# Meryx/ComputeRayTracer

Measured on AMD Instinct MI355X. Metric: Mrays/sec (+ HBM GB/s vs peak), 1080p 250k-tri scene, 1/2/4/8 MI355X, higher is better.
Workload: dtype f32; 1 GPU; S2 atrium250k: 253952 triangles + cornell walls/light, 1920x1080, 64 spp per step (BASELINE config 3)

## Files before the change

computeraytracer_amd/_lib.py:

```python
from __future__ import annotations

import ctypes as C
import os

_HERE = os.path.dirname(os.path.abspath(__file__))
LIB_PATH = os.environ.get("CRT_LIB") or os.path.join(_HERE, "libcrt.so")

NCOUNTERS = 8
ACCEL_NONE, ACCEL_BVH2, ACCEL_LBVH, ACCEL_PLOC = 0, 1, 2, 3
CNT = dict(rays=0, nodes=1, prims=2, paths=3, bounces=4, shadow=5, hits=6, walked=7)

_P = C.c_void_p
SIGNATURES = {
    "crt_create": (C.c_int, [C.POINTER(_P), C.c_int]),
    "crt_destroy": (None, [_P]),
    "crt_last_error": (C.c_char_p, [_P]),
    "crt_abi_version": (C.c_int, []),
    "crt_upload_scene": (C.c_int, [_P, _P, C.c_size_t, _P, C.c_size_t, _P, C.c_size_t, _P, _P]),
    "crt_set_tile": (C.c_int, [_P, C.c_uint32, C.c_uint32, C.c_uint32, C.c_uint32]),
    "crt_set_row_bands": (C.c_int, [_P, C.c_uint32, C.c_uint32, C.c_uint32]),
    "crt_build_accel": (C.c_int, [_P, C.c_int]),
    "crt_reset": (C.c_int, [_P]),
    "crt_trace": (C.c_int, [_P, C.c_uint32]),
    "crt_sync": (C.c_int, [_P]),
    "crt_sample_count": (C.c_int, [_P, _P]),
    "crt_tile": (C.c_int, [_P, _P]),
    "crt_read_accum": (C.c_int, [_P, _P]),
    "crt_read_rgba8": (C.c_int, [_P, _P]),
    "crt_write_accum": (C.c_int, [_P, _P, C.c_uint32]),
    "crt_read_latest_rgba8": (C.c_int, [_P, _P, _P]),
    "crt_latest_sample": (C.c_int, [_P, _P]),
    "crt_pin_host": (C.c_int, [_P, C.c_size_t]),
    "crt_unpin_host": (C.c_int, [_P]),
    "crt_read_sample_rgba8": (C.c_int, [_P, C.c_uint32, _P]),
    "crt_device_buffers": (C.c_int, [_P, C.POINTER(_P), C.POINTER(_P)]),
    "crt_bind_output": (C.c_int, [_P, _P, _P]),
    "crt_set_stream": (C.c_int, [_P, _P]),
    "crt_enable_counters": (C.c_int, [_P, C.c_int]),
    "crt_counters": (C.c_int, [_P, _P]),
    "crt_reset_counters": (C.c_int, [_P]),
    "crt_last_trace_ms": (C.c_int, [_P, _P, _P]),
    "crt_last_kernel_ms": (C.c_int, [_P, _P, _P]),
    "crt_set_option": (C.c_int, [_P, C.c_char_p, C.c_int64]),
    "crt_accel_stats": (C.c_int, [_P, _P]),
    "crt_get_device": (C.c_int, [_P, _P]),
    "crt_get_stream": (C.c_int, [_P, C.POINTER(_P)]),
    "crt_image_size": (C.c_int, [_P, _P]),
    "crt_comm_unique_id": (C.c_int, [_P, C.c_int]),
    "crt_comm_init": (C.c_int, [_P, _P, C.c_int, C.c_int]),
    "crt_comm_partition": (C.c_int, [_P, C.c_uint32]),
    "crt_gather": (C.c_int, [_P, C.c_int]),
    "crt_read_frame_rgba8": (C.c_int, [_P, _P]),
    "crt_read_frame_accum": (C.c_int, [_P, _P]),
    "crt_frame_device_buffers": (C.c_int, [_P, C.POINTER(_P), C.POINTER(_P)]),
    "crt_comm_info": (C.c_int, [_P, _P]),
    "crt_comm_destroy": (C.c_int, [_P]),
    "crt_layout_rows": (C.c_int, [C.c_uint32, C.c_uint32, C.c_uint32, C.c_uint32, _P, _P]),
    "crt_denoise": (C.c_int, [_P, _P, _P, _P]),
    "crt_denoise_latest": (C.c_int, [_P, _P, _P, _P, _P]),
    "crt_read_gbuffer": (C.c_int, [_P, _P]),
    "crt_read_motion": (C.c_int, [_P, _P]),
    "crt_render_aovs": (C.c_int, [_P, C.c_uint32, _P]),
    "crt_spectrum_rgb": (C.c_int, [_P, _P, _P]),
    "crt_read_albedo_table": (C.c_int, [_P, _P]),
    "crt_render_mattes": (C.c_int, [_P, C.c_uint32, C.c_int, C.c_uint32, _P]),
    "crt_set_primitive_ids": (C.c_int, [_P, C.c_uint32, C.c_uint32, _P]),
    "crt_read_primitive_ids": (C.c_int, [_P, C.c_uint32, C.c_uint32, _P]),
    "crt_debug_intersect": (C.c_int, [_P, _P, C.c_size_t, _P]),
    "crt_debug_trace_rays": (C.c_int, [_P, _P, C.c_size_t, _P, _P]),
    "crt_debug_walk_rays": (C.c_int, [_P, C.c_int, _P, C.c_size_t, _P, _P]),
    "crt_debug_read_accel": (C.c_int, [_P, C.c_int, _P, C.c_size_t, _P]),
    "crt_debug_probes": (C.c_int, [_P, _P]),
    "crt_debug_gen_culled": (C.c_int, [_P, _P]),
    "crt_debug_deferred_nee": (C.c_int, [_P, _P]),
    "crt_debug_tile_classes": (C.c_int, [_P, _P, C.c_size_t]),
    "crt_debug_tile_classes_host": (C.c_int, [_P, _P, C.c_size_t]),
    "crt_debug_tile_class_setups": (C.c_int, [_P, _P]),
# ... 120 lines not shown
```

computeraytracer_amd/csrc/crt_api.cpp:

```cpp
#include "crt_ctx.h"

using namespace crt;

extern "C" void crt_comm_on_destroy(crt_ctx *c);
extern "C" int crt_internal_comm_partitioned(crt_ctx *c);

namespace crt {

long long g_fail_alloc_in = 0;

namespace {
std::string g_create_error;
}

int fail(crt_ctx *c, int code, const char *fmt, ...)
{
    char buf[2048];
    va_list ap;
    va_start(ap, fmt);
    vsnprintf(buf, sizeof buf, fmt, ap);
    va_end(ap);
    if (c) c->err = buf; else g_create_error = buf;
    return code;
}
// ... 182 lines not shown
            return fail(c, CRT_EINVAL, "primitive %zu: spectrum index out of range", i);
    }
    for (size_t i = 0; i < nlight; i++) {
        lts[i] = read_prim((const uint8_t *)lights, i);
        if (lts[i].emission >= nspectra) return fail(c, CRT_EINVAL, "light %zu: emission index out of range", i);
    }
    c->have_scene = false;
    c->accel_mode = -1;
    c->dn.valid = false; c->fdn.valid = false;
    c->sample_offset = 0;
    c->dn.drop();
    c->prims.swap(prims);
    c->prims_moved = false;
    matte_ids_identity(c);
    c->lights.swap(lts);
    std::memcpy(c->camera, camera, sizeof c->camera);
    c->W = (uint32_t)camera[11];
    c->H = (uint32_t)camera[12];

    DevScene &S = c->sc;
    S = DevScene{};
    S.W = c->W; S.H = c->H;
    S.nspectra = (uint32_t)nspectra;
    S.nlight = (uint32_t)nlight;
    S.inv_nlight = 1.0f / (float)S.nlight;
    c->s_prims = prims_scale(c->prims);
    S.hit_pad = pad_of(c->s_prims, c->camera);
    c->accel_stale = false; c->accel_topo = false;
    c->rf_ready = false;
    S.nf_last[0] = S.nf_last[1] = kNoHit;
    for (size_t i = c->prims.size(); i-- > 0 && S.nf_last[1] == kNoHit;)
        if (c->prims[i].category != 2u) (S.nf_last[0] == kNoHit ? S.nf_last[0] : S.nf_last[1]) = (uint32_t)i;
    camera_frame(c->camera, S.cam);

    HIPCHK(c, c->d_raw.alloc(std::max<size_t>(nprim * 80, 16)));
    if (nprim) HIPCHK(c, hipMemcpy(c->d_raw.p, primitives, nprim * 80, hipMemcpyHostToDevice));
    HIPCHK(c, c->d_spectra.alloc(nspectra * kNLambda));
    HIPCHK(c, hipMemcpy(c->d_spectra.p, spectra, nspectra * kNLambda * sizeof(float), hipMemcpyHostToDevice));
    HIPCHK(c, c->d_cie.alloc(3 * kNCie));
    HIPCHK(c, hipMemcpy(c->d_cie.p, cie, 3 * kNCie * sizeof(float), hipMemcpyHostToDevice));
    c->cie_zero = tc_culled_is_zero(cie);
    aov_rebuild_albedo(c, spectra, nspectra, cie);
    std::vector<float4> hl(nlight * 3);
    for (size_t i = 0; i < nlight; i++) light_rows(c->lights[i], &hl[3 * i]);
    HIPCHK(c, c->d_lights.alloc(hl.size()));
    HIPCHK(c, hipMemcpy(c->d_lights.p, hl.data(), hl.size() * sizeof(float4), hipMemcpyHostToDevice));
    S.spectra = c->d_spectra.p; S.cie = c->d_cie.p; S.lights = c->d_lights.p;

    c->x0 = 0; c->y0 = 0; c->tw = c->W; c->th = c->H;
    c->band = 0x40000000u; c->stride = 1; c->phase = 0;
    c->accum_bound = nullptr; c->rgba_bound = nullptr;
    c->have_scene = true;
    int rc = alloc_tile(c);
    if (rc == CRT_OK) rc = zero_state(c);
    if (rc) c->have_scene = false;
    return rc;
}

int crt_set_tile(crt_ctx *c, uint32_t x0, uint32_t y0, uint32_t x1, uint32_t y1)
{
    if (!c) return CRT_EINVAL;
    if (!c->have_scene) return fail(c, CRT_ESTATE, "crt_set_tile: upload a scene first");
    if (x0 > x1 || y0 > y1 || x1 > c->W || y1 > c->H)
        return fail(c, CRT_EINVAL, "crt_set_tile: rectangle [%u,%u)x[%u,%u) outside %ux%u", x0, x1, y0, y1, c->W, c->H);
    CRT_TRY(quiesce(c, true));
    c->x0 = x0; c->y0 = y0; c->tw = x1 - x0; c->th = y1 - y0;
    c->band = 0x40000000u; c->stride = 1; c->phase = 0;
    return retile(c);
}

int crt_set_row_bands(crt_ctx *c, uint32_t band_rows, uint32_t parts, uint32_t part)
{
    if (!c) return CRT_EINVAL;
    if (!c->have_scene) return fail(c, CRT_ESTATE, "crt_set_row_bands: upload a scene first");
    if (band_rows == 0 || parts == 0 || part >= parts || band_rows > 65536u)
        return fail(c, CRT_EINVAL, "crt_set_row_bands: need band_rows >= 1 and part < parts");
    CRT_TRY(quiesce(c, true));
    uint32_t rows = 0;
    for (uint32_t b = part; (unsigned long long)b * band_rows < c->H; b += parts)
        rows += std::min<uint32_t>(band_rows, c->H - b * band_rows);
    c->x0 = 0; c->y0 = 0; c->tw = c->W; c->th = rows;
    c->band = band_rows; c->stride = parts; c->phase = part;
    return retile(c);
}

int crt_build_accel(crt_ctx *c, int mode)
{
    if (!c) return CRT_EINVAL;
    if (!c->have_scene) return fail(c, CRT_ESTATE, "crt_build_accel: upload a scene first");
    if (mode != CRT_ACCEL_NONE && mode != CRT_ACCEL_BVH2 && mode != CRT_ACCEL_LBVH && mode != CRT_ACCEL_PLOC)
        return fail(c, CRT_EINVAL, "crt_build_accel: unknown mode %d", mode);
    c->want_builder = mode == CRT_ACCEL_LBVH ? 1 : mode == CRT_ACCEL_PLOC ? 2 : 0;
    if (c->want_builder) mode = CRT_ACCEL_BVH2;
    CRT_TRY(quiesce(c, true));
    c->accel_mode = -1;
    c->dn.valid = false; c->fdn.valid = false;
    return build_tree(c, mode);
}

int crt_reset(crt_ctx *c)
{
    if (!c) return CRT_EINVAL;
    if (!c->have_scene) return fail(c, CRT_ESTATE, "crt_reset: upload a scene first");
    CRT_TRY(quiesce(c, false));
    return zero_state(c);
}

int crt_trace(crt_ctx *c, uint32_t n_samples)
{
    if (!c) return CRT_EINVAL;
    if (c->as_on) return as_refuse(c, "crt_trace");
    if (!c->have_scene) return fail(c, CRT_ESTATE, "crt_trace: upload a scene first");
    if (c->accel_mode < 0) return fail(c, CRT_ESTATE, "crt_trace: call crt_build_accel first");
    if (c->accel_stale) return fail(c, CRT_ESTATE, "crt_trace: primitives were updated: call crt_refit_accel or crt_build_accel first");
    if (c->sample_offset) {
        if (!(c->pipeline == 1 && c->accel_mode == CRT_ACCEL_BVH2))
            return fail(c, CRT_ESTATE, "crt_trace: a sample offset needs the wavefront pipeline (\"pipeline\" = 1 and a tree): "
                                       "crt_set_sample_offset(ctx, 0) first");
        if ((unsigned long long)c->sample_offset + c->sample + n_samples > 0xFFFFFFFFull)
            return fail(c, CRT_EINVAL, "crt_trace: sample offset %u + %u samples so far + %u pass 2^32 - 1", c->sample_offset, c->sample, n_samples);
    }
    HIPCHK(c, hipSetDevice(c->device));
    if ((size_t)c->tw * c->th != 0 && (!accum_ptr(c) || !rgba_ptr(c)))
        return fail(c, CRT_ENOMEM, "crt_trace: the tile's output buffers are not allocated (an earlier crt_set_tile / crt_set_row_bands failed)");
    TraceParams P = trace_params(c);
    c->last_launches = 0;
    c->last_timed = true;
    c->last_iterations = 0;
    HIPCHK(c, hipEventRecord(c->ev0, c->stream));
// ... 451 lines not shown
        if (!c->time_kernels) return fail(c, CRT_ESTATE, "crt_last_kernel_ms: set option time_kernels=1 before crt_trace");
        HIPCHK(c, hipStreamSynchronize(c->stream));
        n = c->last_trace_kernel_launches;
        for (uint32_t i = 0; i < n; i++) {
            float t = 0.0f;
            HIPCHK(c, hipEventElapsedTime(&t, c->kev[2 * (size_t)i], c->kev[2 * (size_t)i + 1]));
            total += t;
        }
        c->last_trace_kernel_launches = 0;
    } else {
        HIPCHK(c, hipEventElapsedTime(&total, c->ev0, c->ev1));
        n = c->last_launches;
    }
    if (ms) *ms = total;
    if (launches) *launches = n;
    return CRT_OK;
}

int crt_accel_stats(crt_ctx *c, uint64_t out[8])
{
    if (!c || !out) return CRT_EINVAL;
    if (c->accel_topo) return fail(c, CRT_ESTATE, "crt_accel_stats: the tree belongs to another primitive list: call crt_refit_accel or crt_build_accel first");
    const bool wide = c->pipeline == 1 && c->accel_mode == CRT_ACCEL_BVH2 && c->bvh4.n_inner > 0;
    const bool wide8 = wide && c->bvh8q.ok;
    out[4] = wide ? (c->bvh4q.ok ? 16 : 32) : 32;
    out[5] = wide8 ? 8 : wide ? 4 : 2;
    out[6] = wide8 ? c->bvh8q.n_inner : wide ? c->bvh4.n_inner : c->bvh.n_inner;
    out[7] = (uint64_t)c->accel_builder;
    out[0] = c->bvh.n_inner; out[1] = c->bvh.n_leaves; out[2] = c->bvh.max_depth;
    out[3] = (uint64_t)c->bvh.n_inner * 64u + (uint64_t)c->bvh4.n_inner * 128u + (uint64_t)c->prims.size() * 48u;
    return CRT_OK;
}

int crt_set_option(crt_ctx *c, const char *name, int64_t value)
{
    if (!c || !name) return CRT_EINVAL;
    CRT_TRY(wf_flush(c));
    if (!std::strcmp(name, "debug_fail_alloc")) { g_fail_alloc_in = value; return CRT_OK; }
    if (!std::strcmp(name, "ploc_radius")) {
        if (value < 1 || value > 32) return fail(c, CRT_EINVAL, "crt_set_option: ploc_radius is 1..32");
        c->ploc.radius = (uint32_t)value;
        return CRT_OK;
    }
    if (!std::strcmp(name, "refit_rebuild_pct")) {
        if (value != 0 && (value < 100 || value > 100000)) return fail(c, CRT_EINVAL, "crt_set_option: refit_rebuild_pct is 0 (off) or 100..100000");
        c->refit_rebuild_pct = (int)value;
        return CRT_OK;
    }
    if (!std::strcmp(name, "debug_ploc_max_depth")) {
        if (value < 1 || value > 62) return fail(c, CRT_EINVAL, "crt_set_option: debug_ploc_max_depth is 1..62");
        c->ploc.max_depth = (uint32_t)value;
        return CRT_OK;
    }
    if (!std::strcmp(name, "debug_ploc_max_rounds")) {
        if (value < 1) return fail(c, CRT_EINVAL, "crt_set_option: debug_ploc_max_rounds is >= 1");
        c->ploc.max_rounds = (uint32_t)std::min<int64_t>(value, 1 << 30);
        return CRT_OK;
    }
    if (!std::strcmp(name, "wf_defer")) { c->wf_defer = value != 0; return CRT_OK; }
    if (!std::strcmp(name, "spp_per_launch")) { c->spp_per_launch = (uint32_t)std::max<int64_t>(0, value); return CRT_OK; }
    if (!std::strcmp(name, "pipeline")) { c->pipeline = value ? 1 : 0; return CRT_OK; }
    if (!std::strcmp(name, "quantize")) { c->quantize = value ? 1 : 0; return CRT_OK; }
    if (!std::strcmp(name, "wf_width")) { c->wf_width = value == 4 ? 4 : 8; return CRT_OK; }
    if (!std::strcmp(name, "wf_finish_at")) { c->wf_finish_at = (uint32_t)std::max<int64_t>(0, value); return CRT_OK; }
    if (!std::strcmp(name, "wf_flush_at")) { c->wf_flush_at = (uint32_t)std::max<int64_t>(0, value); return CRT_OK; }
    if (!std::strcmp(name, "wf_side_ppw")) { c->wf_side_ppw = (uint32_t)std::min<int64_t>(64, std::max<int64_t>(1, value)); return CRT_OK; }
// ... 15 lines not shown
    if (!std::strcmp(name, "adaptive_temporal")) {
        if (value != 0 && value != 1) return fail(c, CRT_EINVAL, "crt_set_option: adaptive_temporal is 0 or 1");
        c->adaptive_temporal = value != 0;
        return CRT_OK;
    }
    if (!std::strcmp(name, "svgf_spatial_pct")) {
        if (value != 0 && (value < 25 || value > 10000)) return fail(c, CRT_EINVAL, "crt_set_option: svgf_spatial_pct is 0 (off) or 25..10000");
        c->svgf_spatial_pct = (int)value;
        return CRT_OK;
    }
    if (!std::strcmp(name, "denoise_latest_wave_blocks")) {
        if (value != 0 && value != 1) return fail(c, CRT_EINVAL, "crt_set_option: denoise_latest_wave_blocks is 0 or 1");
        c->dn.wave_blocks = value != 0;
        return CRT_OK;
    }
    if (!std::strcmp(name, "temporal_clip_pct")) {
        if (value != 0 && (value < 25 || value > 10000)) return fail(c, CRT_EINVAL, "crt_set_option: temporal_clip_pct is 0 (off) or 25..10000");
        if (!value && c->dn.relit) c->dn.drop();
        if (!value) { c->dn.box.release(); c->dn.box_ran = false; }
        c->dn.clip_pct = (int)value;
        return CRT_OK;
    }
    if (!std::strcmp(name, "frame_ring")) {
        c->frame_ring = (uint32_t)std::min<int64_t>(256, std::max<int64_t>(0, value));
        c->ring_from = c->sample + 1u;
        if (c->have_scene) { HIPCHK(c, hipSetDevice(c->device)); HIPCHK(c, hipStreamSynchronize(c->stream)); return alloc_frames(c); }
        return CRT_OK;
    }
    if (!std::strcmp(name, "wf_gen_blocks")) { c->wf_gen_blocks = (int)std::min<int64_t>(4096, std::max<int64_t>(1, value)); return CRT_OK; }
    if (!std::strcmp(name, "wf_trace_form")) { c->wf_trace_form = value == 1 ? 1 : 2; return CRT_OK; }
    if (!std::strcmp(name, "wf_cull_miss")) { c->wf_cull_miss = value != 0; return CRT_OK; }
    if (!std::strcmp(name, "wf_cull_classes")) { c->wf_cull_classes = value != 0; return CRT_OK; }
    if (!std::strcmp(name, "wf_defer_nee")) { c->wf_defer_nee = value != 0; return CRT_OK; }
    if (!std::strcmp(name, "wf_affinity")) { c->wf_affinity = value != 0; return CRT_OK; }
    if (!std::strcmp(name, "wf_pipes")) { c->wf_pipes = (int)std::min<int64_t>(crt_ctx::kMaxPipes, std::max<int64_t>(1, value)); return CRT_OK; }
    if (!std::strcmp(name, "wf_pool")) { c->wf_pool = (uint32_t)std::max<int64_t>(0, value); return CRT_OK; }
    if (!std::strcmp(name, "wf_waves_per_cu")) { c->wf_waves_per_cu = (uint32_t)std::min<int64_t>(32, std::max<int64_t>(0, value)); return CRT_OK; }
    if (!std::strcmp(name, "time_kernels")) {
        c->time_kernels = value != 0; c->last_trace_kernel_launches = 0;
        HIPCHK(c, hipSetDevice(c->device));
        while (value > 1 && c->kev.size() < 2 * (size_t)std::min<int64_t>(value, 1 << 20)) {
            Event e;
            HIPCHK(c, e.create());
            c->kev.push_back(std::move(e));
        }
        return CRT_OK;
    }
    return fail(c, CRT_EINVAL, "crt_set_option: unknown option '%s'", name);
}

}
```

computeraytracer_amd/csrc/crt_ctx.h:

```cpp
#pragma once
#include <hip/hip_runtime.h>

#include <algorithm>
#include <cfloat>
#include <cmath>
#include <cstdarg>
#include <cstdio>
#include <cstdlib>
#include <cstring>
#include <memory>
#include <string>
#include <utility>
#include <vector>

#include "../../include/crt.h"
#include "crt_bvh.h"
#include "crt_device.h"
#include "crt_launch.h"
#include "crt_math.h"
#include "crt_tile_class.h"
#include "crt_wf_policy.h"

namespace crt {

struct HostPrim {
    uint32_t category;
    f3 d1, d2, d3;
    uint32_t emission, reflectance, material, index;
};

extern long long g_fail_alloc_in;

template <typename T>
struct DevBuf {
    T *p = nullptr;
    size_t n = 0;
    DevBuf() = default;
    DevBuf(DevBuf &&o) noexcept : p(o.p), n(o.n) { o.p = nullptr; o.n = 0; }
    DevBuf &operator=(DevBuf &&o) noexcept { std::swap(p, o.p); std::swap(n, o.n); return *this; }
    DevBuf(const DevBuf &) = delete;
    DevBuf &operator=(const DevBuf &) = delete;
    ~DevBuf() { release(); }
    hipError_t alloc(size_t count) {
        release();
        if (count == 0) return hipSuccess;
        const bool inject = g_fail_alloc_in > 0 && --g_fail_alloc_in == 0;
        const hipError_t e = inject ? hipErrorOutOfMemory : hipMalloc((void **)&p, count * sizeof(T));
        if (e != hipSuccess) { p = nullptr; return e; }
        n = count;
        return hipSuccess;
    }
    void release() { if (p) (void)hipFree(p); p = nullptr; n = 0; }
// ... 97 lines not shown
    uint32_t published = 0;
    uint32_t pending = 0;
    bool in_publish = false;
    uint32_t sample_offset = 0;
    uint32_t frame_id = 0;
    int wf_cohort = 16;

    DevBuf<unsigned long long> d_counters;
    bool counting = false;
    float last_ms = 0.0f;
    uint32_t last_launches = 0;
    bool last_timed = false;
    uint32_t spp_per_launch = 0;

    int pipeline = 1;
    uint32_t wf_pool = 0;
    uint32_t wf_waves_per_cu = 0;
    int num_cu = 0;
    DevBuf<float4> w_ray_o, w_ray_d, w_sh_d, w_beta, w_radiance, w_nee, w_staging[crt::kWfRing], w_recA, w_recB;
    DevBuf<uint4> w_rng, w_misc, w_recC;
    DevBuf<float2> w_hit;
    DevBuf<uint32_t> w_vis, w_dead, w_tea;
    DevBuf<uint8_t> w_dflag;
    DevBuf<uint32_t> w_tile_cls;
    static constexpr int kMaxPipes = crt::kWfMaxPipes;
    int wf_pipes = 2;
    int wf_defer = 1;
    int wf_tail_walk = 1;
    int wf_gen_blocks = 128;
    int wf_trace_form = 2;
    int wf_cull_miss = 1;
    int wf_cull_classes = 1;
    int wf_defer_nee = 1;
    int wf_affinity = 0;
    uint64_t mapped_gen_launches = 0;
    uint64_t tile_cls_setups = 0;
    bool cie_zero = false;
    int wf_chunk = 1;
    int wf_ahead = 3;
    int wf_ring = 32;
    int wf_pool_spp = 8;
    double wf_feed = 1.0;
    std::unique_ptr<crt::WfRun> run;
    uint32_t wf_finish_at = 32768;
    uint32_t wf_flush_at = 4096;
    uint32_t wf_side_ppw = 64, wf_flush_ppw = 4;
    DevBuf<crt::WfCtl> w_ctl[kMaxPipes];
    DevBuf<crt::WfWorkQ> w_wq;
    crt::Pinned<crt::WfStatus> h_status[kMaxPipes];
    crt::WfStatus *d_status[kMaxPipes] = {};
    crt::Event ev_status[kMaxPipes][crt::kStatusRing];
    crt::Event ev_done[kMaxPipes][crt::kStatusRing];
    crt::Pinned<uint32_t> h_dropped;
    bool wf_host_ready = false;
    crt::Stream pipe_stream[kMaxPipes];
    crt::Stream pub_stream;
    static constexpr int kFinishStreams = 3;
    crt::Stream fin_stream[kFinishStreams];
    crt::Event ev_fin[kFinishStreams];
    int fin_next = 0;
    crt::Event ev_fork, ev_join[kMaxPipes], ev_pub_join[kMaxPipes];
    crt::Event ev_evict[kMaxPipes][crt::kWfRing];
    crt::Event ev_resolved[crt::kWfRing];
    crt::Event ev_pub[crt::kWfRing];
    bool time_kernels = false;
    std::vector<crt::Event> kev;
// ... 107 lines not shown
        hipError_t e_ = (call);                                                                   \
        if (e_ != hipSuccess)                                                                     \
            return fail(c, e_ == hipErrorOutOfMemory ? CRT_ENOMEM : CRT_EDEVICE, "%s: %s", #call, \
                        hipGetErrorString(e_));                                                   \
    } while (0)

#define CRT_TRY(expr)                 \
    do {                              \
        const int rc_ = (expr);       \
        if (rc_) return rc_;          \
    } while (0)

#define CRT_ENSURE(c, buf, count)                              \
    do {                                                       \
        if (buf.n < (count)) HIPCHK(c, buf.alloc(count));      \
    } while (0)

inline float4 *accum_ptr(crt_ctx *c) { return c->accum_bound ? c->accum_bound : c->d_accum.p; }
inline uchar4 *rgba_ptr(crt_ctx *c) { return c->rgba_bound ? c->rgba_bound : c->d_rgba.p; }

int quiesce(crt_ctx *c, bool sync);

int alloc_tile(crt_ctx *c);
int zero_state(crt_ctx *c);
int as_refuse(crt_ctx *c, const char *what);
int as_refuse_broken(crt_ctx *c, const char *what);

HostPrim read_prim(const uint8_t *base, size_t i);
float prims_scale(const std::vector<HostPrim> &prims);
float pad_of(float S, const float cam[16]);
void light_rows(const HostPrim &l, float4 out[3]);
void camera_frame(const float cam[16], float out[12]);
int build_tree(crt_ctx *c, int mode);
uint32_t wf_stack_need(const crt_ctx *c);
uint32_t wf_stack_lds(const crt_ctx *c);
uint32_t wf_overflow_levels(const crt_ctx *c);

enum DnState { DN_UNIFORM, DN_ADAPTIVE, DN_EITHER, DN_TEMPORAL };
int dn_begin(crt_ctx *c, const char *what, uint32_t iterations, const float *values, int count, const char *which, DnState state);
int dn_finish(crt_ctx *c, size_t n, const float4 *res, float *rgb_out, uint8_t *rgba8_out, const float *plane = nullptr,
              float *plane_out = nullptr);
int dn_adaptive_params(crt_ctx *c, const char *what, const crt_denoise_adaptive_params *params, crt_denoise_adaptive_params *out);
int dn_check_state(crt_ctx *c, const char *what, bool adaptive = false);
int dn_adaptive_run(crt_ctx *c, const crt_denoise_adaptive_params &dp, bool rgba, bool var, float4 **res, const float **var_dev);

void aov_rebuild_albedo(crt_ctx *c, const float *spectra, size_t nspectra, const float *cie);

void matte_ids_identity(crt_ctx *c);
void matte_ids_reserve(crt_ctx *c, size_t n_new);
void matte_ids_remove(crt_ctx *c, const crt_prim_range *live, size_t m);
void matte_ids_append(crt_ctx *c, uint32_t count);

struct AsBatch {
    uint32_t off;
    uint32_t n_active;
    uint32_t commit;
};
WfOptions wf_options(const crt_ctx *c);
int wf_ensure_overflow(crt_ctx *c);
int wf_flush(crt_ctx *c);
int wf_check_dropped(crt_ctx *c);
int wf_tick(crt_ctx *c);
int wf_publish_pending(crt_ctx *c, bool force);
int wf_trace_batch(crt_ctx *c, uint32_t n, const AsBatch *as = nullptr);
int wf_wait_sample(crt_ctx *c, uint32_t sample);
double wf_now_ms();
// ... 4 lines not shown
```

computeraytracer_amd/csrc/crt_debug.cpp:

```cpp
#include "crt_ctx.h"

using namespace crt;

extern "C" {

int crt_debug_intersect(crt_ctx *c, const float *rays, size_t n, float *out)
{
    if (!c || (!rays && n) || (!out && n)) return CRT_EINVAL;
    if (!c->have_scene || c->accel_mode < 0) return fail(c, CRT_ESTATE, "crt_debug_intersect: scene + accel required");
    if (c->accel_stale) return fail(c, CRT_ESTATE, "crt_debug_intersect: primitives were updated: call crt_refit_accel or crt_build_accel first");
    HIPCHK(c, hipSetDevice(c->device));
    DevBuf<float> din, dout;
    HIPCHK(c, din.alloc(n * 8));
    hipError_t e = dout.alloc(n * 8);
    if (e == hipSuccess) e = hipMemcpyAsync(din.p, rays, n * 8 * sizeof(float), hipMemcpyHostToDevice, c->stream);
    if (e == hipSuccess) e = launch_debug_intersect(c->sc, din.p, n, dout.p, c->accel_mode == CRT_ACCEL_NONE, c->stream);
    if (e == hipSuccess) e = hipMemcpyAsync(out, dout.p, n * 8 * sizeof(float), hipMemcpyDeviceToHost, c->stream);
    if (e == hipSuccess) e = hipStreamSynchronize(c->stream);
    if (e != hipSuccess) return fail(c, CRT_EDEVICE, "crt_debug_intersect: %s", hipGetErrorString(e));
    return CRT_OK;
}

int crt_debug_trace_rays(crt_ctx *c, const float *rays, size_t n, uint32_t *out, uint64_t report[8])
{
// ... 166 lines not shown
    const bool device_route = tree && n4 > 0 && c->bvh4.nodes.size() < n4 * (size_t)kNode4Floats;
    const bool live4 = tree && n4 > 0 && !device_route, live4q = tree && n4 > 0 && c->sc.nodes4q != nullptr, live8q = n8 > 0 && c->sc.nodes8q != nullptr;
    double hdr[CRT_ACCEL_HEADER_N] = {0};
    const void *src = nullptr;
    size_t need = 0;
    switch (what) {
    case CRT_ACCEL_PART_HEADER: {
        const size_t lanes = (size_t)c->num_cu * wf_waves(wf_options(c)) * 64u * (size_t)std::max(1, c->wf_pipes);
        hdr[0] = c->accel_mode; hdr[1] = c->accel_builder; hdr[2] = (double)n;
        hdr[3] = tree ? c->sc.root : -1; hdr[4] = tree ? c->sc.root4 : -1; hdr[5] = live8q ? c->sc.root8 : -1;
        hdr[6] = (double)n2; hdr[7] = (double)n4; hdr[8] = (double)n8;
        hdr[9] = live4; hdr[10] = live4q; hdr[11] = live8q;
        for (int a = 0; a < 3; a++) { hdr[12 + a] = c->sc.qbase[a]; hdr[15 + a] = c->sc.qscale[a]; }
        hdr[18] = c->sc.hit_pad; hdr[19] = c->tree_pad;
        hdr[20] = c->bvh.max_depth; hdr[21] = c->bvh4.max_depth; hdr[22] = c->bvh8q.max_depth; hdr[23] = c->wf_depth;
        hdr[24] = wf_stack_need(c); hdr[25] = wf_stack_lds(c); hdr[26] = wf_overflow_levels(c);
        hdr[27] = lanes ? (double)(c->w_overflow.n / lanes) : 0.0;
        hdr[28] = c->accel_stale; hdr[29] = device_route;
        need = sizeof hdr;
        break;
    }
    case CRT_ACCEL_PART_NODES2: src = c->d_nodes.p; need = n2 * kNodeFloats * sizeof(float); break;
    case CRT_ACCEL_PART_NODES4: src = c->d_nodes4.p; need = live4 ? n4 * kNode4Floats * sizeof(float) : 0; break;
    case CRT_ACCEL_PART_NODES4Q: src = c->d_nodes4q.p; need = live4q ? n4 * 16 * sizeof(uint32_t) : 0; break;
    case CRT_ACCEL_PART_NODES8Q: src = c->d_nodes8q.p; need = live8q ? n8 * 32 * sizeof(uint32_t) : 0; break;
    case CRT_ACCEL_PART_PRIM: src = c->d_prim.p; need = n * 3 * sizeof(float4); break;
    case CRT_ACCEL_PART_PRIMD: src = c->d_primD.p; need = tree ? n * sizeof(float4) : 0; break;
    default: src = c->d_slot_of_index.p; need = n * sizeof(uint32_t); break;
    }
    if (bytes) *bytes = need;
    if (!out) return CRT_OK;
    if (capacity < need) return fail(c, CRT_EINVAL, "crt_debug_read_accel: part %d holds %zu bytes, the buffer %zu", what, need, capacity);
    if (what == CRT_ACCEL_PART_HEADER) std::memcpy(out, hdr, need);
    else if (need) HIPCHK(c, hipMemcpy(out, src, need, hipMemcpyDeviceToHost));
    return CRT_OK;
}

int crt_debug_math(crt_ctx *c, int fn, const float *a, const float *b, float *out, size_t n)
{
    if (!c || !a || !b || !out) return CRT_EINVAL;
    HIPCHK(c, hipSetDevice(c->device));
    DevBuf<float> da, db, dout;
    hipError_t e = da.alloc(n);
    if (e == hipSuccess) e = db.alloc(n);
    if (e == hipSuccess) e = dout.alloc(n);
    if (e == hipSuccess && n) e = hipMemcpyAsync(da.p, a, n * sizeof(float), hipMemcpyHostToDevice, c->stream);
    if (e == hipSuccess && n) e = hipMemcpyAsync(db.p, b, n * sizeof(float), hipMemcpyHostToDevice, c->stream);
    if (e == hipSuccess) e = launch_debug_math(fn, da.p, db.p, dout.p, n, c->stream);
    if (e == hipSuccess && n) e = hipMemcpyAsync(out, dout.p, n * sizeof(float), hipMemcpyDeviceToHost, c->stream);
    if (e == hipSuccess) e = hipStreamSynchronize(c->stream);
    if (e != hipSuccess) return fail(c, CRT_EDEVICE, "crt_debug_math: %s", hipGetErrorString(e));
    return CRT_OK;
}

int crt_debug_read_moments(crt_ctx *c, float *out)
{
    if (!c || !out) return CRT_EINVAL;
    CRT_TRY(dn_begin(c, "crt_debug_read_moments", 0, nullptr, 0, "", DN_TEMPORAL));
    if (!c->dn.cur.valid || c->dn.cur.frame != c->frame_id || !c->dn.cur.has_m)
        return fail(c, CRT_ESTATE, "crt_debug_read_moments: no crt_denoise_svgf in this frame yet, or a crt_denoise_temporal after it "
                                   "(the CURRENT slot carries no moments)");
    const size_t n = (size_t)c->tw * c->th;
    if (n) HIPCHK(c, hipMemcpyAsync(out, c->dn.cur.m.p, n * sizeof(float4), hipMemcpyDeviceToHost, c->stream));
    return dn_finish(c, n, nullptr, nullptr, nullptr);
}

// ... 81 lines not shown
```

computeraytracer_amd/csrc/crt_device.h:

```cpp
#pragma once
#include <hip/hip_runtime.h>
#include <stdint.h>

#include "crt_work_map.h"

namespace crt {

constexpr uint32_t kNoHit = 0xFFFFFFFFu;
constexpr int kStackDepth = 64;
constexpr uint32_t kWalk4q = 1u, kWalkFellBack = 2u;
constexpr uint32_t kNLambda = 301;
constexpr uint32_t kNCie = 471;
constexpr int CRT_NCOUNTERS_DEV = 16;

struct DevScene {
    const float4 *prim;
    const float4 *primD;
    const uint32_t *slot_of_index;
    const float4 *nodes;
    const float4 *nodes4;
    const uint4 *nodes4q;
    const uint4 *nodes8q;
    const float *spectra;
    const float *cie;
    const float4 *lights;
    uint32_t nprim;
    uint32_t npatch;
    int32_t root;
    int32_t root4;
    int32_t root8;
    uint32_t n_nodes4;
    uint32_t nspectra;
    uint32_t nlight;
    float hit_pad;
    uint32_t nf_last[2];
    float inv_nlight;
    uint32_t W, H;
    float qbase[3], qscale[3];
    float cam[12];
};

struct TraceParams {
    DevScene sc;
    uint32_t x0, y0, tw, th;
    uint32_t band, stride, phase;
    uint32_t first_sample, n_samples;
    float4 *accum;
    uchar4 *rgba;
    unsigned long long *counters;
    uint32_t tiles_x, tiles_y;
};

struct AsTiles {
    const uint32_t *active;
    const uint32_t *base;
    float *q;
    uint32_t n_active;
};

struct AsParams {
    const float4 *accum;
    const float *q;
    const uint32_t *counts;
    float *errors;
    uint32_t *flags;
    uint32_t *active;
    uint32_t *n_active;
    uint32_t tw, th, tiles_x, tiles_y;
    uint32_t min_samples, max_samples;
    float threshold;
};

struct AsVarParams {
// ... 220 lines not shown
```

computeraytracer_amd/csrc/crt_launch.h:

```cpp
#pragma once
#include <hip/hip_runtime.h>

#include <vector>

#include "../../include/crt.h"
#include "crt_bvh.h"
#include "crt_device.h"

namespace crt {

hipError_t launch_trace(const TraceParams &P, bool count, bool brute, hipStream_t stream);
hipError_t launch_trace_adaptive(const TraceParams &P, const AsTiles &A, bool count, bool brute, hipStream_t stream);
hipError_t launch_debug_intersect(const DevScene &S, const float *rays, size_t n, float *out, int brute, hipStream_t stream);
hipError_t launch_debug_walk_rays(const DevScene &S, int walk, const float *rays, size_t n, uint32_t *out, hipStream_t stream);
hipError_t launch_debug_math(int fn, const float *a, const float *b, float *out, size_t n, hipStream_t stream);
hipError_t launch_assemble(const void *full, void *frame, uint32_t elem_bytes, uint32_t W, uint32_t H, uint32_t world, uint32_t rows_max,
                           uint32_t band, hipStream_t stream);

hipError_t wf_launch_init(const WfParams &P, hipStream_t s);
hipError_t wf_launch_tea(const WfParams &P, uint32_t *out, hipStream_t s);
hipError_t wf_launch_tile_classes(const WfParams &P, uint32_t *out, hipStream_t s);
bool wf_gen_culls(const WfParams &P);
bool wf_gen_mapped(const WfParams &P);
hipError_t wf_launch_shade(const WfParams &P, uint32_t it, hipStream_t s);
hipError_t wf_launch_gen(const WfParams &P, uint32_t it, hipStream_t s, const AsTiles *A);
hipError_t wf_launch_trace(const WfParams &P, uint32_t it, uint32_t trace_blocks, hipStream_t s);
int wf_trace_kernel(const WfParams &P);
hipError_t wf_launch_finish(const WfParams &P, WfFinishSegs G, uint32_t max_paths, hipStream_t s);
hipError_t wf_launch_resolve(const WfParams &P, uint32_t last_sample, hipStream_t s);
hipError_t wf_launch_resolve_adaptive(const WfParams &P, const AsTiles &A, uint32_t call_end, hipStream_t s);

hipError_t as_launch_select(const AsParams &A, bool compact, hipStream_t s);
hipError_t as_launch_select_var(const AsVarParams &V, const AsParams *compact, hipStream_t s);
hipError_t as_launch_commit(uint32_t *counts, const uint32_t *active, uint32_t n_active, uint32_t samples, hipStream_t s);

hipError_t build_lbvh(const float *lo, const float *hi, uint32_t n, Bvh &out, hipStream_t stream);
hipError_t build_lbvh_device(const unsigned char *d_raw, uint32_t n, float hit_pad, float4 *d_prim, float4 *d_primD,
                             uint32_t *d_slot_of_index, float *d_nodes2, uint4 *d_nodes4q, LbvhDeviceResult &res, hipStream_t stream);
template <typename T> struct DevBuf;
hipError_t lbvh_sorted_keys_host(const float *lo, const float *hi, uint32_t n, float *d_lo, float *d_hi, unsigned long long *d_keys,
                                 unsigned long long *d_sorted, DevBuf<char> &sort_tmp, hipStream_t stream);
hipError_t lbvh_sorted_keys_device(const unsigned char *d_raw, uint32_t n, float hit_pad, float *d_lo, float *d_hi, uint32_t *d_cbox,
                                   unsigned long long *d_keys, unsigned long long *d_sorted, DevBuf<char> &sort_tmp, hipStream_t stream);
hipError_t lbvh_launch_gather(const unsigned char *d_raw, const unsigned long long *d_keys, uint32_t n, float4 *d_prim, float4 *d_primD,
                              uint32_t *d_slot_of_index, hipStream_t stream);
hipError_t lbvh_collapse_device(const float *d_nodes2, uint32_t n, uint4 *d_nodes4q, LbvhDeviceResult &res, hipStream_t stream);

hipError_t build_ploc(const float *lo, const float *hi, uint32_t n, const PlocOptions &opt, Bvh &out, PlocInfo &info, hipStream_t stream);
hipError_t build_ploc_device(const unsigned char *d_raw, uint32_t n, float hit_pad, const PlocOptions &opt, float4 *d_prim, float4 *d_primD,
                             uint32_t *d_slot_of_index, float *d_nodes2, uint4 *d_nodes4q, LbvhDeviceResult &res, PlocInfo &info,
                             hipStream_t stream);

hipError_t refit_launch_pad(const unsigned char *raw, uint32_t n, uint32_t *out, hipStream_t s);
hipError_t refit_launch_prims(const unsigned char *raw, uint32_t first, uint32_t count, const uint32_t *slot_of_index, float4 *prim,
                              float4 *primD, hipStream_t s);
hipError_t refit_launch_transform(unsigned char *raw, const uint32_t *start, const crt_prim_transform *ops, uint32_t n_ops, uint32_t total,
                                  const uint32_t *slot_of_index, float4 *prim, float4 *primD, hipStream_t s);
hipError_t refit_launch_compact(const unsigned char *src, unsigned char *dst, const uint32_t *tab, uint32_t n_gaps, uint32_t n_new, hipStream_t s);
hipError_t refit_levels(const void *nodes, uint32_t width, bool quantised, int root, uint32_t cap, int *list, uint32_t *counter,
                        uint32_t *nch, std::vector<uint32_t> &off, hipStream_t s);
hipError_t refit_launch_bvh2(const float4 *prim, float pad, const int *list, const std::vector<uint32_t> &off, float *nodes, hipStream_t s);
hipError_t refit_launch_wide(const float4 *prim, float pad, const int *list, const std::vector<uint32_t> &off, const void *refs,
                             bool quantised, const uint32_t *nch, float *fb, hipStream_t s);
hipError_t refit_launch_quant4(const float *fb, const uint32_t *nch, uint32_t n4, uint4 *nodes4q, const double base[3], const double scale[3],
                               hipStream_t s);

hipError_t quality_launch(int layout, const void *nodes, uint32_t n, uint32_t root, const float base[3], const float scale[3],
                          double2 *partial, double *out, hipStream_t s);

hipError_t dn_launch_gbuffer(const DevScene &S, uint32_t x0, uint32_t y0, uint32_t tw, uint32_t th, float4 *gbuf, uint32_t *key,
                             int brute, hipStream_t stream);
hipError_t dn_launch_filter(const DnFilter &F, const float4 *accum, float n, float sigma_color, float4 **out);
hipError_t dn_launch_prepare(const DnFilter &F, const float4 *accum, float n, hipStream_t stream);
hipError_t dn_launch_passes(const DnFilter &F, float sigma_color, bool wave_blocks, float4 **out);
hipError_t dn_launch_filter_adaptive(const DnFilter &F, const float4 *accum, const float *q, const uint32_t *counts, uint2 *kv,
                                     float *var, float sigma_variance, float4 **out);
hipError_t dn_launch_temporal(const DnFilter &F, DnReprojParams P, const uint32_t *counts, float sigma_color, float4 *box, float gamma,
                              float4 **out);
hipError_t dn_launch_svgf(const DnFilter &F, DnSvgfParams P, const uint32_t *counts, uint2 *kv, float *var, float sigma_variance,
                          float spatial_b, float4 *box, float gamma, float4 **out);
hipError_t dn_launch_motion(const DnReprojParams &P, float2 *out, hipStream_t stream);

hipError_t aov_launch(const DevScene &S, const AovParams &P, hipStream_t stream);

hipError_t matte_launch(const DevScene &S, const MatteParams &P, hipStream_t stream);

}
```

computeraytracer_amd/csrc/crt_lbvh.hip:

```cpp
#include <hip/hip_runtime.h>
#include <hipcub/hipcub.hpp>

#include <algorithm>
#include <cfloat>
#include <cstring>
#include <vector>

#include "crt_bvh.h"
#include "crt_ctx.h"
#include "crt_launch.h"
#include "crt_math.h"
#include "crt_prim.h"

namespace crt {
namespace {

__device__ __forceinline__ uint32_t expand10(uint32_t v)
{
    v &= 0x3FFu;
    v = (v | (v << 16)) & 0x030000FFu;
    v = (v | (v << 8)) & 0x0300F00Fu;
    v = (v | (v << 4)) & 0x030C30C3u;
    v = (v | (v << 2)) & 0x09249249u;
    return v;
// ... 262 lines not shown
        if (best < 0) break;
        CBox a, b;
        load_children(nodes2, ch[best].ref, a, b);
        ch[best] = a; ch[n++] = b;
    }
    uint32_t k = 0;
    for (int i = 0; i < n; i++) k += ch[i].ref >= 0 ? 1u : 0u;
    uint32_t pos = 0;
    if (k) pos = atomicAdd(out_count, k);
    int refs[4] = {0, 0, 0, 0};
    uint32_t j = 0;
    for (int i = 0; i < n; i++) {
        if (ch[i].ref >= 0) { frontier_out[pos + j] = ch[i].ref; refs[i] = (int)(next_base + pos + j); j++; }
        else refs[i] = ch[i].ref;
    }
    const double base[3] = {bx, by, bz}, scale[3] = {sx, sy, sz};
    uint32_t q[24];
    for (int i = 0; i < 4; i++)
        for (int a = 0; a < 3; a++) {
            if (i >= n) { q[4 * a + i] = 65535u; q[12 + 4 * a + i] = 0u; continue; }
            const double l = ((double)ch[i].lo[a] - base[a]) / scale[a], h = ((double)ch[i].hi[a] - base[a]) / scale[a];
            long long ql = (long long)floor(l) - 1, qh = (long long)ceil(h) + 1;
            ql = ql < 0 ? 0 : (ql > 65535 ? 65535 : ql); qh = qh < 0 ? 0 : (qh > 65535 ? 65535 : qh);
            q[4 * a + i] = (uint32_t)ql; q[12 + 4 * a + i] = (uint32_t)qh;
        }
    uint4 *o = nodes4q + 4 * (size_t)(level_base + t);
    o[0] = uint4{q[0] | (q[1] << 16), q[2] | (q[3] << 16), q[4] | (q[5] << 16), q[6] | (q[7] << 16)};
    o[1] = uint4{q[8] | (q[9] << 16), q[10] | (q[11] << 16), q[12] | (q[13] << 16), q[14] | (q[15] << 16)};
    o[2] = uint4{q[16] | (q[17] << 16), q[18] | (q[19] << 16), q[20] | (q[21] << 16), q[22] | (q[23] << 16)};
    o[3] = uint4{(uint32_t)refs[0], (uint32_t)refs[1], (uint32_t)refs[2], (uint32_t)refs[3]};
}

__global__ __launch_bounds__(256) void k_lbvh_gather_prims(const unsigned char *__restrict__ raw, const unsigned long long *__restrict__ keys, uint32_t n,
                                                           float4 *__restrict__ prim, float4 *__restrict__ primD, uint32_t *__restrict__ slot_of_index)
{
    const uint32_t slot = blockIdx.x * 256u + threadIdx.x;
    if (slot >= n) return;
    const RawPrim p = load_raw(raw, (size_t)(keys[slot] & 0xFFFFFFFFull));
    float4 A, B, C, D;
    prim_record(p, A, B, C, D);
    prim[3 * (size_t)slot + 0] = A; prim[3 * (size_t)slot + 1] = B; prim[3 * (size_t)slot + 2] = C;
    primD[slot] = D;
    slot_of_index[p.index] = slot;
}

}

hipError_t lbvh_sorted_keys_device(const unsigned char *d_raw, uint32_t n, float hit_pad, float *d_lo, float *d_hi, uint32_t *d_cbox,
                                   unsigned long long *d_keys, unsigned long long *d_sorted, DevBuf<char> &sort_tmp, hipStream_t stream)
{
    hipError_t e;
    const uint32_t cinit[6] = {0xFFFFFFFFu, 0xFFFFFFFFu, 0xFFFFFFFFu, 0u, 0u, 0u};
    LB(hipMemcpyAsync(d_cbox, cinit, sizeof cinit, hipMemcpyHostToDevice, stream));
    const unsigned blocks = (n + 255u) / 256u;
    hipLaunchKernelGGL(k_lbvh_prim_bounds, dim3(blocks), dim3(256), 0, stream, d_raw, n, hit_pad, d_lo, d_hi, d_cbox);
    LB(hipGetLastError());
    hipLaunchKernelGGL(k_lbvh_keys_dev, dim3(blocks), dim3(256), 0, stream, d_lo, d_hi, n, d_cbox, d_keys);
    LB(hipGetLastError());
    size_t tmp_bytes = 0;
    LB(hipcub::DeviceRadixSort::SortKeys(nullptr, tmp_bytes, d_keys, d_sorted, (int)n, 0, 62, stream));
    LB(sort_tmp.alloc(std::max<size_t>(tmp_bytes, 1)));
    LB(hipcub::DeviceRadixSort::SortKeys(sort_tmp.p, tmp_bytes, d_keys, d_sorted, (int)n, 0, 62, stream));
    return hipSuccess;
}

hipError_t lbvh_launch_gather(const unsigned char *d_raw, const unsigned long long *d_keys, uint32_t n, float4 *d_prim, float4 *d_primD,
                              uint32_t *d_slot_of_index, hipStream_t stream)
{
    hipLaunchKernelGGL(k_lbvh_gather_prims, dim3((n + 255u) / 256u), dim3(256), 0, stream, d_raw, d_keys, n, d_prim, d_primD, d_slot_of_index);
    return hipGetLastError();
}

hipError_t lbvh_collapse_device(const float *d_nodes2, uint32_t n, uint4 *d_nodes4q, LbvhDeviceResult &res, hipStream_t stream)
{
    hipError_t e;
    DevBuf<int> d_front[2];
    DevBuf<unsigned int> d_count;
    float rootrec[kNodeFloats];
    LB(hipMemcpyAsync(rootrec, d_nodes2, sizeof rootrec, hipMemcpyDeviceToHost, stream));
    LB(hipStreamSynchronize(stream));
    double base[3], scale[3];
    for (int a = 0; a < 3; a++) {
        const float glo = std::min(rootrec[a], rootrec[6 + a]), ghi = std::max(rootrec[3 + a], rootrec[9 + a]);
        if (!(glo > -1.0e30f) || !(ghi < 1.0e30f)) return hipSuccess;
        const float ext = std::max(ghi - glo, 1.0e-3f);
        const float mag = std::max(std::fabs(glo), std::fabs(ghi));
        if (mag > 16.0f * ext) return hipSuccess;
        res.qbase[a] = glo; res.qscale[a] = ext / 65533.0f;
        base[a] = res.qbase[a]; scale[a] = res.qscale[a];
    }
    LB(d_front[0].alloc(n / 2 + 2)); LB(d_front[1].alloc(n / 2 + 2)); LB(d_count.alloc(1));
    const int root = 0;
    LB(hipMemcpyAsync(d_front[0].p, &root, sizeof root, hipMemcpyHostToDevice, stream));
    uint32_t count = 1, level_base = 0;
    int cur = 0;
    for (int level = 0; count > 0; level++) {
        if (level > 64) return hipErrorUnknown;
        LB(hipMemsetAsync(d_count.p, 0, 4, stream));
        hipLaunchKernelGGL(k_lbvh_collapse_level, dim3((count + 255u) / 256u), dim3(256), 0, stream, d_nodes2, (const int *)d_front[cur].p, count,
                           level_base, d_front[cur ^ 1].p, d_count.p, level_base + count, d_nodes4q, base[0], base[1], base[2], scale[0], scale[1], scale[2]);
        LB(hipGetLastError());
        uint32_t next = 0;
        LB(hipMemcpyAsync(&next, d_count.p, 4, hipMemcpyDeviceToHost, stream));
        LB(hipStreamSynchronize(stream));
        level_base += count;
        count = next;
        cur ^= 1;
        res.depth4 = (uint32_t)level + 1u;
    }
    res.n_nodes4 = level_base;
    res.quantised = true;
    return hipSuccess;
}

hipError_t build_lbvh_device(const unsigned char *d_raw, uint32_t n, float hit_pad, float4 *d_prim, float4 *d_primD,
                             uint32_t *d_slot_of_index, float *d_nodes2, uint4 *d_nodes4q, LbvhDeviceResult &res, hipStream_t stream)
{
    res = LbvhDeviceResult();
    if (n < 2) return hipErrorInvalidValue;
    Tmp<float> d_lo, d_hi, d_nb;
    Tmp<unsigned long long> d_keys, d_sorted;
    Tmp<int> d_child, d_pi, d_pl, d_height;
    Tmp<unsigned int> d_flag, d_small;
    DevBuf<char> d_tmp;
    hipError_t e;
    LB(d_lo.alloc((size_t)n * 3)); LB(d_hi.alloc((size_t)n * 3));
    LB(d_keys.alloc(n)); LB(d_sorted.alloc(n));
    LB(d_child.alloc((size_t)2 * (n - 1))); LB(d_pi.alloc(n - 1)); LB(d_pl.alloc(n));
    LB(d_flag.alloc(n - 1)); LB(d_nb.alloc((size_t)6 * (n - 1))); LB(d_height.alloc(n - 1));
    LB(d_small.alloc(16));
    LB(hipMemsetAsync(d_flag.p, 0, (size_t)(n - 1) * 4, stream));
    LB(lbvh_sorted_keys_device(d_raw, n, hit_pad, d_lo.p, d_hi.p, d_small.p, d_keys.p, d_sorted.p, d_tmp, stream));
    const unsigned blocks = (n + 255u) / 256u;
    hipLaunchKernelGGL(k_lbvh_hierarchy, dim3(blocks), dim3(256), 0, stream, d_sorted.p, (int)n, d_child.p, d_pi.p, d_pl.p);
    LB(hipGetLastError());
    hipLaunchKernelGGL(k_lbvh_bounds, dim3(blocks), dim3(256), 0, stream, d_sorted.p, (int)n, d_lo.p, d_hi.p, d_child.p, d_pi.p, d_pl.p,
                       d_flag.p, d_nb.p, d_nodes2, d_height.p);
    LB(hipGetLastError());
    LB(lbvh_launch_gather(d_raw, d_sorted.p, n, d_prim, d_primD, d_slot_of_index, stream));
    int depth = 0;
    LB(hipMemcpyAsync(&depth, d_height.p, sizeof depth, hipMemcpyDeviceToHost, stream));
    LB(hipStreamSynchronize(stream));
    res.max_depth = (uint32_t)depth;
    return lbvh_collapse_device(d_nodes2, n, d_nodes4q, res, stream);
}
#undef LB

}
```

computeraytracer_amd/csrc/crt_matte.hip:

```cpp
#include "crt_launch.h"
#include "crt_shade.h"

namespace crt {

__global__ __launch_bounds__(64) void k_matte(const DevScene S, const MatteParams P)
{
    __shared__ int lds_stack[kStackDepth * 64];
    extern __shared__ uint32_t lds_table[];
    const uint32_t lane = threadIdx.x;
    const uint32_t lx = (blockIdx.x % P.tiles_x) * 8u + (lane & 7u), ly = (blockIdx.x / P.tiles_x) * 8u + (lane >> 3);
    if (lx >= P.tw || ly >= P.th) return;
    int *stk = lds_stack + lane;
    uint32_t *tid = lds_table + lane, *tcount = lds_table + P.slots * 64u + lane;
    const uint32_t px = P.x0 + lx, py = P.y0 + ly;
    const uint32_t n = P.counts ? P.counts[blockIdx.x] : P.n;
    const uint32_t tea_xy = tea(px, py * 100u);
    uint32_t h = 0, used = 0, over = 0;
    for (uint32_t j = 1; j <= n; j++) {
        Rng rng;
        f3 o, d;
        primary_ray(S, px, py, P.first + j, tea_xy, rng, o, d);
        float t_max = CRT_INFINITY;
        uint32_t b_index = kNoHit, b_slot = kNoHit, cn = 0, cp = 0;
        if (P.brute || !finite3(o) || !finite3(d)) {
            for (uint32_t i = 0; i < S.nprim; i++)
                hit_test<true>(S, S.slot_of_index[i], o, d, 0xFFFFFFFFu, 0.001f, t_max, b_index, b_slot);
        } else {
            traverse<false>(S, stk, o, d, 0xFFFFFFFFu, false, t_max, b_index, b_slot, cn, cp);
        }
        if (b_slot == kNoHit) continue;
        uint32_t id = b_index;
        if (P.source == CRT_MATTE_OBJECT) {
            id = P.table[b_index];
        } else if (P.source == CRT_MATTE_MATERIAL) {
            const uint32_t meta = f_bits(S.prim[3 * b_slot].w);
            id = (((meta >> 2) & 3u) << 24) | ((meta >> 18) & 0x3FFFu);
        }
        h++;
        uint32_t s = 0;
        while (s < used && tid[s * 64u] != id) s++;
        if (s < used) {
            tcount[s * 64u]++;
        } else if (used < P.slots) {
            tid[used * 64u] = id;
            tcount[used * 64u] = 1u;
            used++;
        } else {
            over++;
        }
    }
    const size_t npix = (size_t)P.tw * P.th, pix = (size_t)ly * P.tw + lx;
    for (uint32_t r = 0; r < P.slots; r++) {
        uint32_t id = 0xFFFFFFFFu, count = 0;
        if (r < used) {
            uint32_t best = r;
            id = tid[r * 64u];
            count = tcount[r * 64u];
            for (uint32_t s = r + 1; s < used; s++) {
                const uint32_t is = tid[s * 64u], cs = tcount[s * 64u];
                if (cs > count || (cs == count && is < id)) { best = s; id = is; count = cs; }
            }
            if (best != r) {
                tid[best * 64u] = tid[r * 64u];
                tcount[best * 64u] = tcount[r * 64u];
            }
        }
        if (P.ids) P.ids[r * npix + pix] = id;
        if (P.counts_out) P.counts_out[r * npix + pix] = count;
// ... 15 lines not shown
```

computeraytracer_amd/csrc/crt_ploc.hip:

```cpp
#include <hip/hip_runtime.h>
#include <hipcub/hipcub.hpp>

#include <algorithm>
#include <cfloat>
#include <utility>
#include <vector>

#include "crt_bvh.h"
#include "crt_ctx.h"
#include "crt_launch.h"
#include "crt_math.h"

namespace crt {
namespace {

constexpr int kPlocBlock = 256;
constexpr int kPlocMaxRadius = 32;
constexpr int kPlocStage = kPlocBlock + 2 * kPlocMaxRadius;

struct PlocClusters {
    float *box;
    int *ref;
    uint32_t *cnt;
    int *height;
// ... 180 lines not shown
}

}

hipError_t build_ploc(const float *lo, const float *hi, uint32_t n, const PlocOptions &opt, Bvh &out, PlocInfo &info, hipStream_t stream)
{
    out = Bvh();
    info = PlocInfo();
    if (n < 2) return hipErrorInvalidValue;
    DevBuf<float> d_lo, d_hi, d_nodes;
    DevBuf<unsigned long long> d_keys, d_sorted, d_order;
    DevBuf<char> d_tmp;
    hipError_t e;
    PL(d_lo.alloc((size_t)n * 3)); PL(d_hi.alloc((size_t)n * 3));
    PL(d_keys.alloc(n)); PL(d_sorted.alloc(n)); PL(d_order.alloc(n));
    PL(d_nodes.alloc((size_t)(n - 1) * kNodeFloats));
    PL(lbvh_sorted_keys_host(lo, hi, n, d_lo.p, d_hi.p, d_keys.p, d_sorted.p, d_tmp, stream));
    PL(ploc_core(d_sorted.p, d_lo.p, d_hi.p, n, opt, d_nodes.p, d_order.p, info, stream));
    if (info.abandoned) return hipSuccess;
    out.nodes.resize((size_t)(n - 1) * kNodeFloats);
    std::vector<unsigned long long> keys(n);
    PL(hipMemcpyAsync(out.nodes.data(), d_nodes.p, out.nodes.size() * sizeof(float), hipMemcpyDeviceToHost, stream));
    PL(hipMemcpyAsync(keys.data(), d_order.p, (size_t)n * 8, hipMemcpyDeviceToHost, stream));
    PL(hipStreamSynchronize(stream));
    out.order.resize(n);
    for (size_t s = 0; s < n; s++) out.order[s] = (uint32_t)(keys[s] & 0xFFFFFFFFull);
    out.root = 0;
    out.n_inner = n - 1;
    out.n_leaves = n;
    out.max_depth = info.depth;
    return hipSuccess;
}

hipError_t build_ploc_device(const unsigned char *d_raw, uint32_t n, float hit_pad, const PlocOptions &opt, float4 *d_prim, float4 *d_primD,
                             uint32_t *d_slot_of_index, float *d_nodes2, uint4 *d_nodes4q, LbvhDeviceResult &res, PlocInfo &info,
                             hipStream_t stream)
{
    res = LbvhDeviceResult();
    info = PlocInfo();
    if (n < 2) return hipErrorInvalidValue;
    DevBuf<float> d_lo, d_hi;
    DevBuf<unsigned long long> d_keys, d_sorted, d_order;
    DevBuf<uint32_t> d_cbox;
    DevBuf<char> d_tmp;
    hipError_t e;
    PL(d_lo.alloc((size_t)n * 3)); PL(d_hi.alloc((size_t)n * 3));
    PL(d_keys.alloc(n)); PL(d_sorted.alloc(n)); PL(d_order.alloc(n)); PL(d_cbox.alloc(8));
    PL(lbvh_sorted_keys_device(d_raw, n, hit_pad, d_lo.p, d_hi.p, d_cbox.p, d_keys.p, d_sorted.p, d_tmp, stream));
    PL(ploc_core(d_sorted.p, d_lo.p, d_hi.p, n, opt, d_nodes2, d_order.p, info, stream));
    if (info.abandoned) return hipSuccess;
    PL(lbvh_launch_gather(d_raw, d_order.p, n, d_prim, d_primD, d_slot_of_index, stream));
    res.max_depth = info.depth;
    return lbvh_collapse_device(d_nodes2, n, d_nodes4q, res, stream);
}
#undef PL

}
```

computeraytracer_amd/csrc/crt_prim.h:

```cpp
#pragma once
#include <hip/hip_runtime.h>

#include "crt_math.h"

namespace crt {

struct RawPrim { uint32_t category; f3 d1, d2, d3; uint32_t emission, reflectance, material, index; };

__device__ __forceinline__ RawPrim load_raw(const unsigned char *__restrict__ raw, size_t i)
{
    const uint4 *r = (const uint4 *)(raw + i * 80);
    const uint4 a = r[0], b = r[1], c = r[2], d = r[3], e = r[4];
    RawPrim p;
    p.category = a.x;
    p.d1 = f3{bits_f(b.x), bits_f(b.y), bits_f(b.z)};
    p.d2 = f3{bits_f(c.x), bits_f(c.y), bits_f(c.z)};
    p.d3 = f3{bits_f(d.x), bits_f(d.y), bits_f(d.z)};
    p.emission = e.x; p.reflectance = e.y; p.material = e.z; p.index = e.w;
    return p;
}

__device__ __forceinline__ void prim_bounds(uint32_t category, f3 d1, f3 d2, f3 d3, float pad, float l[3], float h[3])
{
    const float S = pad * 131072.0f;
    f3 cs[4];
    int nc;
    if (category == 1u) {
        const float r = abs_(d2.x);
        cs[0] = f3{d1.x - r, d1.y - r, d1.z - r}; cs[1] = f3{d1.x + r, d1.y + r, d1.z + r}; nc = 2;
    } else {
        cs[0] = d1; cs[1] = d1 + d2; cs[2] = d1 + d3; nc = 3;
        if (category == 0u) { cs[3] = cs[1] + d3; nc = 4; }
    }
    l[0] = cs[0].x; l[1] = cs[0].y; l[2] = cs[0].z; h[0] = cs[0].x; h[1] = cs[0].y; h[2] = cs[0].z;
    for (int k = 1; k < nc; k++) {
        l[0] = fminf(l[0], cs[k].x); l[1] = fminf(l[1], cs[k].y); l[2] = fminf(l[2], cs[k].z);
        h[0] = fmaxf(h[0], cs[k].x); h[1] = fmaxf(h[1], cs[k].y); h[2] = fmaxf(h[2], cs[k].z);
    }
// ... 51 lines not shown
```

computeraytracer_amd/csrc/crt_refit.hip:

```cpp
#include <hip/hip_runtime.h>

#include <vector>

#include "../../include/crt.h"
#include "crt_bvh.h"
#include "crt_launch.h"
#include "crt_math.h"
#include "crt_prim.h"

namespace crt {
namespace {

__device__ __forceinline__ void leaf_box(const float4 *__restrict__ prim, uint32_t first, uint32_t count, float pad, float b[6])
{
    for (uint32_t k = 0; k < count; k++) {
        const float4 A = prim[3 * (size_t)(first + k) + 0], B = prim[3 * (size_t)(first + k) + 1], C = prim[3 * (size_t)(first + k) + 2];
        float l[3], h[3];
        prim_bounds(f_bits(A.w) & 3u, f3{A.x, A.y, A.z}, f3{B.x, B.y, B.z}, f3{C.x, C.y, C.z}, pad, l, h);
        for (int a = 0; a < 3; a++) {
            b[a] = k ? fminf(b[a], l[a]) : l[a];
            b[3 + a] = k ? fmaxf(b[3 + a], h[a]) : h[a];
        }
    }
}

__global__ __launch_bounds__(256) void k_refit_pad(const unsigned char *__restrict__ raw, uint32_t n, uint32_t *__restrict__ out)
{
    const uint32_t i = blockIdx.x * 256u + threadIdx.x;
    float S = 0.0f;
    if (i < n) {
        const RawPrim p = load_raw(raw, i);
        f3 c[4];
        int nc;
        if (p.category == 1u) {
            const float r = abs_(p.d2.x);
            c[0] = f3{p.d1.x - r, p.d1.y - r, p.d1.z - r}; c[1] = f3{p.d1.x + r, p.d1.y + r, p.d1.z + r}; nc = 2;
        } else {
            c[0] = p.d1; c[1] = p.d1 + p.d2; c[2] = p.d1 + p.d3; nc = 3;
            if (p.category == 0u) { c[3] = c[1] + p.d3; nc = 4; }
        }
        for (int k = 0; k < nc; k++) { S = max_(S, abs_(c[k].x)); S = max_(S, abs_(c[k].y)); S = max_(S, abs_(c[k].z)); }
    }
    uint32_t u = f_bits(S);
    for (int off = 32; off > 0; off >>= 1) { const uint32_t o = (uint32_t)__shfl_xor((int)u, off, 64); u = o > u ? o : u; }
    if ((threadIdx.x & 63u) == 0u) atomicMax(out, u);
}

__global__ __launch_bounds__(256) void k_refit_prims(const unsigned char *__restrict__ raw, uint32_t first, uint32_t count,
                                                     const uint32_t *__restrict__ slot_of_index, float4 *__restrict__ prim,
                                                     float4 *__restrict__ primD)
{
    const uint32_t k = blockIdx.x * 256u + threadIdx.x;
    if (k >= count) return;
    const RawPrim p = load_raw(raw, (size_t)first + k);
    float4 A, B, C, D;
    prim_record(p, A, B, C, D);
    const uint32_t slot = slot_of_index[first + k];
    prim[3 * (size_t)slot + 0] = A; prim[3 * (size_t)slot + 1] = B; prim[3 * (size_t)slot + 2] = C;
    primD[slot] = D;
}

__device__ __forceinline__ f3 xf_vector(const float *__restrict__ m, f3 v)
{
    return f3{__fadd_rn(__fadd_rn(__fmul_rn(m[0], v.x), __fmul_rn(m[1], v.y)), __fmul_rn(m[2], v.z)),
              __fadd_rn(__fadd_rn(__fmul_rn(m[4], v.x), __fmul_rn(m[5], v.y)), __fmul_rn(m[6], v.z)),
              __fadd_rn(__fadd_rn(__fmul_rn(m[8], v.x), __fmul_rn(m[9], v.y)), __fmul_rn(m[10], v.z))};
}
__device__ __forceinline__ f3 xf_point(const float *__restrict__ m, f3 p)
{
    const f3 v = xf_vector(m, p);
    return f3{__fadd_rn(v.x, m[3]), __fadd_rn(v.y, m[7]), __fadd_rn(v.z, m[11])};
}

__global__ __launch_bounds__(256) void k_refit_transform(unsigned char *raw, const uint32_t *__restrict__ start, const crt_prim_transform *__restrict__ ops,
                                                         uint32_t n_ops, uint32_t total, const uint32_t *__restrict__ slot_of_index,
                                                         float4 *__restrict__ prim, float4 *__restrict__ primD)
{
    const uint32_t t = blockIdx.x * 256u + threadIdx.x;
    if (t >= total) return;
    uint32_t lo = 0, hi = n_ops;
    while (hi - lo > 1u) {
        const uint32_t mid = (lo + hi) >> 1;
        if (start[mid] <= t) lo = mid; else hi = mid;
    }
    const crt_prim_transform &op = ops[lo];
    const size_t i = (size_t)op.first + (t - start[lo]);
    RawPrim p = load_raw(raw, i);
    float *rec = (float *)(raw + i * 80);
    p.d1 = xf_point(op.m, p.d1);
    rec[4] = p.d1.x; rec[5] = p.d1.y; rec[6] = p.d1.z;
    if (p.category == 1u) {
        p.d2.x = __fmul_rn(p.d2.x, op.radius_scale);
        rec[8] = p.d2.x;
    } else {
        p.d2 = xf_vector(op.m, p.d2);
        p.d3 = xf_vector(op.m, p.d3);
        rec[8] = p.d2.x; rec[9] = p.d2.y; rec[10] = p.d2.z;
        rec[12] = p.d3.x; rec[13] = p.d3.y; rec[14] = p.d3.z;
    }
    if (!prim) return;
    float4 A, B, C, D;
    prim_record(p, A, B, C, D);
    const uint32_t slot = slot_of_index[i];
    prim[3 * (size_t)slot + 0] = A; prim[3 * (size_t)slot + 1] = B; prim[3 * (size_t)slot + 2] = C;
    primD[slot] = D;
}

__global__ __launch_bounds__(256) void k_edit_compact(const uint4 *__restrict__ src, uint4 *__restrict__ dst, const uint32_t *__restrict__ gap,
                                                      const uint32_t *__restrict__ cum, uint32_t n_gaps, uint32_t n_new)
{
    const size_t t = (size_t)blockIdx.x * 256u + threadIdx.x;
    if (t >= (size_t)n_new * 5u) return;
    const uint32_t j = (uint32_t)(t / 5u), chunk = (uint32_t)(t - (size_t)j * 5u);
    uint32_t lo = 0, hi = n_gaps;
    while (lo < hi) {
        const uint32_t mid = (lo + hi) >> 1;
        if (gap[mid] <= j) lo = mid + 1; else hi = mid;
    }
    uint4 v = src[((size_t)j + cum[lo]) * 5u + chunk];
    if (chunk == 4u) v.w = j;
    dst[t] = v;
}

__global__ __launch_bounds__(256) void k_refit_expand(const uint32_t *__restrict__ nodes, uint32_t stride, uint32_t ref_at, uint32_t width,
                                                      const int *__restrict__ in, uint32_t count, int *__restrict__ out, uint32_t cap,
                                                      uint32_t *__restrict__ out_count, uint32_t *__restrict__ nch)
{
    const uint32_t t = blockIdx.x * 256u + threadIdx.x;
    if (t >= count) return;
    const int node = in[t];
    int inner[4];
    uint32_t k = 0, m = 0;
    for (uint32_t c = 0; c < width; c++) {
        const int ref = (int)nodes[(size_t)node * stride + ref_at + c];
        if (width == 4 && ref == 0) continue;
        m++;
        if (ref >= 0) inner[k++] = ref;
    }
    if (nch) nch[node] = m;
    if (!k) return;
    const uint32_t pos = atomicAdd(out_count, k);
    for (uint32_t j = 0; j < k; j++)
        if (pos + j < cap) out[pos + j] = inner[j];
}

__global__ __launch_bounds__(256) void k_refit_bvh2(const float4 *__restrict__ prim, float pad, const int *__restrict__ list, uint32_t count,
                                                    float *__restrict__ nodes)
{
    const uint32_t t = blockIdx.x * 256u + threadIdx.x;
    if (t >= count) return;
    float *nd = nodes + (size_t)list[t] * kNodeFloats;
    for (int c = 0; c < 2; c++) {
        const int ref = (int)f_bits(nd[12 + c]);
        float b[6];
        if (ref < 0) {
            leaf_box(prim, (uint32_t)(~ref) >> 3, ((uint32_t)(~ref) & 7u) + 1u, pad, b);
        } else {
            const float4 *ch = (const float4 *)(nodes + (size_t)ref * kNodeFloats);
            const float4 q0 = ch[0], q1 = ch[1], q2 = ch[2];
            b[0] = fminf(q0.x, q1.z); b[1] = fminf(q0.y, q1.w); b[2] = fminf(q0.z, q2.x);
            b[3] = fmaxf(q0.w, q2.y); b[4] = fmaxf(q1.x, q2.z); b[5] = fmaxf(q1.y, q2.w);
        }
        for (int a = 0; a < 6; a++) nd[6 * c + a] = b[a];
    }
}

__global__ __launch_bounds__(256) void k_refit_wide(const float4 *__restrict__ prim, float pad, const int *__restrict__ list, uint32_t count,
                                                    const uint32_t *__restrict__ refs, uint32_t stride, uint32_t ref_at,
                                                    const uint32_t *__restrict__ nch, float *__restrict__ fb)
{
    const uint32_t t = blockIdx.x * 256u + threadIdx.x;
    if (t >= count) return;
    const int node = list[t];
    float *nd = fb + (size_t)node * kNode4Floats;
    for (uint32_t c = 0; c < 4; c++) {
        const int ref = (int)refs[(size_t)node * stride + ref_at + c];
        if (ref == 0) continue;
        float b[6];
        if (ref < 0) {
            leaf_box(prim, (uint32_t)(~ref) >> 3, ((uint32_t)(~ref) & 7u) + 1u, pad, b);
        } else {
            const float *ch = fb + (size_t)ref * kNode4Floats;
            const uint32_t k = nch[ref];
            for (int a = 0; a < 6; a++) b[a] = ch[4 * a];
            for (uint32_t i = 1; i < k; i++)
                for (int a = 0; a < 3; a++) { b[a] = fminf(b[a], ch[4 * a + i]); b[3 + a] = fmaxf(b[3 + a], ch[12 + 4 * a + i]); }
        }
        for (int a = 0; a < 6; a++) nd[4 * a + c] = b[a];
    }
}

__global__ __launch_bounds__(256) void k_refit_quant4(const float *__restrict__ fb, const uint32_t *__restrict__ nch, uint32_t n4,
                                                      uint4 *__restrict__ nodes4q, double bx, double by, double bz, double sx, double sy, double sz)
{
    const uint32_t t = blockIdx.x * 256u + threadIdx.x;
    if (t >= n4) return;
    const float *nd = fb + (size_t)t * kNode4Floats;
    const uint32_t n = nch[t];
    const double base[3] = {bx, by, bz}, scale[3] = {sx, sy, sz};
    uint32_t q[24];
    for (int i = 0; i < 4; i++)
        for (int a = 0; a < 3; a++) {
            if ((uint32_t)i >= n) { q[4 * a + i] = 65535u; q[12 + 4 * a + i] = 0u; continue; }
            const double l = ((double)nd[4 * a + i] - base[a]) / scale[a], h = ((double)nd[12 + 4 * a + i] - base[a]) / scale[a];
            long long ql = (long long)floor(l) - 1, qh = (long long)ceil(h) + 1;
            ql = ql < 0 ? 0 : (ql > 65535 ? 65535 : ql); qh = qh < 0 ? 0 : (qh > 65535 ? 65535 : qh);
            q[4 * a + i] = (uint32_t)ql; q[12 + 4 * a + i] = (uint32_t)qh;
        }
    uint4 *o = nodes4q + 4 * (size_t)t;
    o[0] = uint4{q[0] | (q[1] << 16), q[2] | (q[3] << 16), q[4] | (q[5] << 16), q[6] | (q[7] << 16)};
    o[1] = uint4{q[8] | (q[9] << 16), q[10] | (q[11] << 16), q[12] | (q[13] << 16), q[14] | (q[15] << 16)};
    o[2] = uint4{q[16] | (q[17] << 16), q[18] | (q[19] << 16), q[20] | (q[21] << 16), q[22] | (q[23] << 16)};
}

inline unsigned blocks_of(size_t n) { return (unsigned)((n + 255u) / 256u); }

}

hipError_t refit_launch_pad(const unsigned char *raw, uint32_t n, uint32_t *out, hipStream_t s)
{
    hipError_t e = hipMemsetAsync(out, 0, 4, s);
    if (e != hipSuccess || n == 0) return e;
    hipLaunchKernelGGL(k_refit_pad, dim3(blocks_of(n)), dim3(256), 0, s, raw, n, out);
    return hipGetLastError();
}

hipError_t refit_launch_prims(const unsigned char *raw, uint32_t first, uint32_t count, const uint32_t *slot_of_index, float4 *prim,
                              float4 *primD, hipStream_t s)
{
    if (count == 0) return hipSuccess;
    hipLaunchKernelGGL(k_refit_prims, dim3(blocks_of(count)), dim3(256), 0, s, raw, first, count, slot_of_index, prim, primD);
    return hipGetLastError();
}

hipError_t refit_launch_transform(unsigned char *raw, const uint32_t *start, const crt_prim_transform *ops, uint32_t n_ops, uint32_t total,
                                  const uint32_t *slot_of_index, float4 *prim, float4 *primD, hipStream_t s)
{
    if (total == 0) return hipSuccess;
    hipLaunchKernelGGL(k_refit_transform, dim3(blocks_of(total)), dim3(256), 0, s, raw, start, ops, n_ops, total, slot_of_index, prim, primD);
    return hipGetLastError();
}

hipError_t refit_launch_compact(const unsigned char *src, unsigned char *dst, const uint32_t *tab, uint32_t n_gaps, uint32_t n_new, hipStream_t s)
{
    if (n_new == 0) return hipSuccess;
    hipLaunchKernelGGL(k_edit_compact, dim3(blocks_of((size_t)n_new * 5u)), dim3(256), 0, s, (const uint4 *)src, (uint4 *)dst, tab, tab + n_gaps,
                       n_gaps, n_new);
    return hipGetLastError();
}

hipError_t refit_levels(const void *nodes, uint32_t width, bool quantised, int root, uint32_t cap, int *list, uint32_t *counter,
                        uint32_t *nch, std::vector<uint32_t> &off, hipStream_t s)
{
    off.assign(1, 0u);
    if (root < 0 || cap == 0) return hipSuccess;
    const uint32_t stride = (width == 2 || quantised) ? 16u : 32u, ref_at = (width == 2 || quantised) ? 12u : 24u;
    hipError_t e = hipMemcpyAsync(list, &root, 4, hipMemcpyHostToDevice, s);
    uint32_t count = 1;
    while (e == hipSuccess && count) {
        const uint32_t base = off.back();
        off.push_back(base + count);
        if (off.size() > 130) return hipErrorUnknown;
        e = hipMemsetAsync(counter, 0, 4, s);
        if (e != hipSuccess) break;
        hipLaunchKernelGGL(k_refit_expand, dim3(blocks_of(count)), dim3(256), 0, s, (const uint32_t *)nodes, stride, ref_at, width,
                           list + base, count, list + base + count, cap - (base + count), counter, nch);
        e = hipGetLastError();
        uint32_t next = 0;
        if (e == hipSuccess) e = hipMemcpyAsync(&next, counter, 4, hipMemcpyDeviceToHost, s);
        if (e == hipSuccess) e = hipStreamSynchronize(s);
        if (e == hipSuccess && next > cap - (base + count)) return hipErrorUnknown;
        count = next;
    }
    return e;
}

hipError_t refit_launch_bvh2(const float4 *prim, float pad, const int *list, const std::vector<uint32_t> &off, float *nodes, hipStream_t s)
{
    for (size_t l = off.size() - 1; l-- > 0;) {
        const uint32_t count = off[l + 1] - off[l];
        hipLaunchKernelGGL(k_refit_bvh2, dim3(blocks_of(count)), dim3(256), 0, s, prim, pad, list + off[l], count, nodes);
        const hipError_t e = hipGetLastError();
        if (e != hipSuccess) return e;
    }
    return hipSuccess;
}

hipError_t refit_launch_wide(const float4 *prim, float pad, const int *list, const std::vector<uint32_t> &off, const void *refs,
                             bool quantised, const uint32_t *nch, float *fb, hipStream_t s)
{
    for (size_t l = off.size() - 1; l-- > 0;) {
        const uint32_t count = off[l + 1] - off[l];
        hipLaunchKernelGGL(k_refit_wide, dim3(blocks_of(count)), dim3(256), 0, s, prim, pad, list + off[l], count, (const uint32_t *)refs,
                           quantised ? 16u : 32u, quantised ? 12u : 24u, nch, fb);
        const hipError_t e = hipGetLastError();
        if (e != hipSuccess) return e;
    }
    return hipSuccess;
}

hipError_t refit_launch_quant4(const float *fb, const uint32_t *nch, uint32_t n4, uint4 *nodes4q, const double base[3], const double scale[3],
                               hipStream_t s)
{
    if (n4 == 0) return hipSuccess;
    hipLaunchKernelGGL(k_refit_quant4, dim3(blocks_of(n4)), dim3(256), 0, s, fb, nch, n4, nodes4q, base[0], base[1], base[2], scale[0],
                       scale[1], scale[2]);
    return hipGetLastError();
}

}
```

computeraytracer_amd/csrc/crt_scene.cpp:

```cpp
#include "crt_ctx.h"

using namespace crt;

namespace crt {

HostPrim read_prim(const uint8_t *base, size_t i)
{
    HostPrim p;
    const uint8_t *r = base + i * 80;
    float f[9];
    uint32_t u[4];
    std::memcpy(&p.category, r, 4);
    std::memcpy(f, r + 16, 12); std::memcpy(f + 3, r + 32, 12); std::memcpy(f + 6, r + 48, 12);
    std::memcpy(u, r + 64, 16);
    p.d1 = f3{f[0], f[1], f[2]}; p.d2 = f3{f[3], f[4], f[5]}; p.d3 = f3{f[6], f[7], f[8]};
    p.emission = u[0]; p.reflectance = u[1]; p.material = u[2]; p.index = u[3];
    return p;
}

static int prim_corners(const HostPrim &p, f3 out[4])
{
    if (p.category == 1u) {
        float r = abs_(p.d2.x);
        out[0] = f3{p.d1.x - r, p.d1.y - r, p.d1.z - r};
// ... 43 lines not shown
    float light_area = length(l.d2) * length(l.d3);
    out[0] = float4{l.d1.x, l.d1.y, l.d1.z, bits_f(l.emission)};
    out[1] = float4{l.d2.x, l.d2.y, l.d2.z, bits_f(l.index)};
    out[2] = float4{l.d3.x, l.d3.y, l.d3.z, 1.0f / light_area};
}

void camera_frame(const float cam[16], float out[12])
{
    f3 eye = f3{cam[0], cam[1], cam[2]}, lookat = f3{cam[4], cam[5], cam[6]}, up = f3{cam[8], cam[9], cam[10]};
    f3 w = normalize(eye - lookat);
    f3 u = normalize(cross(up, w));
    f3 v = cross(w, u);
    float aspect_ratio = cam[11] / cam[12];
    float viewport_height = 2.0f * tan_(cam[13] / 2.0f);
    float viewport_width = aspect_ratio * viewport_height;
    f3 horizontal = u * viewport_width;
    f3 vertical = v * viewport_height;
    f3 llc = ((eye - horizontal / 2.0f) - vertical / 2.0f) - w;
    out[0] = llc.x; out[1] = llc.y; out[2] = llc.z;
    out[3] = horizontal.x; out[4] = horizontal.y; out[5] = horizontal.z;
    out[6] = vertical.x; out[7] = vertical.y; out[8] = vertical.z;
    out[9] = eye.x; out[10] = eye.y; out[11] = eye.z;
}

static void ploc_abandoned_note(crt_ctx *c, const PlocInfo &info)
{
    if (info.abandoned == 1)
        (void)fail(c, CRT_OK, "crt_build_accel: the PLOC hierarchy is %u levels deep, more than the %u the walk's stacks allow; built the LBVH instead",
                   info.depth, c->ploc.max_depth);
    else
        (void)fail(c, CRT_OK, "crt_build_accel: the PLOC build had not finished after %u rounds (the limit); built the LBVH instead", info.rounds);
}

static int build_accel_on_device(crt_ctx *c, bool *done)
{
    *done = false;
    const uint32_t n = (uint32_t)c->prims.size();
    if (n < 2 || !c->quantize || c->wf_width != 4 || c->d_raw.n < (size_t)n * 80) return CRT_OK;
    HIPCHK(c, c->d_prim.alloc((size_t)n * 3));
    HIPCHK(c, c->d_primD.alloc(n));
    HIPCHK(c, c->d_slot_of_index.alloc(n));
    HIPCHK(c, c->d_nodes.alloc((size_t)(n - 1) * 4));
    HIPCHK(c, c->d_nodes4q.alloc((size_t)(n - 1) * 4));
    HIPCHK(c, c->d_nodes4.alloc(8));
    LbvhDeviceResult res;
    int builder = 1;
    if (c->want_builder == 2) {
        PlocInfo info;
        const hipError_t e = build_ploc_device(c->d_raw.p, n, c->sc.hit_pad, c->ploc, c->d_prim.p, c->d_primD.p, c->d_slot_of_index.p,
                                               (float *)c->d_nodes.p, c->d_nodes4q.p, res, info, c->stream);
        if (e != hipSuccess) return fail(c, e == hipErrorOutOfMemory ? CRT_ENOMEM : CRT_EDEVICE, "crt_build_accel: GPU PLOC build: %s", hipGetErrorString(e));
        if (info.abandoned) ploc_abandoned_note(c, info);
        else builder = 2;
    }
    if (builder == 1) {
        const hipError_t e = build_lbvh_device(c->d_raw.p, n, c->sc.hit_pad, c->d_prim.p, c->d_primD.p, c->d_slot_of_index.p,
                                               (float *)c->d_nodes.p, c->d_nodes4q.p, res, c->stream);
        if (e != hipSuccess) return fail(c, e == hipErrorOutOfMemory ? CRT_ENOMEM : CRT_EDEVICE, "crt_build_accel: GPU LBVH build: %s", hipGetErrorString(e));
    }
    if (!res.quantised) return CRT_OK;
    c->bvh = Bvh(); c->bvh4 = Bvh4(); c->bvh4q = Bvh4Q(); c->bvh8q = Bvh8Q();
    c->bvh.root = 0; c->bvh.n_inner = n - 1; c->bvh.n_leaves = n; c->bvh.max_depth = res.max_depth;
    c->bvh4.root = 0; c->bvh4.n_inner = res.n_nodes4; c->bvh4.max_depth = res.depth4;
    c->bvh4q.ok = true;
    for (int a = 0; a < 3; a++) { c->bvh4q.base[a] = res.qbase[a]; c->bvh4q.scale[a] = res.qscale[a]; c->sc.qbase[a] = res.qbase[a]; c->sc.qscale[a] = res.qscale[a]; }
    c->accel_builder = builder;
    c->sc.prim = c->d_prim.p; c->sc.primD = c->d_primD.p; c->sc.slot_of_index = c->d_slot_of_index.p;
    c->sc.nodes = c->d_nodes.p; c->sc.root = 0;
    c->sc.nodes4 = c->d_nodes4.p; c->sc.root4 = 0; c->sc.n_nodes4 = res.n_nodes4;
    c->sc.nodes4q = c->d_nodes4q.p;
    c->sc.nodes8q = nullptr; c->sc.root8 = -1;
    c->sc.nprim = n;
    c->sc.npatch = 0;
    for (const HostPrim &hp_ : c->prims) c->sc.npatch += hp_.category == 0u ? 1u : 0u;
    c->accel_mode = CRT_ACCEL_BVH2;
    *done = true;
    return CRT_OK;
}

static int upload_geometry(crt_ctx *c, int mode)
{
    const uint32_t n = (uint32_t)c->prims.size();
    const float pad = c->sc.hit_pad;
    if (mode == CRT_ACCEL_BVH2 && c->want_builder != 0) {
        bool done = false;
        int rc = build_accel_on_device(c, &done);
        if (rc || done) return rc;
    }
    CRT_TRY(refresh_prims(c));
    std::vector<uint32_t> order;
    c->bvh = Bvh();
    if (mode == CRT_ACCEL_BVH2 && n > 0) {
        float S = pad * 131072.0f;
        std::vector<float> lo((size_t)n * 3), hi((size_t)n * 3);
        f3 cs[4];
        for (uint32_t i = 0; i < n; i++) {
            const HostPrim &p = c->prims[i];
            int nc = prim_corners(p, cs);
            float l[3] = {cs[0].x, cs[0].y, cs[0].z}, h[3] = {cs[0].x, cs[0].y, cs[0].z};
            for (int k = 1; k < nc; k++) {
                l[0] = std::min(l[0], cs[k].x); l[1] = std::min(l[1], cs[k].y); l[2] = std::min(l[2], cs[k].z);
                h[0] = std::max(h[0], cs[k].x); h[1] = std::max(h[1], cs[k].y); h[2] = std::max(h[2], cs[k].z);
            }
            float g = 2.0f * pad;
            if (p.category == 0u) {
                double e1[3] = {p.d2.x, p.d2.y, p.d2.z}, e2[3] = {p.d3.x, p.d3.y, p.d3.z};
                double g11 = e1[0] * e1[0] + e1[1] * e1[1] + e1[2] * e1[2];
// ... 21 lines not shown
            }
            for (int a = 0; a < 3; a++) {
                if (!(l[a] == l[a]) || !(h[a] == h[a]) || std::isinf(l[a]) || std::isinf(h[a])) {
                    l[a] = -3.0e38f; h[a] = 3.0e38f;
                }
                lo[3 * i + a] = l[a] - g; hi[3 * i + a] = h[a] + g;
            }
        }
        c->accel_builder = 0;
        if (c->want_builder != 0 && n >= 2) {
            int builder = 1;
            if (c->want_builder == 2) {
                PlocInfo info;
                hipError_t e = build_ploc(lo.data(), hi.data(), n, c->ploc, c->bvh, info, c->stream);
                if (e != hipSuccess) return fail(c, e == hipErrorOutOfMemory ? CRT_ENOMEM : CRT_EDEVICE, "crt_build_accel: GPU PLOC build: %s", hipGetErrorString(e));
                if (info.abandoned) ploc_abandoned_note(c, info);
                else builder = 2;
            }
            if (builder == 1) {
                hipError_t e = build_lbvh(lo.data(), hi.data(), n, c->bvh, c->stream);
                if (e != hipSuccess) return fail(c, e == hipErrorOutOfMemory ? CRT_ENOMEM : CRT_EDEVICE, "crt_build_accel: GPU LBVH build: %s", hipGetErrorString(e));
            }
            c->accel_builder = builder;
        } else {
            build_bvh2(lo.data(), hi.data(), n, c->bvh);
        }
        order = c->bvh.order;
    } else {
        order.resize(n);
        for (uint32_t i = 0; i < n; i++) order[i] = i;
        c->bvh.root = -1;
    }

    std::vector<float4> hp((size_t)n * 3), hd(n);
    std::vector<uint32_t> slot_of(n);
    for (uint32_t slot = 0; slot < n; slot++) {
        const HostPrim &p = c->prims[order[slot]];
        slot_of[p.index] = slot;
        uint32_t meta = (p.category & 3u) | ((p.material & 3u) << 2) | ((p.emission & 0x3FFFu) << 4) |
                        ((p.reflectance & 0x3FFFu) << 18);
        float4 A = {p.d1.x, p.d1.y, p.d1.z, bits_f(meta)};
        float4 B = {p.d2.x, p.d2.y, p.d2.z, bits_f(p.index)};
        float4 C = {p.d3.x, p.d3.y, p.d3.z, 0.0f};
        float4 D = {0.0f, 0.0f, 0.0f, 0.0f};
        if (p.category == 0u) {
            f3 nrm = normalize(cross(p.d2, p.d3));
            D = float4{nrm.x, nrm.y, nrm.z, dot(p.d2, p.d2)};
            C.w = dot(p.d3, p.d3);
        } else if (p.category == 1u) {
            float r = p.d2.x;
            B = float4{r, r * r, 0.0f, bits_f(p.index)};
        }
        hp[3 * (size_t)slot + 0] = A; hp[3 * (size_t)slot + 1] = B; hp[3 * (size_t)slot + 2] = C;
        hd[slot] = D;
    }
    HIPCHK(c, c->d_prim.alloc(std::max<size_t>(hp.size(), 3)));
    HIPCHK(c, c->d_primD.alloc(std::max<size_t>(hd.size(), 1)));
    HIPCHK(c, c->d_slot_of_index.alloc(std::max<size_t>(n, 1)));
    if (n) {
        HIPCHK(c, hipMemcpy(c->d_prim.p, hp.data(), hp.size() * sizeof(float4), hipMemcpyHostToDevice));
        HIPCHK(c, hipMemcpy(c->d_primD.p, hd.data(), hd.size() * sizeof(float4), hipMemcpyHostToDevice));
        HIPCHK(c, hipMemcpy(c->d_slot_of_index.p, slot_of.data(), n * sizeof(uint32_t), hipMemcpyHostToDevice));
    }
    size_t nn = c->bvh.nodes.size() / 4;
    HIPCHK(c, c->d_nodes.alloc(std::max<size_t>(nn, 4)));
    if (nn) HIPCHK(c, hipMemcpy(c->d_nodes.p, c->bvh.nodes.data(), nn * sizeof(float4), hipMemcpyHostToDevice));
    c->sc.prim = c->d_prim.p;
    c->sc.primD = c->d_primD.p;
    c->sc.slot_of_index = c->d_slot_of_index.p;
    c->bvh4 = Bvh4();
    if (mode == CRT_ACCEL_BVH2 && n > 0) collapse_bvh4(c->bvh, c->bvh4);
    size_t nn4 = c->bvh4.nodes.size() / 4;
    HIPCHK(c, c->d_nodes4.alloc(std::max<size_t>(nn4, 8)));
    if (nn4) HIPCHK(c, hipMemcpy(c->d_nodes4.p, c->bvh4.nodes.data(), nn4 * sizeof(float4), hipMemcpyHostToDevice));
    c->sc.nodes4 = c->d_nodes4.p;
    c->sc.root4 = c->bvh4.root;
    c->sc.n_nodes4 = c->bvh4.n_inner;
    c->bvh4q = Bvh4Q();
    c->sc.nodes4q = nullptr;
    if (c->quantize && c->bvh4.n_inner) quantize_bvh4(c->bvh4, c->bvh4q);
    if (c->bvh4q.ok) {
        size_t nq = c->bvh4q.nodes.size() / 4;
        HIPCHK(c, c->d_nodes4q.alloc(nq));
        HIPCHK(c, hipMemcpy(c->d_nodes4q.p, c->bvh4q.nodes.data(), nq * sizeof(uint4), hipMemcpyHostToDevice));
        c->sc.nodes4q = c->d_nodes4q.p;
        for (int a = 0; a < 3; a++) { c->sc.qbase[a] = c->bvh4q.base[a]; c->sc.qscale[a] = c->bvh4q.scale[a]; }
    }
    c->bvh8q = Bvh8Q();
    c->sc.nodes8q = nullptr;
    c->sc.root8 = -1;
    if (c->quantize && c->wf_width == 8 && c->bvh4q.ok) build_bvh8q(c->bvh, c->bvh8q);
    if (c->bvh8q.ok) {
        const size_t nq = c->bvh8q.nodes.size() / 4;
        HIPCHK(c, c->d_nodes8q.alloc(nq));
        HIPCHK(c, hipMemcpy(c->d_nodes8q.p, c->bvh8q.nodes.data(), nq * sizeof(uint4), hipMemcpyHostToDevice));
        c->sc.nodes8q = c->d_nodes8q.p;
        c->sc.root8 = c->bvh8q.root;
        for (int a = 0; a < 3; a++) { c->sc.qbase[a] = c->bvh8q.base[a]; c->sc.qscale[a] = c->bvh8q.scale[a]; }
    }
    c->sc.nodes = c->d_nodes.p;
    c->sc.root = c->bvh.root;
    c->sc.nprim = n;
    c->sc.npatch = 0;
    for (const HostPrim &hp_ : c->prims) c->sc.npatch += hp_.category == 0u ? 1u : 0u;
    c->accel_mode = mode;
    return CRT_OK;
}

uint32_t wf_stack_need(const crt_ctx *c) { return (c->bvh8q.ok ? 7u : 3u) * c->wf_depth; }
uint32_t wf_stack_lds(const crt_ctx *c) { return (c->wf_trace_form == 2 && c->bvh4q.ok && !c->bvh8q.ok) ? (uint32_t)kWfStackLds2 : (uint32_t)kWfStackLds; }
uint32_t wf_overflow_levels(const crt_ctx *c)
{
    const uint32_t need = wf_stack_need(c), lds = wf_stack_lds(c);
    return std::max(kWfOverflowLevels, need > lds ? need - lds : 0u);
}

int build_tree(crt_ctx *c, int mode)
{
    c->rf_ready = false;
    c->q_built_ok = false;
    c->refits = 0;
    c->wf_depth = 0;
    int rc = upload_geometry(c, mode);
    if (rc == CRT_OK && mode == CRT_ACCEL_BVH2) {
        c->wf_depth = c->bvh8q.ok ? c->bvh8q.max_depth : c->bvh4.max_depth;
        const uint32_t lds_min = c->bvh4q.ok && !c->bvh8q.ok ? (uint32_t)kWfStackLds2 : (uint32_t)kWfStackLds;
        if (c->accel_builder != 0 && wf_stack_need(c) > lds_min + kWfOverflowMaxLevels) {
            const uint32_t depth = c->wf_depth, width = c->bvh8q.ok ? 8u : 4u;
            const int wanted = c->want_builder;
            const char *made = c->accel_builder == 2 ? "PLOC tree" : "LBVH";
            c->want_builder = 0; c->accel_mode = -1;
            rc = upload_geometry(c, mode);
            c->want_builder = wanted;
            if (rc == CRT_OK) {
                c->wf_depth = c->bvh8q.ok ? c->bvh8q.max_depth : c->bvh4.max_depth;
                (void)fail(c, CRT_OK, "crt_build_accel: the %u-wide %s is %u levels deep (its walk would need %u stack entries per lane, "
                                      "more than %u + %u); built with the host SAH builder instead (%u levels)",
                           width, made, depth, (width - 1u) * depth, lds_min, kWfOverflowMaxLevels, c->wf_depth);
            }
        }
    }
    if (rc == CRT_OK) { c->accel_stale = false; c->accel_topo = false; c->tree_pad = c->sc.hit_pad; }
    return rc;
}

}

// ... 58 lines not shown
    if (c->accel_topo) {
        *rebuilt = true;
        c->accel_mode = -1;
        CRT_TRY(build_tree(c, CRT_ACCEL_BVH2));
        return quality_as_built(c);
    }
    if (c->bvh8q.ok) {
        *rebuilt = true;
        c->accel_mode = -1;
        return build_tree(c, CRT_ACCEL_BVH2);
    }
    const float pad = c->sc.hit_pad;
    const uint32_t n2 = c->bvh.n_inner, n4 = c->bvh4.n_inner;
    if (n2 == 0 || c->sc.root < 0) { c->accel_stale = false; c->tree_pad = pad; return CRT_OK; }
    const bool quant = c->sc.nodes4q != nullptr && n4 > 0;
    const bool wide_float = n4 > 0 && c->bvh4.nodes.size() >= (size_t)n4 * kNode4Floats;
    const bool wide = quant || wide_float;
    const void *refs4 = quant ? (const void *)c->d_nodes4q.p : (const void *)c->d_nodes4.p;
    if (!c->rf_ready) {
        CRT_TRY(quality_as_built(c));
        HIPCHK(c, c->rf_cnt.alloc(1));
        HIPCHK(c, c->rf_lv2.alloc(n2));
        HIPCHK(c, refit_levels(c->d_nodes.p, 2, false, c->sc.root, n2, c->rf_lv2.p, c->rf_cnt.p, nullptr, c->rf_off2, c->stream));
        if (c->rf_off2.back() != n2) return fail(c, CRT_EDEVICE, "crt_refit_accel: the BVH2 has %u inner nodes, its levels list %u", n2, c->rf_off2.back());
        if (wide) {
            HIPCHK(c, c->rf_lv4.alloc(n4));
            HIPCHK(c, c->rf_nch4.alloc(n4));
            HIPCHK(c, refit_levels(refs4, 4, quant, 0, n4, c->rf_lv4.p, c->rf_cnt.p, c->rf_nch4.p, c->rf_off4, c->stream));
            if (c->rf_off4.back() != n4) return fail(c, CRT_EDEVICE, "crt_refit_accel: the 4-wide tree has %u nodes, its levels list %u", n4, c->rf_off4.back());
            if (!wide_float) HIPCHK(c, c->rf_fb.alloc((size_t)n4 * kNode4Floats));
        }
        c->rf_ready = true;
    }
    HIPCHK(c, refit_launch_bvh2(c->d_prim.p, pad, c->rf_lv2.p, c->rf_off2, (float *)c->d_nodes.p, c->stream));
    if (wide) {
        float *fb = wide_float ? (float *)c->d_nodes4.p : c->rf_fb.p;
        HIPCHK(c, refit_launch_wide(c->d_prim.p, pad, c->rf_lv4.p, c->rf_off4, refs4, quant, c->rf_nch4.p, fb, c->stream));
        if (quant) {
            float root[kNode4Floats];
            uint32_t k = 0;
            HIPCHK(c, hipMemcpyAsync(root, fb, sizeof root, hipMemcpyDeviceToHost, c->stream));
            HIPCHK(c, hipMemcpyAsync(&k, c->rf_nch4.p, 4, hipMemcpyDeviceToHost, c->stream));
            HIPCHK(c, hipStreamSynchronize(c->stream));
            float glo[3] = {FLT_MAX, FLT_MAX, FLT_MAX}, ghi[3] = {-FLT_MAX, -FLT_MAX, -FLT_MAX}, base[3], scale[3];
            bool ok = k > 0 && k <= 4;
            for (uint32_t i = 0; ok && i < k; i++)
                for (int a = 0; a < 3; a++) {
                    const float l = root[4 * a + i], h = root[12 + 4 * a + i];
                    if (!(l > -1.0e30f) || !(h < 1.0e30f)) ok = false;
                    glo[a] = std::min(glo[a], l); ghi[a] = std::max(ghi[a], h);
                }
            for (int a = 0; ok && a < 3; a++) {
                const float ext = std::max(ghi[a] - glo[a], 1.0e-3f);
                const float mag = std::max(std::fabs(glo[a]), std::fabs(ghi[a]));
                if (mag > 16.0f * ext) ok = false;
                base[a] = glo[a]; scale[a] = ext / 65533.0f;
            }
            if (!ok) {
                *rebuilt = true;
                c->accel_mode = -1;
                return build_tree(c, CRT_ACCEL_BVH2);
            }
            const double bd[3] = {base[0], base[1], base[2]}, sd[3] = {scale[0], scale[1], scale[2]};
            HIPCHK(c, refit_launch_quant4(fb, c->rf_nch4.p, n4, c->d_nodes4q.p, bd, sd, c->stream));
            for (int a = 0; a < 3; a++) { c->sc.qbase[a] = c->bvh4q.base[a] = base[a]; c->sc.qscale[a] = c->bvh4q.scale[a] = scale[a]; }
        }
    }
    HIPCHK(c, hipStreamSynchronize(c->stream));
    c->tree_pad = pad;
    c->accel_stale = false;
// ... 49 lines not shown
    HIPCHK(c, hipMemcpyAsync(&sb, scan_out, 4, hipMemcpyDeviceToHost, c->stream));
    HIPCHK(c, hipStreamSynchronize(c->stream));
    c->s_prims = bits_f(sb);
    c->sc.hit_pad = pad_of(c->s_prims, c->camera);
    if (c->accel_mode == CRT_ACCEL_BVH2) c->accel_stale = true;
    return edit_end(c);
}

int crt_update_primitives(crt_ctx *c, uint32_t first, uint32_t count, const void *records)
{
    if (!c) return CRT_EINVAL;
    if (!records && count) return fail(c, CRT_EINVAL, "crt_update_primitives: records is NULL");
    if (!c->have_scene) return fail(c, CRT_ESTATE, "crt_update_primitives: upload a scene first");
    const size_t n = c->prims.size();
    if ((uint64_t)first + count > n)
        return fail(c, CRT_EINVAL, "crt_update_primitives: range [%u, %llu) outside the scene's %zu primitives", first,
                    (unsigned long long)first + count, n);
    std::vector<HostPrim> np(count);
    for (uint32_t k = 0; k < count; k++) {
        const uint32_t i = first + k;
        const HostPrim p = np[k] = read_prim((const uint8_t *)records, k), &o = c->prims[i];
        if (p.index != i) return fail(c, CRT_EINVAL, "crt_update_primitives: record %u: index is %u, must equal the array position %u", k, p.index, i);
        if (p.category != o.category || p.material != o.material)
            return fail(c, CRT_EINVAL, "crt_update_primitives: primitive %u: category and material cannot change (a topology edit: crt_upload_scene)", i);
        if (p.emission >= c->sc.nspectra || p.reflectance >= c->sc.nspectra)
            return fail(c, CRT_EINVAL, "crt_update_primitives: primitive %u: spectrum index out of range", i);
    }
    CRT_TRY(quiesce(c, true));
    CRT_TRY(prims_edit_history(c));
    std::copy(np.begin(), np.end(), c->prims.begin() + first);
    if (count) {
        HIPCHK(c, hipMemcpyAsync(c->d_raw.p + (size_t)first * 80, records, (size_t)count * 80, hipMemcpyHostToDevice, c->stream));
        if (c->accel_mode >= 0 && !c->accel_topo)
            HIPCHK(c, refit_launch_prims(c->d_raw.p, first, count, c->d_slot_of_index.p, c->d_prim.p, c->d_primD.p, c->stream));
    }
    return prims_edit_end(c);
}

int crt_transform_primitives(crt_ctx *c, const crt_prim_transform *ops, uint32_t n_ops)
{
    if (!c) return CRT_EINVAL;
    if (!ops && n_ops) return fail(c, CRT_EINVAL, "crt_transform_primitives: ops is NULL");
    if (!c->have_scene) return fail(c, CRT_ESTATE, "crt_transform_primitives: upload a scene first");
    const size_t n = c->prims.size();
    std::vector<uint32_t> live;
    for (uint32_t k = 0; k < n_ops; k++) {
        const crt_prim_transform &o = ops[k];
        if ((uint64_t)o.first + o.count > n)
            return fail(c, CRT_EINVAL, "crt_transform_primitives: op %u: range [%u, %llu) outside the scene's %zu primitives", k, o.first,
                        (unsigned long long)o.first + o.count, n);
        bool finite = std::isfinite(o.radius_scale);
        for (int a = 0; a < 12; a++) finite = finite && std::isfinite(o.m[a]);
        if (!finite) return fail(c, CRT_EINVAL, "crt_transform_primitives: op %u: a non-finite matrix entry or radius_scale", k);
        if (o.count) live.push_back(k);
    }
    std::vector<uint32_t> by_first(live);
    std::sort(by_first.begin(), by_first.end(), [&](uint32_t a, uint32_t b) { return ops[a].first < ops[b].first; });
    for (size_t j = 1; j < by_first.size(); j++) {
        const crt_prim_transform &a = ops[by_first[j - 1]], &b = ops[by_first[j]];
        if (a.first + a.count > b.first)
            return fail(c, CRT_EINVAL, "crt_transform_primitives: ops %u and %u overlap: both move primitive %u", by_first[j - 1], by_first[j], b.first);
    }
    const size_t op_dw = sizeof(crt_prim_transform) / 4, head = (live.size() + 1 + op_dw - 1) / op_dw * op_dw;
    std::vector<uint32_t> tab(head + live.size() * op_dw, 0u);
    uint32_t total = 0;
    for (size_t j = 0; j < live.size(); j++) {
        tab[j] = total;
        total += ops[live[j]].count;
        std::memcpy(&tab[head + j * op_dw], &ops[live[j]], sizeof(crt_prim_transform));
    }
    tab[live.size()] = total;
    CRT_TRY(quiesce(c, true));
    if (total && c->xf_tab.n < tab.size()) HIPCHK(c, c->xf_tab.alloc(std::max(tab.size(), 2 * c->xf_tab.n)));
    CRT_TRY(prims_edit_history(c));
    if (total) {
        HIPCHK(c, hipMemcpyAsync(c->xf_tab.p, tab.data(), tab.size() * 4, hipMemcpyHostToDevice, c->stream));
        const bool built = c->accel_mode >= 0 && !c->accel_topo;
        HIPCHK(c, refit_launch_transform(c->d_raw.p, c->xf_tab.p, (const crt_prim_transform *)(c->xf_tab.p + head), (uint32_t)live.size(), total,
                                         c->d_slot_of_index.p, built ? c->d_prim.p : nullptr, built ? c->d_primD.p : nullptr, c->stream));
        c->prims_moved = true;
    }
    return prims_edit_end(c);
}


struct TopoEdit {
    std::vector<HostPrim> lights;
    bool lights_replaced = false;
    bool lights_changed = false;
    DevBuf<float4> d_lights;
    DevBuf<unsigned char> raw, snap;
    DevBuf<float4> prim, primD;
    DevBuf<uint32_t> slot, scan;
    std::vector<uint32_t> iota, tab;
    std::vector<float4> rows;
};

static int topo_lights(crt_ctx *c, const char *what, const void *lights, size_t nlight, TopoEdit &e)
{
    if (!lights) {
        if (nlight) return fail(c, CRT_EINVAL, "%s: lights is NULL with nlight = %zu (NULL, 0 keeps the light list)", what, nlight);
        e.lights = c->lights;
        return CRT_OK;
    }
    if (nlight < 1) return fail(c, CRT_EINVAL, "%s: at least one light record is required", what);
    e.lights.resize(nlight);
    for (size_t i = 0; i < nlight; i++) {
        e.lights[i] = read_prim((const uint8_t *)lights, i);
        if (e.lights[i].emission >= c->sc.nspectra) return fail(c, CRT_EINVAL, "%s: light %zu: emission index out of range", what, i);
    }
    e.lights_replaced = true;
    return CRT_OK;
}

static int topo_alloc(crt_ctx *c, TopoEdit &e, size_t n_new, size_t new_raw, size_t new_snap, bool records_change)
{
    if (new_raw) HIPCHK(c, e.raw.alloc(new_raw));
    if (new_snap) HIPCHK(c, e.snap.alloc(new_snap));
    if (e.lights_replaced) HIPCHK(c, e.d_lights.alloc(e.lights.size() * 3));
    if (records_change && c->accel_mode == CRT_ACCEL_NONE) {
        HIPCHK(c, e.prim.alloc(std::max<size_t>(n_new * 3, 3)));
        HIPCHK(c, e.primD.alloc(std::max<size_t>(n_new, 1)));
        HIPCHK(c, e.slot.alloc(std::max<size_t>(n_new, 1)));
    }
    HIPCHK(c, e.scan.alloc(1));
    return CRT_OK;
}

static int topo_commit(crt_ctx *c, TopoEdit &e, bool records_change)
{
    DevScene &S = c->sc;
    const uint32_t n = (uint32_t)c->prims.size();
    if (e.lights_replaced || e.lights_changed) {
        e.rows.resize(e.lights.size() * 3);
        for (size_t i = 0; i < e.lights.size(); i++) light_rows(e.lights[i], &e.rows[3 * i]);
        if (e.lights_replaced) {
            c->d_lights = std::move(e.d_lights);
            S.lights = c->d_lights.p;
            S.nlight = (uint32_t)e.lights.size();
            S.inv_nlight = 1.0f / (float)S.nlight;
            c->dn.drop();
        }
        c->lights.swap(e.lights);
        HIPCHK(c, hipMemcpyAsync(c->d_lights.p, e.rows.data(), e.rows.size() * sizeof(float4), hipMemcpyHostToDevice, c->stream));
    }
    if (records_change) {
        S.nf_last[0] = S.nf_last[1] = kNoHit;
        for (size_t i = n; i-- > 0 && S.nf_last[1] == kNoHit;)
            if (c->prims[i].category != 2u) (S.nf_last[0] == kNoHit ? S.nf_last[0] : S.nf_last[1]) = (uint32_t)i;
        if (c->accel_mode == CRT_ACCEL_NONE) {
            e.iota.resize(n);
            for (uint32_t i = 0; i < n; i++) e.iota[i] = i;
            HIPCHK(c, hipMemcpyAsync(e.slot.p, e.iota.data(), (size_t)n * 4, hipMemcpyHostToDevice, c->stream));
            HIPCHK(c, refit_launch_prims(c->d_raw.p, 0, n, e.slot.p, e.prim.p, e.primD.p, c->stream));
            c->d_prim = std::move(e.prim); c->d_primD = std::move(e.primD); c->d_slot_of_index = std::move(e.slot);
            S.prim = c->d_prim.p; S.primD = c->d_primD.p; S.slot_of_index = c->d_slot_of_index.p;
            S.nprim = n;
            S.npatch = 0;
            for (const HostPrim &p : c->prims) S.npatch += p.category == 0u ? 1u : 0u;
        }
        if (c->accel_mode == CRT_ACCEL_BVH2) c->accel_topo = true;
    }
    return prims_edit_end(c, e.scan.p);
}

int crt_remove_primitives(crt_ctx *c, const crt_prim_range *ranges, uint32_t n_ranges, const void *lights, size_t nlight)
{
    if (!c) return CRT_EINVAL;
    if (!ranges && n_ranges) return fail(c, CRT_EINVAL, "crt_remove_primitives: ranges is NULL");
    if (!c->have_scene) return fail(c, CRT_ESTATE, "crt_remove_primitives: upload a scene first");
    const size_t n = c->prims.size();
    std::vector<crt_prim_range> live;
    for (uint32_t k = 0; k < n_ranges; k++) {
        if ((uint64_t)ranges[k].first + ranges[k].count > n)
            return fail(c, CRT_EINVAL, "crt_remove_primitives: range %u: [%u, %llu) outside the scene's %zu primitives", k, ranges[k].first,
                        (unsigned long long)ranges[k].first + ranges[k].count, n);
        if (ranges[k].count) live.push_back(ranges[k]);
    }
    std::sort(live.begin(), live.end(), [](const crt_prim_range &a, const crt_prim_range &b) { return a.first < b.first; });
    for (size_t j = 1; j < live.size(); j++)
        if (live[j - 1].first + live[j - 1].count > live[j].first)
            return fail(c, CRT_EINVAL, "crt_remove_primitives: two ranges overlap: both remove primitive %u", live[j].first);
    const size_t m = live.size();
    TopoEdit e;
    e.tab.assign(2 * m + 1, 0u);
    uint32_t total = 0;
    for (size_t j = 0; j < m; j++) {
        e.tab[j] = live[j].first - total;
        total += live[j].count;
        e.tab[m + 1 + j] = total;
    }
    if (total && total == n)
// ... 173 lines not shown
```

computeraytracer_amd/csrc/crt_shade.h:

```cpp
#pragma once
#include "crt_device.h"
#include "crt_math.h"
#include "../../include/crt.h"

namespace crt {

#define CRT_PI 3.14159265359f
#define CRT_INFINITY 2139095040.0f
constexpr uint32_t kMaxDepthPath = 100;
constexpr uint32_t kGrid = 16;
constexpr uint32_t kDiffuse = 0, kLight = 1, kGlass = 2;

struct Rng { uint32_t x, y, z, w; };

__device__ __forceinline__ uint32_t tea(uint32_t v0, uint32_t v1)
{
    uint32_t s0 = 0;
#pragma unroll
    for (int n = 0; n < 16; n++) {
        s0 += 0x9e3779b9u;
        v0 += ((v1 << 4) + 0xa341316cu) ^ (v1 + s0) ^ ((v1 >> 5) + 0xc8013ea4u);
        v1 += ((v0 << 4) + 0xad90777du) ^ (v0 + s0) ^ ((v0 >> 5) + 0x7e95761eu);
    }
    return v0;
}

__device__ __forceinline__ float rnd(Rng &s)
{
    s.x = s.x * 1664525u + 1013904223u;
    s.y = s.y * 1664525u + 1013904223u;
    s.z = s.z * 1664525u + 1013904223u;
    s.w = s.w * 1664525u + 1013904223u;
    s.x += s.y * s.w; s.y += s.z * s.x; s.z += s.x * s.y; s.w += s.y * s.z;
    s.x ^= s.x >> 16; s.y ^= s.y >> 16; s.z ^= s.z >> 16; s.w ^= s.w >> 16;
    s.x += s.y * s.w; s.y += s.z * s.x; s.z += s.x * s.y; s.w += s.y * s.z;
// ... 96 lines not shown
    t = dot(e2, qvec) * inv;
    const f3 p = ray_at(o, d, t);
    const f3 v1 = v0 + e1, v2 = v0 + e2;
    const f3 lo = f3{min_(v0.x, min_(v1.x, v2.x)) - hit_pad, min_(v0.y, min_(v1.y, v2.y)) - hit_pad, min_(v0.z, min_(v1.z, v2.z)) - hit_pad};
    const f3 hi = f3{max_(v0.x, max_(v1.x, v2.x)) + hit_pad, max_(v0.y, max_(v1.y, v2.y)) + hit_pad, max_(v0.z, max_(v1.z, v2.z)) + hit_pad};
    const bool in = (p.x >= lo.x) & (p.x <= hi.x) & (p.y >= lo.y) & (p.y <= hi.y) & (p.z >= lo.z) & (p.z <= hi.z);
    const bool wins = beats_flat(t, t_min, t_max, index, b_index, b_slot);
    return (exclude != index) & (det != 0.0f) & (u >= 0.0f) & (u <= 1.0f) & (v >= 0.0f) & ((u + v) <= 1.0f) & wins & in;
}

__device__ __forceinline__ bool patch_accepts_flat(const float4 A, const float4 B, const float4 C, const float4 D, f3 o, f3 d,
                                                   uint32_t exclude, float t_min, float t_max, uint32_t b_index, uint32_t b_slot, float &t)
{
    const uint32_t index = f_bits(B.w);
    f3 n = xyz(D);
    float ndotd = dot(n, d);
    const bool flip = ndotd > 0.0f;
    n = f3{flip ? -n.x : n.x, flip ? -n.y : n.y, flip ? -n.z : n.z};
    ndotd = flip ? -ndotd : ndotd;
    const f3 P0 = xyz(A);
    t = dot(n, P0 - o) / ndotd;
    const f3 m = ray_at(o, d, t) - P0;
    const float u = dot(m, xyz(B)) / D.w;
    const float v = dot(m, xyz(C)) / C.w;
    const bool grazing = abs_(ndotd) < 0.0001f;
    const bool wins = beats_flat(t, t_min, t_max, index, b_index, b_slot);
    return (exclude != index) & !grazing & wins & !((u < 0.0f) | (u > 1.0f) | (v < 0.0f) | (v > 1.0f));
}

template <bool LITERAL>
__device__ __forceinline__ bool hit_test(const DevScene &S, uint32_t slot, f3 o, f3 d, uint32_t exclude,
                                         float t_min, float &t_max, uint32_t &b_index, uint32_t &b_slot)
{
    const float4 A = S.prim[3 * slot + 0];
    const float4 B = S.prim[3 * slot + 1];
    const float4 C = S.prim[3 * slot + 2];
    float4 D = float4{0.0f, 0.0f, 0.0f, 0.0f};
    if (exclude != f_bits(B.w) && (f_bits(A.w) & 3u) == 0u) D = S.primD[slot];
    return hit_test_rec<LITERAL>(A, B, C, D, S.hit_pad, slot, o, d, exclude, t_min, t_max, b_index, b_slot);
}

__device__ __forceinline__ void hit_attributes_rec(const float4 A, const float4 B, const float4 C, const float4 D, f3 o, f3 d,
                                                   float t, f3 &pos, f3 &nrm, uint32_t &meta)
{
    meta = f_bits(A.w);
    const uint32_t cat = meta & 3u;
    pos = ray_at(o, d, t);
    if (cat == 1u) {
        nrm = normalize(pos - xyz(A));
    } else {
        f3 n;
        if (cat == 0u) n = xyz(D);
        else n = normalize(cross(xyz(B), xyz(C)));
        nrm = (dot(n, d) > 0.0f) ? -n : n;
    }
}

__device__ __forceinline__ void hit_attributes(const DevScene &S, uint32_t slot, f3 o, f3 d, float t,
                                               f3 &pos, f3 &nrm, uint32_t &meta)
{
    const float4 A = S.prim[3 * slot + 0];
    const uint32_t cat = f_bits(A.w) & 3u;
    float4 B = float4{0.0f, 0.0f, 0.0f, 0.0f}, C = B, D = B;
    if (cat == 0u) D = S.primD[slot];
    else if (cat == 2u) { B = S.prim[3 * slot + 1]; C = S.prim[3 * slot + 2]; }
    hit_attributes_rec(A, B, C, D, o, d, t, pos, nrm, meta);
}

__device__ __noinline__ void intersect_all(const DevScene &S, f3 o, f3 d, uint32_t exclude, float &t_max,
                                           uint32_t &b_index, uint32_t &b_slot, uint32_t &c_prims)
{
    for (uint32_t i = 0; i < S.nprim; i++)
        hit_test<true>(S, S.slot_of_index[i], o, d, exclude, 0.001f, t_max, b_index, b_slot);
    c_prims += S.nprim;
}

__device__ __forceinline__ bool finite3(f3 v)
{
    return abs_(v.x) < 3.0e38f && abs_(v.y) < 3.0e38f && abs_(v.z) < 3.0e38f;
}

template <bool COUNT>
__device__ __forceinline__ void traverse(const DevScene &S, int *stk, f3 o, f3 d, uint32_t exclude,
                                         bool anyhit, float &t_max, uint32_t &b_index, uint32_t &b_slot,
                                         uint32_t &c_nodes, uint32_t &c_prims)
{
    const float t_min = 0.001f;
    if (S.nprim == 0u) return;
    const float tiny = 1.0e-20f;
    f3 id;
    id.x = 1.0f / (abs_(d.x) > tiny ? d.x : __builtin_copysignf(tiny, d.x));
    id.y = 1.0f / (abs_(d.y) > tiny ? d.y : __builtin_copysignf(tiny, d.y));
    id.z = 1.0f / (abs_(d.z) > tiny ? d.z : __builtin_copysignf(tiny, d.z));
    const f3 oid = f3{o.x * id.x, o.y * id.y, o.z * id.z};
    const uint32_t b_slot_in = b_slot;
    int sp = 0;
    int node = S.root;
    for (;;) {
// ... 296 lines not shown
```

computeraytracer_amd/csrc/crt_wavefront.hip:

```cpp
#include "crt_shade.h"
#include "crt_tile_class.h"
#include "crt_launch.h"
#include <algorithm>

namespace crt {

#ifndef CRT_WF_STACK
#define CRT_WF_STACK 32
#endif
#ifndef CRT_WF_REFILL
#define CRT_WF_REFILL 24
#endif
#ifndef CRT_WF_INNER_RUN
#define CRT_WF_INNER_RUN 6
#endif
#ifndef CRT_WF_BURSTS
#define CRT_WF_BURSTS 4
#endif
#ifndef CRT_WF_BVH4
#define CRT_WF_BVH4 1
#endif
#ifndef CRT_WF_LEAF_AT
#define CRT_WF_LEAF_AT 32
#endif
#ifndef CRT_WF_SPEC
#define CRT_WF_SPEC 1
#endif
#ifndef CRT_WF_PATCH_RECOMPUTE
#define CRT_WF_PATCH_RECOMPUTE 20
#endif
#ifndef CRT_WF_SHADE_BLOCK
#define CRT_WF_SHADE_BLOCK 64
#endif
#ifndef CRT_WF_SHADE_MIN_WAVES
#define CRT_WF_SHADE_MIN_WAVES 1
#endif
#ifndef CRT_WF_MIN_WAVES
#define CRT_WF_MIN_WAVES 1
#endif
static_assert(kTcGrid == kGrid && kTcNLambda == kNLambda && kTcNCie == kNCie, "crt_tile_class.h restates these");
constexpr int kWfStack = CRT_WF_STACK;
static_assert(kWfStack == kWfStackLds, "crt_scene.cpp sizes the overflow area from kWfStackLds");
constexpr int kNoNode = 0x7FFFFFFF;
constexpr int kTraceChunk = 128;
constexpr int kRefillAt = CRT_WF_REFILL;

__device__ __forceinline__ uint32_t lane_id() { return threadIdx.x & 63u; }

#ifndef CRT_WF_NT
#define CRT_WF_NT 1
#endif
typedef float v4f __attribute__((ext_vector_type(4)));
typedef float v2f __attribute__((ext_vector_type(2)));
typedef uint32_t v4u __attribute__((ext_vector_type(4)));
#if CRT_WF_NT
__device__ __forceinline__ float4 ldnt(const float4 *p) { const v4f v = __builtin_nontemporal_load((const v4f *)p); return float4{v.x, v.y, v.z, v.w}; }
__device__ __forceinline__ uint4 ldnt(const uint4 *p) { const v4u v = __builtin_nontemporal_load((const v4u *)p); return uint4{v.x, v.y, v.z, v.w}; }
__device__ __forceinline__ float2 ldnt(const float2 *p) { const v2f v = __builtin_nontemporal_load((const v2f *)p); return float2{v.x, v.y}; }
__device__ __forceinline__ uint32_t ldnt(const uint32_t *p) { return __builtin_nontemporal_load(p); }
__device__ __forceinline__ void stnt(float4 *p, float4 v) { __builtin_nontemporal_store(v4f{v.x, v.y, v.z, v.w}, (v4f *)p); }
__device__ __forceinline__ void stnt(uint4 *p, uint4 v) { __builtin_nontemporal_store(v4u{v.x, v.y, v.z, v.w}, (v4u *)p); }
__device__ __forceinline__ void stnt(float2 *p, float2 v) { __builtin_nontemporal_store(v2f{v.x, v.y}, (v2f *)p); }
__device__ __forceinline__ void stnt(uint32_t *p, uint32_t v) { __builtin_nontemporal_store(v, p); }
typedef uint32_t v2u __attribute__((ext_vector_type(2)));
__device__ __forceinline__ void stnt(uint2 *p, uint2 v) { __builtin_nontemporal_store(v2u{v.x, v.y}, (v2u *)p); }
#else
template <class T> __device__ __forceinline__ T ldnt(const T *p) { return *p; }
template <class T> __device__ __forceinline__ void stnt(T *p, T v) { *p = v; }
#endif
__device__ __forceinline__ uint32_t prefix_popc(unsigned long long mask, uint32_t lane)
{
    return (uint32_t)__popcll(mask & ((1ull << lane) - 1ull));
}

__device__ __noinline__ float2 resolve_nonfinite(const float4 *prim, const float4 *primD, const uint32_t *slot_of_index,
                                                 uint32_t nprim, float hit_pad, float ox, float oy, float oz, float dx,
                                                 float dy, float dz, uint32_t exclude)
{
    DevScene S{};
    S.prim = prim; S.primD = primD; S.slot_of_index = slot_of_index; S.nprim = nprim; S.hit_pad = hit_pad;
    float tm = CRT_INFINITY;
    uint32_t bi = kNoHit, bs = kNoHit;
    const f3 o = f3{ox, oy, oz}, d = f3{dx, dy, dz};
    for (uint32_t i = 0; i < nprim; i++) hit_test<true>(S, slot_of_index[i], o, d, exclude, 0.001f, tm, bi, bs);
    return float2{tm, bits_f(bs)};
}

struct CamRay { f3 eye, d; Rng rng; uint32_t lambda; bool nan_ray; };
__device__ __forceinline__ CamRay camera_ray(const DevScene &S, uint32_t px, uint32_t py, uint32_t sample, uint32_t seed)
{
    CamRay c;
    c.rng = Rng{py, px * 100u, sample, seed};
    const float jx = rnd(c.rng);
    const float fs = ((float)px + ((float)(sample % kGrid) + jx) / (float)kGrid) / (float)S.W;
    const float jy = rnd(c.rng);
    const float ft = ((float)S.H - (float)py + ((float)(sample % kGrid) + jy) / (float)kGrid) / (float)S.H;
    const f3 llc = f3{S.cam[0], S.cam[1], S.cam[2]}, hor = f3{S.cam[3], S.cam[4], S.cam[5]};
    const f3 ver = f3{S.cam[6], S.cam[7], S.cam[8]};
    c.eye = f3{S.cam[9], S.cam[10], S.cam[11]};
    c.d = normalize(((llc + hor * fs) + ver * ft) - c.eye);
    const float ul = rnd(c.rng);
    c.lambda = (uint32_t)(301.0f * ul);
    c.nan_ray = !finite3(c.eye) || !finite3(c.d);
    return c;
}

__device__ __forceinline__ void work_pixel(const WfParams &P, uint32_t work, uint32_t &px, uint32_t &py)
{
    const uint32_t pp = work % P.npix_padded;
    const uint32_t tile = pp >> 6, l = pp & 63u;
    const uint32_t lx = (tile % P.tiles_x) * 8u + (l & 7u), ly = (tile / P.tiles_x) * 8u + (l >> 3);
    px = P.x0 + lx;
    py = P.y0 + (ly / P.band) * P.band * P.stride + P.phase * P.band + ly % P.band;
}

struct PathRegs {
    f3 ray_o, ray_d;
    f4 beta, radiance;
    Rng rng;
    float last_pdf, etaScale;
    uint32_t exclude, work, flags;
};

__device__ __forceinline__ void wavelengths_of(uint32_t lambda, uint32_t wl[4])
{
    wl[0] = lambda; wl[1] = (lambda + 4u) % kNLambda; wl[2] = (lambda + 8u) % kNLambda;
    wl[3] = (lambda + 12u) % kNLambda;
}

struct LightRec { float4 L0, L1, L2, A, B, C, D; uint32_t slot; float pdf_area; };

template <bool UNIFORM>
__device__ __forceinline__ LightRec load_light(const DevScene &S, uint32_t li)
{
    LightRec r;
    r.A = float4{0.0f, 0.0f, 0.0f, 0.0f}; r.B = r.A; r.C = r.A; r.D = r.A; r.slot = kNoHit; r.pdf_area = 0.0f;
    if (UNIFORM) {
        typedef const __attribute__((address_space(4))) v4f *cptr4;
        typedef const __attribute__((address_space(4))) uint32_t *cptr1;
        auto ld = [](cptr4 p) { const v4f v = *p; return float4{v.x, v.y, v.z, v.w}; };
        const cptr4 lg = (cptr4)S.lights;
        r.L0 = ld(lg); r.L1 = ld(lg + 1); r.L2 = ld(lg + 2);
        const uint32_t include = f_bits(r.L1.w);
        if (include < S.nprim) {
            r.slot = ((cptr1)S.slot_of_index)[include];
            const cptr4 pg = (cptr4)S.prim + 3 * (size_t)r.slot;
            r.A = ld(pg); r.B = ld(pg + 1); r.C = ld(pg + 2); r.D = ld((cptr4)S.primD + r.slot);
            r.pdf_area = r.L2.w;
        }
    } else {
        r.L0 = S.lights[3 * li + 0]; r.L1 = S.lights[3 * li + 1]; r.L2 = S.lights[3 * li + 2];
        const uint32_t include = f_bits(r.L1.w);
        if (include < S.nprim) {
            r.slot = S.slot_of_index[include];
            r.A = S.prim[3 * (size_t)r.slot + 0]; r.B = S.prim[3 * (size_t)r.slot + 1]; r.C = S.prim[3 * (size_t)r.slot + 2];
            r.D = S.primD[r.slot];
            uint32_t l2 = (f_bits(r.A.w) >> 4) & 0x3FFFu;
            if (l2 >= S.nlight) l2 = S.nlight - 1u;
            r.pdf_area = S.lights[3 * l2 + 2].w;
        }
    }
    return r;
}

__device__ __forceinline__ f4 nee_term(const DevScene &S, const LightRec &L, f3 pos, f3 ldir, float t_l, float cos_theta,
                                       const f4 spec)
{
    f3 lp, ln; uint32_t lmeta;
    hit_attributes_rec(L.A, L.B, L.C, L.D, pos, ldir, t_l, lp, ln, lmeta);
    f4 le = spec * cos_theta;
    float pdf_l = compute_light_pdf_area(L.pdf_area, S.inv_nlight, lp, ln, pos, ldir);
    float pdf_b = cos_theta / CRT_PI;
    float weight_l = power_heuristic(1.0f, pdf_l, 1.0f, pdf_b);
    return (le * weight_l) / pdf_l;
}

struct ShadeCnt { uint32_t rays = 0, bounces = 0, shadow = 0, hits = 0, paths = 0, prims = 0, walk = 0; };
struct ShadowOut { bool emit; f3 d; float t_l; uint32_t l_index, l_slot; f4 c; };

template <bool COUNT, bool FINISH>
__device__ __forceinline__ ShadowOut light_sample(const WfParams &P, const LightRec &L, uint32_t slot, f3 pos, f3 nrm, uint32_t b_index,
                                                  float u, float v2, f4 brdf, f4 beta, f4 &radiance, bool &rad_dirty, const uint32_t wl[4], ShadeCnt &cn)
{
    const DevScene &S = P.sc;
    ShadowOut out{false, f3{0.0f, 0.0f, 0.0f}, 0.0f, 0u, 0u, f4{0.0f, 0.0f, 0.0f, 0.0f}};
    f3 pl = (xyz(L.L0) + xyz(L.L1) * u) + xyz(L.L2) * v2;
    f3 ldir = normalize(pl - pos);
    const uint32_t include = f_bits(L.L1.w);
    if (COUNT) { cn.rays++; cn.shadow++; }
// ... 56 lines not shown
    PathRegs R;
    R.flags = 0;
    LightRec LU{};
    if (S.nlight == 1u) LU = load_light<true>(S, 0u);
    uint4 misc = uint4{0, 0, 0, 0}, rs = uint4{0, 0, 0, 0};
    float4 v_ro = float4{0, 0, 0, 0}, v_rd = v_ro, v_beta = v_ro, v_rad = v_ro, v_nee = v_ro;
    float2 h = float2{0.0f, 0.0f};
    uint32_t vis_in = 0, dflag = 0;
    if (in_pool) {
        misc = ldnt(&P.misc[slot]); v_ro = ldnt(&P.ray_o[slot]); v_rd = ldnt(&P.ray_d[slot]); v_beta = ldnt(&P.beta[slot]);
        v_rad = ldnt(&P.radiance[slot]); rs = ldnt(&P.rng[slot]); h = ldnt(&P.hit[slot]); vis_in = ldnt(&P.vis[slot]);
#ifndef CRT_WHATIF_NO_NEE
        v_nee = ldnt(&P.nee[slot]);
#endif
        if (!FINISH) dflag = P.dflag[slot];
    }
    CRT_PROBE(tp, 1)
    if (!FINISH && (dflag & kWfDeferred)) {
        if (vis_in == 1u) stnt(&P.staging[dflag & (kWfRing - 1u)][f_bits(v_nee.w)], float4{v_nee.x, v_nee.y, v_nee.z, 0.0f});
        P.dflag[slot] = (uint8_t)0;
    }
    R.work = misc.x; R.flags = misc.y; R.last_pdf = bits_f(misc.z); R.etaScale = bits_f(misc.w);
    bool alive = in_pool && (R.flags & kWfAlive);
    bool emit_ext = false, emit_sh = false;
    bool sh_primary = false;
    bool finished = false, rad_dirty = false, deferred = false;
    f4 sh_c = f4{0.0f, 0.0f, 0.0f, 0.0f};
    f3 out_sd = f3{0, 0, 0}; float out_tl = 0.0f; uint32_t out_lindex = 0, out_lslot = 0;
    const bool nan_ray = alive && (R.flags & kWfNanRay) != 0u;
    if (nan_ray) R.flags &= ~kWfNanRay;
    const uint32_t h_slot = f_bits(h.y);
    const bool has_hit = alive && !nan_ray && !(R.flags & kWfDying) && h_slot != kNoHit;
    float4 hA = float4{0, 0, 0, 0}, hB = hA, hC = hA, hD = hA;
    if (has_hit) { hA = S.prim[3 * (size_t)h_slot + 0]; hB = S.prim[3 * (size_t)h_slot + 1]; hC = S.prim[3 * (size_t)h_slot + 2]; if (S.npatch) hD = S.primD[h_slot]; }
    CRT_PROBE(tp, 2)

    if (alive) {
        if (R.flags & kWfFresh) {
            uint32_t px, py;
            work_pixel(P, R.work, px, py);
            const CamRay c = camera_ray(S, px, py, misc.z, misc.w);
            v_ro = float4{c.eye.x, c.eye.y, c.eye.z, bits_f(0xFFFFFFFFu)};
            v_rd = float4{c.d.x, c.d.y, c.d.z, 0.0f};
            v_beta = float4{1.0f, 1.0f, 1.0f, 1.0f};
            rs = uint4{c.rng.x, c.rng.y, c.rng.z, c.rng.w};
            R.last_pdf = 1.0f; R.etaScale = 1.0f;
            R.flags &= ~kWfFresh;
        }
        R.ray_o = xyz(v_ro); R.exclude = f_bits(v_ro.w);
        R.ray_d = xyz(v_rd);
        R.beta = f4{v_beta.x, v_beta.y, v_beta.z, v_beta.w};
        R.rng = Rng{rs.x, rs.y, rs.z, rs.w};
        R.radiance = (R.flags & kWfHasRad) ? f4{v_rad.x, v_rad.y, v_rad.z, v_rad.w} : f4{0.0f, 0.0f, 0.0f, 0.0f};
        uint32_t wl[4];
        wavelengths_of((R.flags >> kWfLambdaShift) & 0x1FFu, wl);
        uint32_t depth = (R.flags >> kWfDepthShift) & 0xFFu;

        if (R.flags & kWfShadow) {
            if (vis_in == 1u) { R.radiance = R.radiance + f4{v_nee.x, v_nee.y, v_nee.z, v_nee.w}; rad_dirty = true; }
            R.flags &= ~kWfShadow;
        }
        if (R.flags & kWfDying) {
            finished = true;
        } else if (nan_ray) {
            emit_ext = true;
        } else {
            const uint32_t b_slot = h_slot;
// ... 115 lines not shown
            const size_t cell = (size_t)sample_off * ((size_t)P.tw * P.th) + (size_t)ly * P.tw + lx;
            stnt(&P.staging[(R.flags >> kWfBatchShift) & (kWfRing - 1u)][cell], float4{c.x, c.y, c.z, 0.0f});
            if (!FINISH && deferred) {
                const f3 c1 = spectral_to_xyz(S, R.radiance + sh_c, wl);
                stnt(&P.nee[slot], float4{c1.x, c1.y, c1.z, bits_f((uint32_t)cell)});
                P.dflag[slot] = (uint8_t)(kWfDeferred | ((R.flags >> kWfBatchShift) & (kWfRing - 1u)));
            }
            alive = false;
            if (COUNT) cn.paths++;
        }
    }

    CRT_PROBE(tp, 3)
    const uint32_t batch = (R.flags >> kWfBatchShift) & (kWfRing - 1u);
    if (!alive) R.flags = 0;
    ShadeOut so;
    so.deferred = deferred;
    so.alive = alive; so.emit_ext = emit_ext; so.emit_sh = emit_sh; so.sh_primary = sh_primary; so.rad_dirty = rad_dirty;
    so.batch = batch;
    so.R = R; so.sd = out_sd; so.t_l = out_tl; so.l_index = out_lindex; so.l_slot = out_lslot;
    return so;
}

template <bool COUNT, bool FINISH>
__device__ __forceinline__ uint32_t shade_store(const WfParams &P, uint32_t slot, bool in_pool, ShadeOut &so, ShadeCnt &cn)
{
    const DevScene &S = P.sc;
    PathRegs &R = so.R;
    uint32_t resolved = 0u;
    if (in_pool) {
        if (so.alive) {
            stnt(&P.ray_o[slot], float4{R.ray_o.x, R.ray_o.y, R.ray_o.z, bits_f(R.exclude)});
            if (so.emit_ext && (!finite3(R.ray_o) || !finite3(R.ray_d))) {
                P.hit[slot] = resolve_nonfinite(S.prim, S.primD, S.slot_of_index, S.nprim, S.hit_pad, R.ray_o.x, R.ray_o.y, R.ray_o.z,
                                                R.ray_d.x, R.ray_d.y, R.ray_d.z, R.exclude);
                if (COUNT) cn.prims += S.nprim;
                resolved = 1u;
            }
            stnt(&P.ray_d[slot], float4{R.ray_d.x, R.ray_d.y, R.ray_d.z, bits_f(resolved)});
            if (so.rad_dirty || (FINISH && !(R.flags & kWfHasRad))) {
                stnt(&P.radiance[slot], float4{R.radiance.x, R.radiance.y, R.radiance.z, R.radiance.w});
                R.flags |= kWfHasRad;
            }
            stnt(&P.rng[slot], uint4{R.rng.x, R.rng.y, R.rng.z, R.rng.w});
#ifdef CRT_WHATIF_EXTRA_STREAM
            if (!FINISH) { const float4 x = ldnt(&P.sh_d[slot]); stnt(&P.sh_d[slot], float4{x.y, x.x, x.w, x.z}); }
#endif
            stnt(&P.beta[slot], float4{R.beta.x, R.beta.y, R.beta.z, R.beta.w});
        }
        stnt(&P.misc[slot], so.alive ? uint4{R.work, R.flags, f_bits(R.last_pdf), f_bits(R.etaScale)} : uint4{0u, 0u, 0u, 0u});
    }
    return resolved;
}

__device__ __noinline__ void write_status(const WfCtl *ctl, const WfWorkQ *wq, uint32_t it_end, WfStatus *out)
{
    const uint32_t lane = lane_id();
    const WfShard &sh = ctl->shard[(it_end - 1u) & 3u][lane];
    const uint32_t mine = sh.n[0] + sh.n[1] + sh.n[2] + sh.n[3];
    unsigned long long rays = mine;
    uint32_t bound = mine;
    for (int off = 32; off > 0; off >>= 1) {
        rays += __shfl_xor(rays, off, 64);
        bound = max(bound, (uint32_t)__shfl_xor((int)bound, off, 64));
    }
    if (lane == 0) { out->dropped = ctl->dropped; out->bound = bound; out->pad_ = 0; out->rays = rays; }
#pragma unroll 1
// ... 617 lines not shown
            }
        }
        if (__ballot(active) == 0ull) {
            if (exhausted) break;
            continue;
        }

#pragma unroll 1
        for (int pass = 0; pass < 64; pass++) {
#if CRT_WF_SPEC
            if (active && node < 0 && pend == 0 && sp > 0) {
                pend = node;
                sp--; node = stack_pop(stk, ovf, ovl, sp);
            }
#endif
            const bool inner = active && node >= 0 && node != kNoNode;
            const bool leaf = active && (node < 0 || pend != 0);
            const int ni = __popcll(__ballot(inner)), nl = __popcll(__ballot(leaf)), nb = __popcll(__ballot(inner || leaf));
            if (nb == 0) break;
            if (!exhausted && 64 - nb >= kRefillAt && pass > 0) break;
            if (nl >= CRT_WF_LEAF_AT || ni == 0) {
                if (COUNT) {
                    d_leaf_it++; d_leaf_act += (uint32_t)nl;
                    uint32_t mc = leaf ? ((~(uint32_t)(pend != 0 ? pend : node)) & 7u) + 1u : 0u;
                    for (int off = 32; off > 0; off >>= 1) mc = max(mc, (uint32_t)__shfl_xor((int)mc, off, 64));
                    d_prim_it += mc;
                }
                if (leaf) {
                    const bool from_pend = pend != 0;
                    const uint32_t enc = ~(uint32_t)(from_pend ? pend : node);
                    const uint32_t first = enc >> 3, cnt = (enc & 7u) + 1u;
                    for (uint32_t i = 0; i < cnt; i++) {
                        const uint32_t ps = first + i;
                        const float4 A = prim[3 * (size_t)ps + 0], B = prim[3 * (size_t)ps + 1], C = prim[3 * (size_t)ps + 2];
                        if ((f_bits(A.w) & 3u) == 2u) tri_test(A, B, C, ps, o, d, excl, t_min, hit_pad, t_max, b_index, b_slot);
                        else hit_test<false>(S, ps, o, d, excl, t_min, t_max, b_index, b_slot);
                    }
                    if (COUNT) c_prims += cnt;
                    if (from_pend) pend = 0;
                    else if (sp > 0) { sp--; node = stack_pop(stk, ovf, ovl, sp); }
                    else node = kNoNode;
                    bool done = false;
                    if (shadow && b_slot != b_slot_in) done = true;
                    else if (node == kNoNode && pend == 0) done = true;
                    if (done) {
                        if (shadow) stnt(&g_vis[slot], (b_slot == b_slot_in) ? 1u : 0u);
                        else stnt(&g_hit[slot], float2{t_max, bits_f(b_slot)});
                        active = false;
                    }
                }
            } else {
                if (COUNT) { d_inner_it++; d_inner_act += (uint32_t)ni; }
                if (inner && QUANT == 2) {
                    const uint4 *nq = nodesq + 8 * (size_t)node;
                    const uint4 LX = nq[0], LY = nq[1], LZ = nq[2], HX = nq[3], HY = nq[4], HZ = nq[5], RA = nq[6], RB = nq[7];
                    const bool gx = nx != 0, gy = ny != 0, gz = nz != 0;
                    const uint4 NX = gx ? HX : LX, FX = gx ? LX : HX;
                    const uint4 NY = gy ? HY : LY, FY = gy ? LY : HY;
                    const uint4 NZ = gz ? HZ : LZ, FZ = gz ? LZ : HZ;
                    float k0, k1, k2, k3, k4, k5, k6, k7;
#define CRT_QBOX8(K, C, LOHI) { \
                        const float tn_ = __builtin_fmaxf(__builtin_fmaxf(fma_((float)(LOHI(NX.C)), id.x, oid.x), fma_((float)(LOHI(NY.C)), id.y, oid.y)), \
                                                          __builtin_fmaxf(fma_((float)(LOHI(NZ.C)), id.z, oid.z), t_min)); \
                        const float tf_ = __builtin_fminf(__builtin_fminf(fma_((float)(LOHI(FX.C)), id.x, oid.x), fma_((float)(LOHI(FY.C)), id.y, oid.y)), \
                                                          __builtin_fminf(fma_((float)(LOHI(FZ.C)), id.z, oid.z), t_max)); \
                        K = (tn_ <= tf_ * 1.0000005f) ? tn_ : 3.0e38f; }
#define CRT_LO16(v) ((v) & 0xFFFFu)
// ... 201 lines not shown
    return ((unsigned long long)f_bits(t) << 32) | (unsigned long long)(index == kNoHit ? 0xFFFFFFFFu : 0xFFFFFFFEu - index);
}

#ifndef CRT_WF_T2_WAVES
#define CRT_WF_T2_WAVES 5
#endif
template <bool COUNT>
__global__ __launch_bounds__(64, CRT_WF_T2_WAVES) void k_wf_trace2(const WfParams P, uint32_t it)
{
    __shared__ int lds_stack[kStk2 * 64];
    __shared__ float4 ring[4][kRing2];
    __shared__ uint2 ring_l[kRing2];
    __shared__ unsigned long long cell[64];
#if !CRT_WF_T2_LATE_SLOT
    __shared__ uint32_t cslot[64];
#endif
    __shared__ uint2 tasks[64];
    WfCtl *ctl = P.ctl;
    const uint4 *__restrict__ nodesq = P.sc.nodes4q;
    const f3 qscale = f3{P.sc.qscale[0], P.sc.qscale[1], P.sc.qscale[2]}, qbase = f3{P.sc.qbase[0], P.sc.qbase[1], P.sc.qbase[2]};
    const float4 *__restrict__ prim = P.sc.prim;
    const float4 *__restrict__ primD = P.sc.primD;
    uint32_t *__restrict__ g_vis = P.vis;
    float2 *__restrict__ g_hit = P.hit;
    const size_t cls_stride = (size_t)P.list_cap * kWfShards;
    const float4 *__restrict__ recA = P.recA + (size_t)((it & 1u) * 4u) * cls_stride;
    const float4 *__restrict__ recB = P.recB + (size_t)((it & 1u) * 4u) * cls_stride;
    const uint4 *__restrict__ recC = P.recC + (size_t)((it & 1u) * 4u) * cls_stride;
    const float hit_pad = P.sc.hit_pad;
    const int root = P.sc.root4;
    int *__restrict__ ovf = P.stack_overflow + ((size_t)blockIdx.x * 64 + lane_id());
    const size_t ovl = P.overflow_lanes;
    const uint32_t nprim = P.sc.nprim;
    const bool fetchD = ((unsigned long long)P.sc.npatch << CRT_WF_PATCH_RECOMPUTE) > (unsigned long long)nprim;
    DevScene S = P.sc;
    S.prim = prim; S.primD = primD;

    const uint32_t ringi = it & 3u;
    const uint32_t lane = lane_id();
    int *stk = lds_stack + lane;
    const float t_min = 0.001f;

    const uint32_t home = wf_home_shard(P);
    uint32_t cur_shard = home, sh_e0 = 0, sh_e1 = 0, sh_e2 = 0, sh_total = 0;
    uint32_t chunk_pos = 0, chunk_end = 0, ring_head = 0, ring_n = 0;
    bool have_shard = false, exhausted = false;
    {
        const WfShard &so = ctl->shard[ringi][cur_shard];
        sh_e0 = so.n[0]; sh_e1 = sh_e0 + so.n[1]; sh_e2 = sh_e1 + so.n[2]; sh_total = sh_e2 + so.n[3];
        have_shard = sh_total > 0u;
    }
    bool active = false;
    int pend = 0;
    f3 o = f3{0, 0, 0}, d = f3{0, 0, 0}, id = f3{0, 0, 0}, oid = f3{0, 0, 0};
    uint32_t excl = 0, slot = 0, b_index = kNoHit;
    uint32_t b_in = kNoHit;
#if !CRT_WF_T2_LATE_SLOT
    uint32_t b_slot = kNoHit;
#endif
    float t_max = 0.0f;
    bool shadow = false;
    int node = kNoNode, sp = 0;
    bool gx = false, gy = false, gz = false;
    uint32_t c_nodes = 0, c_prims = 0;
    uint32_t d_inner_it = 0, d_inner_act = 0, d_leaf_it = 0, d_leaf_act = 0, d_prim_it = 0, d_refill = 0, d_refill_lanes = 0, d_scans = 0;
    uint32_t d_max_sp = 0;
    auto ray_out = [&]() {
// ... 117 lines not shown
        for (int pass = 0; pass < 64; pass++) {
            if (active && node < 0 && pend == 0 && sp > 0) {
                pend = node;
                sp--; node = stack_pop2(stk, ovf, ovl, sp);
            }
            const bool inner = active && node >= 0 && node != kNoNode;
            const bool leaf = active && (node < 0 || pend != 0);
            const int ni = __popcll(__ballot(inner)), nl = __popcll(__ballot(leaf)), nb = __popcll(__ballot(active));
            if (nb == 0) break;
            if (pass > 0 && 64 - nb >= CRT_WF_PICK_AT && (ring_n > 0u || !exhausted)) break;
            if (nl >= CRT_WF_LEAF2_AT || ni == 0 || nb - ni >= CRT_WF_STALL_AT) {
                const int lf = pend != 0 ? pend : node;
                const uint32_t cnt = leaf ? ((~(uint32_t)lf) & 7u) + 1u : 0u;
                const unsigned long long c0 = __ballot((cnt & 1u) != 0u), c1 = __ballot((cnt & 2u) != 0u), c2 = __ballot((cnt & 4u) != 0u), c3 = __ballot((cnt & 8u) != 0u);
                const uint32_t pre = mbcnt64(c0) + 2u * mbcnt64(c1) + 4u * mbcnt64(c2) + 8u * mbcnt64(c3);
                const bool incl = leaf && pre + cnt <= 64u;
                const unsigned long long mi = __ballot(incl);
                const uint32_t T = (uint32_t)(__popcll(c0 & mi) + 2 * __popcll(c1 & mi) + 4 * __popcll(c2 & mi) + 8 * __popcll(c3 & mi));
                const uint32_t first = (~(uint32_t)lf) >> 3;
                if (incl) {
                    tasks[pre] = uint2{first, lane};
                    if (cnt > 1u) tasks[pre + 1u] = uint2{first + 1u, lane};
                    if (cnt > 2u) tasks[pre + 2u] = uint2{first + 2u, lane};
                    if (cnt > 3u) tasks[pre + 3u] = uint2{first + 3u, lane};
                    for (uint32_t i = 4; i < cnt; i++) tasks[pre + i] = uint2{first + i, lane};
                }
                __builtin_amdgcn_fence(__ATOMIC_RELEASE, "wavefront");
                __builtin_amdgcn_wave_barrier();
                if (COUNT) { d_leaf_it++; d_leaf_act += T; d_prim_it += 1u; }
                const uint2 tk = lane < T ? tasks[lane] : uint2{0u, lane};
                const int owner = (int)tk.y;
                const uint32_t ps = tk.x;
                float4 A = float4{0, 0, 0, 0}, B = A, C = A, D = A;
                if (lane < T) { A = prim[3 * (size_t)ps + 0]; B = prim[3 * (size_t)ps + 1]; C = prim[3 * (size_t)ps + 2]; if (fetchD) D = primD[ps]; }
                bool from_pend = false;
                if (incl) {
                    from_pend = pend != 0;
                    if (from_pend) pend = 0;
                    else if (sp > 0) { sp--; node = stack_pop2(stk, ovf, ovl, sp); }
                    else node = kNoNode;
                }
                const f3 to = f3{__shfl(o.x, owner, 64), __shfl(o.y, owner, 64), __shfl(o.z, owner, 64)};
                const f3 td = f3{__shfl(d.x, owner, 64), __shfl(d.y, owner, 64), __shfl(d.z, owner, 64)};
                const uint32_t t_excl = (uint32_t)__shfl((int)excl, owner, 64);
                bool acc = false;
                unsigned long long key = 0;
                if (lane < T) {
                    const unsigned long long cur = cell[owner];
                    float tm = bits_f((uint32_t)(cur >> 32));
                    const uint32_t low = (uint32_t)cur;
                    uint32_t bi = low == 0xFFFFFFFFu ? kNoHit : 0xFFFFFFFEu - low;
                    const uint32_t bs0 = low == 0xFFFFFFFFu ? kNoHit : 0xFFFFFFFEu;
                    uint32_t bs = bs0;
#if CRT_WF_T2_FLAT
                    const uint32_t cat = f_bits(A.w) & 3u;
                    bool ok;
                    float t = tm;
                    if (!fetchD && cat == 0u) { const f3 nn = normalize(cross(xyz(B), xyz(C))); D = float4{nn.x, nn.y, nn.z, dot(xyz(B), xyz(B))}; }
                    if (cat == 2u) {
                        ok = tri_accepts_flat(A, B, C, hit_pad, to, td, t_excl, t_min, tm, bi, bs, t);
                    } else if (cat == 0u && CRT_WF_T2_FLAT != 2) {
                        ok = patch_accepts_flat(A, B, C, D, to, td, t_excl, t_min, tm, bi, bs, t);
                    } else {
                        uint32_t si = bi, ss = bs;
                        ok = hit_test_rec<false>(A, B, C, D, hit_pad, ps, to, td, t_excl, t_min, t, si, ss);
                    }
                    tm = ok ? t : tm; bi = ok ? f_bits(B.w) : bi; bs = ok ? ps : bs;
// ... 423 lines not shown
```

computeraytracer_amd/renderer.py:

```python
from __future__ import annotations

import ctypes as C

import numpy as np

from . import _lib
from ._lib import ACCEL_BVH2, ACCEL_LBVH, ACCEL_NONE, ACCEL_PLOC, CNT, CrtError, NCOUNTERS
from .scene import PackedScene

_ACCEL = {"none": ACCEL_NONE, "brute": ACCEL_NONE, "bvh2": ACCEL_BVH2, "bvh": ACCEL_BVH2, "lbvh": ACCEL_LBVH, ACCEL_LBVH: ACCEL_LBVH,
          "ploc": ACCEL_PLOC, ACCEL_PLOC: ACCEL_PLOC, ACCEL_NONE: ACCEL_NONE, ACCEL_BVH2: ACCEL_BVH2}
AOV_PLANES = ("hits", "alpha", "depth", "normal", "albedo")
MATTE_PLANES = ("ids", "counts", "hits", "overflow")
MATTE_SOURCES = {"primitive": 0, "object": 1, "material": 2}
MATTE_NONE = 0xFFFFFFFF


def spectrum_rgb(spectrum, cie) -> np.ndarray:
    s = np.ascontiguousarray(spectrum, np.float32)
    c = np.ascontiguousarray(cie, np.float32)
    if s.size != 301 or c.size != 3 * 471:
        raise ValueError("spectrum must be 301 floats, cie 3 x 471")
    out = np.empty(3, np.float32)
    rc = _lib.load().crt_spectrum_rgb(s.ctypes.data, c.ctypes.data, out.ctypes.data)
# ... 513 lines not shown
        self._chk(self._lib.crt_comm_info(self._h, out))
        return dict(rank=out[0], world=out[1], transport={0: "rccl", 1: "local"}.get(out[2]), rows=out[3])

    def comm_destroy(self):
        self._chk(self._lib.crt_comm_destroy(self._h))
        return self

    def enable_counters(self, on: bool = True):
        self._chk(self._lib.crt_enable_counters(self._h, 1 if on else 0))
        return self

    def reset_counters(self):
        self._chk(self._lib.crt_reset_counters(self._h))
        return self

    def counters(self) -> dict:
        out = np.zeros(NCOUNTERS, np.uint64)
        self._chk(self._lib.crt_counters(self._h, out.ctypes.data))
        return {k: int(out[i]) for k, i in CNT.items()}

    def last_trace_ms(self):
        ms, n = C.c_float(), C.c_uint32()
        self._chk(self._lib.crt_last_trace_ms(self._h, C.byref(ms), C.byref(n)))
        return ms.value, n.value

    def last_kernel_ms(self):
        ms, n = C.c_float(), C.c_uint32()
        self._chk(self._lib.crt_last_kernel_ms(self._h, C.byref(ms), C.byref(n)))
        return ms.value, n.value

    def accel_stats(self) -> dict:
        out = np.zeros(8, np.uint64)
        self._chk(self._lib.crt_accel_stats(self._h, out.ctypes.data))
        return dict(nodes=int(out[0]), leaves=int(out[1]), max_depth=int(out[2]), bytes=int(out[3]),
                    bytes_per_box=int(out[4]), width=int(out[5]), wide_nodes=int(out[6]),
                    builder=("sah-host", "lbvh-gpu", "ploc-gpu")[int(out[7])])

    def debug_intersect(self, origins, directions, exclude=None) -> np.ndarray:
        o = np.asarray(origins, np.float32).reshape(-1, 3)
        d = np.asarray(directions, np.float32).reshape(-1, 3)
        n = o.shape[0]
        rays = np.zeros((n, 8), np.float32)
        rays[:, 0:3] = o
        rays[:, 3:6] = d
        ex = np.full(n, 0xFFFFFFFF, np.uint32) if exclude is None else np.asarray(exclude, np.uint32)
        rays[:, 6] = ex.view(np.float32)
        out = np.zeros((n, 8), np.float32)
        self._chk(self._lib.crt_debug_intersect(self._h, rays.ctypes.data, n, out.ctypes.data))
        return out

    TRACE_KERNELS = ("k_wf_trace<,0>", "k_wf_trace<,1>", "k_wf_trace<,2>", "k_wf_trace2")

    def debug_trace_rays(self, origins, directions, exclude=None, shadow=None, t_light=None, light=None):
        o = np.asarray(origins, np.float32).reshape(-1, 3)
        d = np.asarray(directions, np.float32).reshape(-1, 3)
        n = o.shape[0]
        rays = np.zeros((n, 12), np.float32)
        rays[:, 0:3] = o
        rays[:, 3:6] = d
        ru = rays.view(np.uint32)
        ru[:, 6] = 0xFFFFFFFF if exclude is None else np.asarray(exclude, np.uint32)
        sh = np.zeros(n, bool) if shadow is None else np.asarray(shadow, bool)
        if sh.any():
            ru[:, 7] = sh
            rays[sh, 8] = np.asarray(t_light, np.float32)[sh]
            ru[sh, 9] = np.asarray(light, np.uint32)[sh]
        out = np.zeros((n, 2), np.uint32)
        rep = np.zeros(8, np.uint64)
        self._chk(self._lib.crt_debug_trace_rays(self._h, rays.ctypes.data, n, out.ctypes.data, rep.ctypes.data))
# ... 96 lines not shown
```

include/crt.h:

```cpp
#ifndef CRT_H
#define CRT_H

#include <stddef.h>
#include <stdint.h>

#ifdef __cplusplus
extern "C" {
#endif

#define CRT_ABI_VERSION 2

enum {
    CRT_OK = 0,
    CRT_EINVAL = -1,
    CRT_EDEVICE = -2,
    CRT_ESTATE = -3,
    CRT_ENOMEM = -4
};

enum {
    CRT_ACCEL_NONE = 0,
    CRT_ACCEL_BVH2 = 1,
    CRT_ACCEL_LBVH = 2,
    CRT_ACCEL_PLOC = 3
// ... 167 lines not shown
                         float *history_out);
int crt_denoise_temporal_reset(crt_ctx *ctx);
int crt_read_motion(crt_ctx *ctx, float *out);

typedef struct {
    uint32_t iterations;
    float sigma_variance;
    float sigma_normal;
    float sigma_plane;
    float max_history;
    float normal_tol;
    float plane_tol;
    float min_frames;
} crt_denoise_svgf_params;
int crt_denoise_svgf_defaults(crt_denoise_svgf_params *out);
int crt_denoise_svgf(crt_ctx *ctx, const crt_denoise_svgf_params *params, float *rgb_out, uint8_t *rgba8_out,
                     float *history_out, float *var_out);
int crt_debug_read_moments(crt_ctx *ctx, float *out);

int crt_debug_read_clip_box(crt_ctx *ctx, float *out );

int crt_enable_counters(crt_ctx *ctx, int on);
int crt_counters(crt_ctx *ctx, uint64_t out[CRT_NCOUNTERS]);
int crt_reset_counters(crt_ctx *ctx);

int crt_last_trace_ms(crt_ctx *ctx, float *ms, uint32_t *launches);

int crt_last_kernel_ms(crt_ctx *ctx, float *ms, uint32_t *launches);

int crt_set_option(crt_ctx *ctx, const char *name, int64_t value);

int crt_accel_stats(crt_ctx *ctx, uint64_t out[8]);

int crt_debug_intersect(crt_ctx *ctx, const float *rays, size_t n, float *out);
int crt_debug_trace_rays(crt_ctx *ctx, const float *rays, size_t n, uint32_t *out, uint64_t report[8]);
int crt_debug_walk_rays(crt_ctx *ctx, int walk, const float *rays, size_t n, uint32_t *out, uint64_t report[8]);
int crt_debug_math(crt_ctx *ctx, int fn, const float *a, const float *b, float *out, size_t n);
enum {
    CRT_ACCEL_PART_HEADER = 0, CRT_ACCEL_PART_NODES2 = 1, CRT_ACCEL_PART_NODES4 = 2, CRT_ACCEL_PART_NODES4Q = 3,
    CRT_ACCEL_PART_NODES8Q = 4, CRT_ACCEL_PART_PRIM = 5, CRT_ACCEL_PART_PRIMD = 6, CRT_ACCEL_PART_SLOT_OF_INDEX = 7
};
#define CRT_ACCEL_HEADER_N 32
int crt_debug_read_accel(crt_ctx *ctx, int what, void *out, size_t capacity, size_t *bytes);
int crt_debug_probes(crt_ctx *ctx, uint64_t out[8]);
int crt_debug_gen_culled(crt_ctx *ctx, uint64_t *out);
int crt_debug_deferred_nee(crt_ctx *ctx, uint64_t *out);
int crt_debug_tile_classes(crt_ctx *ctx, uint8_t *out, size_t n_tiles);
int crt_debug_tile_classes_host(crt_ctx *ctx, uint8_t *out, size_t n_tiles);
int crt_debug_tile_class_setups(crt_ctx *ctx, uint64_t *out);
int crt_debug_mapped_gen_launches(crt_ctx *ctx, uint64_t *out);

#ifdef __cplusplus
}
#endif
#endif
```

Measured before the change: 8154 Mrays/s.

## Interleave patch D quad into 64-byte primitive records when patches are common

```diff
diff --git a/computeraytracer_amd/_lib.py b/computeraytracer_amd/_lib.py
--- a/computeraytracer_amd/_lib.py
+++ b/computeraytracer_amd/_lib.py
@@ -43,6 +43,7 @@
     "crt_last_kernel_ms": (C.c_int, [_P, _P, _P]),
     "crt_set_option": (C.c_int, [_P, C.c_char_p, C.c_int64]),
     "crt_accel_stats": (C.c_int, [_P, _P]),
+    "crt_prim_record_quads": (C.c_int, [_P, _P]),
     "crt_get_device": (C.c_int, [_P, _P]),
     "crt_get_stream": (C.c_int, [_P, C.POINTER(_P)]),
     "crt_image_size": (C.c_int, [_P, _P]),
diff --git a/computeraytracer_amd/csrc/crt_api.cpp b/computeraytracer_amd/csrc/crt_api.cpp
--- a/computeraytracer_amd/csrc/crt_api.cpp
+++ b/computeraytracer_amd/csrc/crt_api.cpp
@@ -238,6 +238,7 @@
     for (size_t i = c->prims.size(); i-- > 0 && S.nf_last[1] == kNoHit;)
         if (c->prims[i].category != 2u) (S.nf_last[0] == kNoHit ? S.nf_last[0] : S.nf_last[1]) = (uint32_t)i;
     camera_frame(c->camera, S.cam);
+    choose_prim_layout(c);
 
     HIPCHK(c, c->d_raw.alloc(std::max<size_t>(nprim * 80, 16)));
     if (nprim) HIPCHK(c, hipMemcpy(c->d_raw.p, primitives, nprim * 80, hipMemcpyHostToDevice));
@@ -301,6 +302,7 @@
     CRT_TRY(quiesce(c, true));
     c->accel_mode = -1;
     c->dn.valid = false; c->fdn.valid = false;
+    choose_prim_layout(c);
     return build_tree(c, mode);
 }
 
@@ -818,6 +820,14 @@
     return CRT_OK;
 }
 
+int crt_prim_record_quads(crt_ctx *c, uint32_t *quads)
+{
+    if (!c || !quads) return CRT_EINVAL;
+    if (!c->have_scene) return fail(c, CRT_ESTATE, "crt_prim_record_quads: upload a scene first");
+    *quads = c->sc.prim_quads;
+    return CRT_OK;
+}
+
 int crt_set_option(crt_ctx *c, const char *name, int64_t value)
 {
     if (!c || !name) return CRT_EINVAL;
@@ -899,6 +909,11 @@
     if (!std::strcmp(name, "wf_cull_miss")) { c->wf_cull_miss = value != 0; return CRT_OK; }
     if (!std::strcmp(name, "wf_cull_classes")) { c->wf_cull_classes = value != 0; return CRT_OK; }
     if (!std::strcmp(name, "wf_defer_nee")) { c->wf_defer_nee = value != 0; return CRT_OK; }
+    if (!std::strcmp(name, "prim_record")) {
+        if (!prim_record_option_valid((int)value) || value != (int)value) return fail(c, CRT_EINVAL, "crt_set_option: prim_record is 0 (the rule), 48 or 64");
+        c->prim_record = (int)value;
+        return CRT_OK;
+    }
     if (!std::strcmp(name, "wf_affinity")) { c->wf_affinity = value != 0; return CRT_OK; }
     if (!std::strcmp(name, "wf_pipes")) { c->wf_pipes = (int)std::min<int64_t>(crt_ctx::kMaxPipes, std::max<int64_t>(1, value)); return CRT_OK; }
     if (!std::strcmp(name, "wf_pool")) { c->wf_pool = (uint32_t)std::max<int64_t>(0, value); return CRT_OK; }
diff --git a/computeraytracer_amd/csrc/crt_ctx.h b/computeraytracer_amd/csrc/crt_ctx.h
--- a/computeraytracer_amd/csrc/crt_ctx.h
+++ b/computeraytracer_amd/csrc/crt_ctx.h
@@ -18,6 +18,7 @@
 #include "crt_device.h"
 #include "crt_launch.h"
 #include "crt_math.h"
+#include "crt_prim_layout.h"
 #include "crt_tile_class.h"
 #include "crt_wf_policy.h"
 
@@ -181,6 +182,7 @@
     int wf_cull_miss = 1;
     int wf_cull_classes = 1;
     int wf_defer_nee = 1;
+    int prim_record = 0;
     int wf_affinity = 0;
     uint64_t mapped_gen_launches = 0;
     uint64_t tile_cls_setups = 0;
@@ -354,6 +356,8 @@
 void light_rows(const HostPrim &l, float4 out[3]);
 void camera_frame(const float cam[16], float out[12]);
 int build_tree(crt_ctx *c, int mode);
+void choose_prim_layout(crt_ctx *c);
+inline crt::PrimRecords prim_records(const crt_ctx *c) { return crt::PrimRecords{c->d_prim.p, c->d_primD.p, c->sc.prim_quads}; }
 uint32_t wf_stack_need(const crt_ctx *c);
 uint32_t wf_stack_lds(const crt_ctx *c);
 uint32_t wf_overflow_levels(const crt_ctx *c);
diff --git a/computeraytracer_amd/csrc/crt_debug.cpp b/computeraytracer_amd/csrc/crt_debug.cpp
--- a/computeraytracer_amd/csrc/crt_debug.cpp
+++ b/computeraytracer_amd/csrc/crt_debug.cpp
@@ -222,6 +222,11 @@
     if (!out) return CRT_OK;
     if (capacity < need) return fail(c, CRT_EINVAL, "crt_debug_read_accel: part %d holds %zu bytes, the buffer %zu", what, need, capacity);
     if (what == CRT_ACCEL_PART_HEADER) std::memcpy(out, hdr, need);
+    else if (need && c->sc.prim_quads == 4u && (what == CRT_ACCEL_PART_PRIM || what == CRT_ACCEL_PART_PRIMD)) {
+        const size_t w = what == CRT_ACCEL_PART_PRIM ? 3 * sizeof(float4) : sizeof(float4);
+        const float4 *from = c->d_prim.p + (what == CRT_ACCEL_PART_PRIM ? 0 : 3);
+        HIPCHK(c, hipMemcpy2D(out, w, from, 4 * sizeof(float4), w, n, hipMemcpyDeviceToHost));
+    }
     else if (need) HIPCHK(c, hipMemcpy(out, src, need, hipMemcpyDeviceToHost));
     return CRT_OK;
 }
diff --git a/computeraytracer_amd/csrc/crt_device.h b/computeraytracer_amd/csrc/crt_device.h
--- a/computeraytracer_amd/csrc/crt_device.h
+++ b/computeraytracer_amd/csrc/crt_device.h
@@ -26,6 +26,7 @@
     const float4 *lights;
     uint32_t nprim;
     uint32_t npatch;
+    uint32_t prim_quads;
     int32_t root;
     int32_t root4;
     int32_t root8;
@@ -39,6 +40,8 @@
     float qbase[3], qscale[3];
     float cam[12];
 };
+
+struct PrimRecords { float4 *prim, *primD; uint32_t quads; };
 
 struct TraceParams {
     DevScene sc;
diff --git a/computeraytracer_amd/csrc/crt_launch.h b/computeraytracer_amd/csrc/crt_launch.h
--- a/computeraytracer_amd/csrc/crt_launch.h
+++ b/computeraytracer_amd/csrc/crt_launch.h
@@ -35,32 +35,32 @@
 hipError_t as_launch_commit(uint32_t *counts, const uint32_t *active, uint32_t n_active, uint32_t samples, hipStream_t s);
 
 hipError_t build_lbvh(const float *lo, const float *hi, uint32_t n, Bvh &out, hipStream_t stream);
-hipError_t build_lbvh_device(const unsigned char *d_raw, uint32_t n, float hit_pad, float4 *d_prim, float4 *d_primD,
+hipError_t build_lbvh_device(const unsigned char *d_raw, uint32_t n, float hit_pad, PrimRecords recs,
                              uint32_t *d_slot_of_index, float *d_nodes2, uint4 *d_nodes4q, LbvhDeviceResult &res, hipStream_t stream);
 template <typename T> struct DevBuf;
 hipError_t lbvh_sorted_keys_host(const float *lo, const float *hi, uint32_t n, float *d_lo, float *d_hi, unsigned long long *d_keys,
                                  unsigned long long *d_sorted, DevBuf<char> &sort_tmp, hipStream_t stream);
 hipError_t lbvh_sorted_keys_device(const unsigned char *d_raw, uint32_t n, float hit_pad, float *d_lo, float *d_hi, uint32_t *d_cbox,
                                    unsigned long long *d_keys, unsigned long long *d_sorted, DevBuf<char> &sort_tmp, hipStream_t stream);
-hipError_t lbvh_launch_gather(const unsigned char *d_raw, const unsigned long long *d_keys, uint32_t n, float4 *d_prim, float4 *d_primD,
+hipError_t lbvh_launch_gather(const unsigned char *d_raw, const unsigned long long *d_keys, uint32_t n, PrimRecords recs,
                               uint32_t *d_slot_of_index, hipStream_t stream);
 hipError_t lbvh_collapse_device(const float *d_nodes2, uint32_t n, uint4 *d_nodes4q, LbvhDeviceResult &res, hipStream_t stream);
 
 hipError_t build_ploc(const float *lo, const float *hi, uint32_t n, const PlocOptions &opt, Bvh &out, PlocInfo &info, hipStream_t stream);
-hipError_t build_ploc_device(const unsigned char *d_raw, uint32_t n, float hit_pad, const PlocOptions &opt, float4 *d_prim, float4 *d_primD,
+hipError_t build_ploc_device(const unsigned char *d_raw, uint32_t n, float hit_pad, const PlocOptions &opt, PrimRecords recs,
                              uint32_t *d_slot_of_index, float *d_nodes2, uint4 *d_nodes4q, LbvhDeviceResult &res, PlocInfo &info,
                              hipStream_t stream);
 
 hipError_t refit_launch_pad(const unsigned char *raw, uint32_t n, uint32_t *out, hipStream_t s);
-hipError_t refit_launch_prims(const unsigned char *raw, uint32_t first, uint32_t count, const uint32_t *slot_of_index, float4 *prim,
-                              float4 *primD, hipStream_t s);
+hipError_t refit_launch_prims(const unsigned char *raw, uint32_t first, uint32_t count, const uint32_t *slot_of_index, PrimRecords recs,
+                              hipStream_t s);
 hipError_t refit_launch_transform(unsigned char *raw, const uint32_t *start, const crt_prim_transform *ops, uint32_t n_ops, uint32_t total,
-                                  const uint32_t *slot_of_index, float4 *prim, float4 *primD, hipStream_t s);
+                                  const uint32_t *slot_of_index, PrimRecords recs, hipStream_t s);
 hipError_t refit_launch_compact(const unsigned char *src, unsigned char *dst, const uint32_t *tab, uint32_t n_gaps, uint32_t n_new, hipStream_t s);
 hipError_t refit_levels(const void *nodes, uint32_t width, bool quantised, int root, uint32_t cap, int *list, uint32_t *counter,
                         uint32_t *nch, std::vector<uint32_t> &off, hipStream_t s);
-hipError_t refit_launch_bvh2(const float4 *prim, float pad, const int *list, const std::vector<uint32_t> &off, float *nodes, hipStream_t s);
-hipError_t refit_launch_wide(const float4 *prim, float pad, const int *list, const std::vector<uint32_t> &off, const void *refs,
+hipError_t refit_launch_bvh2(PrimRecords recs, float pad, const int *list, const std::vector<uint32_t> &off, float *nodes, hipStream_t s);
+hipError_t refit_launch_wide(PrimRecords recs, float pad, const int *list, const std::vector<uint32_t> &off, const void *refs,
                              bool quantised, const uint32_t *nch, float *fb, hipStream_t s);
 hipError_t refit_launch_quant4(const float *fb, const uint32_t *nch, uint32_t n4, uint4 *nodes4q, const double base[3], const double scale[3],
                                hipStream_t s);
diff --git a/computeraytracer_amd/csrc/crt_lbvh.hip b/computeraytracer_amd/csrc/crt_lbvh.hip
--- a/computeraytracer_amd/csrc/crt_lbvh.hip
+++ b/computeraytracer_amd/csrc/crt_lbvh.hip
@@ -318,15 +318,14 @@
 }
 
 __global__ __launch_bounds__(256) void k_lbvh_gather_prims(const unsigned char *__restrict__ raw, const unsigned long long *__restrict__ keys, uint32_t n,
-                                                           float4 *__restrict__ prim, float4 *__restrict__ primD, uint32_t *__restrict__ slot_of_index)
+                                                           const PrimRecords recs, uint32_t *__restrict__ slot_of_index)
 {
     const uint32_t slot = blockIdx.x * 256u + threadIdx.x;
     if (slot >= n) return;
     const RawPrim p = load_raw(raw, (size_t)(keys[slot] & 0xFFFFFFFFull));
     float4 A, B, C, D;
     prim_record(p, A, B, C, D);
-    prim[3 * (size_t)slot + 0] = A; prim[3 * (size_t)slot + 1] = B; prim[3 * (size_t)slot + 2] = C;
-    primD[slot] = D;
+    prim_store(recs, slot, A, B, C, D);
     slot_of_index[p.index] = slot;
 }
 
@@ -350,10 +349,10 @@
     return hipSuccess;
 }
 
-hipError_t lbvh_launch_gather(const unsigned char *d_raw, const unsigned long long *d_keys, uint32_t n, float4 *d_prim, float4 *d_primD,
+hipError_t lbvh_launch_gather(const unsigned char *d_raw, const unsigned long long *d_keys, uint32_t n, PrimRecords recs,
                               uint32_t *d_slot_of_index, hipStream_t stream)
 {
-    hipLaunchKernelGGL(k_lbvh_gather_prims, dim3((n + 255u) / 256u), dim3(256), 0, stream, d_raw, d_keys, n, d_prim, d_primD, d_slot_of_index);
+    hipLaunchKernelGGL(k_lbvh_gather_prims, dim3((n + 255u) / 256u), dim3(256), 0, stream, d_raw, d_keys, n, recs, d_slot_of_index);
     return hipGetLastError();
 }
 
@@ -399,7 +398,7 @@
     return hipSuccess;
 }
 
-hipError_t build_lbvh_device(const unsigned char *d_raw, uint32_t n, float hit_pad, float4 *d_prim, float4 *d_primD,
+hipError_t build_lbvh_device(const unsigned char *d_raw, uint32_t n, float hit_pad, PrimRecords recs,
                              uint32_t *d_slot_of_index, float *d_nodes2, uint4 *d_nodes4q, LbvhDeviceResult &res, hipStream_t stream)
 {
     res = LbvhDeviceResult();
@@ -423,7 +422,7 @@
     hipLaunchKernelGGL(k_lbvh_bounds, dim3(blocks), dim3(256), 0, stream, d_sorted.p, (int)n, d_lo.p, d_hi.p, d_child.p, d_pi.p, d_pl.p,
                        d_flag.p, d_nb.p, d_nodes2, d_height.p);
     LB(hipGetLastError());
-    LB(lbvh_launch_gather(d_raw, d_sorted.p, n, d_prim, d_primD, d_slot_of_index, stream));
+    LB(lbvh_launch_gather(d_raw, d_sorted.p, n, recs, d_slot_of_index, stream));
     int depth = 0;
     LB(hipMemcpyAsync(&depth, d_height.p, sizeof depth, hipMemcpyDeviceToHost, stream));
     LB(hipStreamSynchronize(stream));
diff --git a/computeraytracer_amd/csrc/crt_matte.hip b/computeraytracer_amd/csrc/crt_matte.hip
--- a/computeraytracer_amd/csrc/crt_matte.hip
+++ b/computeraytracer_amd/csrc/crt_matte.hip
@@ -33,7 +33,7 @@
         if (P.source == CRT_MATTE_OBJECT) {
             id = P.table[b_index];
         } else if (P.source == CRT_MATTE_MATERIAL) {
-            const uint32_t meta = f_bits(S.prim[3 * b_slot].w);
+            const uint32_t meta = f_bits(prim_part(S, b_slot, 0).w);
             id = (((meta >> 2) & 3u) << 24) | ((meta >> 18) & 0x3FFFu);
         }
         h++;
diff --git a/computeraytracer_amd/csrc/crt_ploc.hip b/computeraytracer_amd/csrc/crt_ploc.hip
--- a/computeraytracer_amd/csrc/crt_ploc.hip
+++ b/computeraytracer_amd/csrc/crt_ploc.hip
@@ -236,7 +236,7 @@
     return hipSuccess;
 }
 
-hipError_t build_ploc_device(const unsigned char *d_raw, uint32_t n, float hit_pad, const PlocOptions &opt, float4 *d_prim, float4 *d_primD,
+hipError_t build_ploc_device(const unsigned char *d_raw, uint32_t n, float hit_pad, const PlocOptions &opt, PrimRecords recs,
                              uint32_t *d_slot_of_index, float *d_nodes2, uint4 *d_nodes4q, LbvhDeviceResult &res, PlocInfo &info,
                              hipStream_t stream)
 {
@@ -253,7 +253,7 @@
     PL(lbvh_sorted_keys_device(d_raw, n, hit_pad, d_lo.p, d_hi.p, d_cbox.p, d_keys.p, d_sorted.p, d_tmp, stream));
     PL(ploc_core(d_sorted.p, d_lo.p, d_hi.p, n, opt, d_nodes2, d_order.p, info, stream));
     if (info.abandoned) return hipSuccess;
-    PL(lbvh_launch_gather(d_raw, d_order.p, n, d_prim, d_primD, d_slot_of_index, stream));
+    PL(lbvh_launch_gather(d_raw, d_order.p, n, recs, d_slot_of_index, stream));
     res.max_depth = info.depth;
     return lbvh_collapse_device(d_nodes2, n, d_nodes4q, res, stream);
 }
diff --git a/computeraytracer_amd/csrc/crt_prim.h b/computeraytracer_amd/csrc/crt_prim.h
--- a/computeraytracer_amd/csrc/crt_prim.h
+++ b/computeraytracer_amd/csrc/crt_prim.h
@@ -1,9 +1,24 @@
 #pragma once
 #include <hip/hip_runtime.h>
 
+#include "crt_device.h"
 #include "crt_math.h"
 
 namespace crt {
+
+__device__ __forceinline__ const float4 &prim_part(const DevScene &S, size_t slot, uint32_t k) { return S.prim[(size_t)S.prim_quads * slot + k]; }
+__device__ __forceinline__ const float4 &prim_partD(const DevScene &S, size_t slot)
+{
+    return S.prim_quads == 4u ? S.prim[(size_t)S.prim_quads * slot + 3u] : S.primD[slot];
+}
+
+__device__ __forceinline__ float4 prim_part(const PrimRecords &R, size_t slot, uint32_t k) { return R.prim[(size_t)R.quads * slot + k]; }
+__device__ __forceinline__ void prim_store(const PrimRecords &R, size_t slot, const float4 A, const float4 B, const float4 C, const float4 D)
+{
+    float4 *r = R.prim + (size_t)R.quads * slot;
+    r[0] = A; r[1] = B; r[2] = C;
+    if (R.quads == 4u) r[3] = D; else R.primD[slot] = D;
+}
 
 struct RawPrim { uint32_t category; f3 d1, d2, d3; uint32_t emission, reflectance, material, index; };
 
diff --git a/computeraytracer_amd/csrc/crt_prim_layout.h b/computeraytracer_amd/csrc/crt_prim_layout.h
--- /dev/null
+++ b/computeraytracer_amd/csrc/crt_prim_layout.h
@@ -0,0 +1,21 @@
+#pragma once
+#include <stdint.h>
+
+#ifndef CRT_WF_PATCH_RECOMPUTE
+#define CRT_WF_PATCH_RECOMPUTE 20
+#endif
+
+namespace crt {
+
+inline uint32_t prim_record_quads(uint32_t nprim, uint32_t npatch)
+{
+    return ((unsigned long long)npatch << CRT_WF_PATCH_RECOMPUTE) > (unsigned long long)nprim ? 4u : 3u;
+}
+
+inline bool prim_record_option_valid(int opt) { return opt == 0 || opt == 48 || opt == 64; }
+inline uint32_t prim_record_quads_for(int opt, uint32_t nprim, uint32_t npatch)
+{
+    return opt == 48 ? 3u : opt == 64 ? 4u : prim_record_quads(nprim, npatch);
+}
+
+}
diff --git a/computeraytracer_amd/csrc/crt_refit.hip b/computeraytracer_amd/csrc/crt_refit.hip
--- a/computeraytracer_amd/csrc/crt_refit.hip
+++ b/computeraytracer_amd/csrc/crt_refit.hip
@@ -11,10 +11,10 @@
 namespace crt {
 namespace {
 
-__device__ __forceinline__ void leaf_box(const float4 *__restrict__ prim, uint32_t first, uint32_t count, float pad, float b[6])
+__device__ __forceinline__ void leaf_box(const PrimRecords &recs, uint32_t first, uint32_t count, float pad, float b[6])
 {
     for (uint32_t k = 0; k < count; k++) {
-        const float4 A = prim[3 * (size_t)(first + k) + 0], B = prim[3 * (size_t)(first + k) + 1], C = prim[3 * (size_t)(first + k) + 2];
+        const float4 A = prim_part(recs, first + k, 0), B = prim_part(recs, first + k, 1), C = prim_part(recs, first + k, 2);
         float l[3], h[3];
         prim_bounds(f_bits(A.w) & 3u, f3{A.x, A.y, A.z}, f3{B.x, B.y, B.z}, f3{C.x, C.y, C.z}, pad, l, h);
         for (int a = 0; a < 3; a++) {
@@ -47,8 +47,7 @@
 }
 
 __global__ __launch_bounds__(256) void k_refit_prims(const unsigned char *__restrict__ raw, uint32_t first, uint32_t count,
-                                                     const uint32_t *__restrict__ slot_of_index, float4 *__restrict__ prim,
-                                                     float4 *__restrict__ primD)
+                                                     const uint32_t *__restrict__ slot_of_index, const PrimRecords recs)
 {
     const uint32_t k = blockIdx.x * 256u + threadIdx.x;
     if (k >= count) return;
@@ -56,8 +55,7 @@
     float4 A, B, C, D;
     prim_record(p, A, B, C, D);
     const uint32_t slot = slot_of_index[first + k];
-    prim[3 * (size_t)slot + 0] = A; prim[3 * (size_t)slot + 1] = B; prim[3 * (size_t)slot + 2] = C;
-    primD[slot] = D;
+    prim_store(recs, slot, A, B, C, D);
 }
 
 __device__ __forceinline__ f3 xf_vector(const float *__restrict__ m, f3 v)
@@ -74,7 +72,7 @@
 
 __global__ __launch_bounds__(256) void k_refit_transform(unsigned char *raw, const uint32_t *__restrict__ start, const crt_prim_transform *__restrict__ ops,
                                                          uint32_t n_ops, uint32_t total, const uint32_t *__restrict__ slot_of_index,
-                                                         float4 *__restrict__ prim, float4 *__restrict__ primD)
+                                                         const PrimRecords recs)
 {
     const uint32_t t = blockIdx.x * 256u + threadIdx.x;
     if (t >= total) return;
@@ -98,12 +96,11 @@
         rec[8] = p.d2.x; rec[9] = p.d2.y; rec[10] = p.d2.z;
         rec[12] = p.d3.x; rec[13] = p.d3.y; rec[14] = p.d3.z;
     }
-    if (!prim) return;
+    if (!recs.prim) return;
     float4 A, B, C, D;
     prim_record(p, A, B, C, D);
     const uint32_t slot = slot_of_index[i];
-    prim[3 * (size_t)slot + 0] = A; prim[3 * (size_t)slot + 1] = B; prim[3 * (size_t)slot + 2] = C;
-    primD[slot] = D;
+    prim_store(recs, slot, A, B, C, D);
 }
 
 __global__ __launch_bounds__(256) void k_edit_compact(const uint4 *__restrict__ src, uint4 *__restrict__ dst, const uint32_t *__restrict__ gap,
@@ -144,7 +141,7 @@
         if (pos + j < cap) out[pos + j] = inner[j];
 }
 
-__global__ __launch_bounds__(256) void k_refit_bvh2(const float4 *__restrict__ prim, float pad, const int *__restrict__ list, uint32_t count,
+__global__ __launch_bounds__(256) void k_refit_bvh2(const PrimRecords recs, float pad, const int *__restrict__ list, uint32_t count,
                                                     float *__restrict__ nodes)
 {
     const uint32_t t = blockIdx.x * 256u + threadIdx.x;
@@ -154,7 +151,7 @@
         const int ref = (int)f_bits(nd[12 + c]);
         float b[6];
         if (ref < 0) {
-            leaf_box(prim, (uint32_t)(~ref) >> 3, ((uint32_t)(~ref) & 7u) + 1u, pad, b);
+            leaf_box(recs, (uint32_t)(~ref) >> 3, ((uint32_t)(~ref) & 7u) + 1u, pad, b);
         } else {
             const float4 *ch = (const float4 *)(nodes + (size_t)ref * kNodeFloats);
             const float4 q0 = ch[0], q1 = ch[1], q2 = ch[2];
@@ -165,7 +162,7 @@
     }
 }
 
-__global__ __launch_bounds__(256) void k_refit_wide(const float4 *__restrict__ prim, float pad, const int *__restrict__ list, uint32_t count,
+__global__ __launch_bounds__(256) void k_refit_wide(const PrimRecords recs, float pad, const int *__restrict__ list, uint32_t count,
                                                     const uint32_t *__restrict__ refs, uint32_t stride, uint32_t ref_at,
                                                     const uint32_t *__restrict__ nch, float *__restrict__ fb)
 {
@@ -178,7 +175,7 @@
         if (ref == 0) continue;
         float b[6];
         if (ref < 0) {
-            leaf_box(prim, (uint32_t)(~ref) >> 3, ((uint32_t)(~ref) & 7u) + 1u, pad, b);
+            leaf_box(recs, (uint32_t)(~ref) >> 3, ((uint32_t)(~ref) & 7u) + 1u, pad, b);
         } else {
             const float *ch = fb + (size_t)ref * kNode4Floats;
             const uint32_t k = nch[ref];
@@ -225,19 +222,19 @@
     return hipGetLastError();
 }
 
-hipError_t refit_launch_prims(const unsigned char *raw, uint32_t first, uint32_t count, const uint32_t *slot_of_index, float4 *prim,
-                              float4 *primD, hipStream_t s)
+hipError_t refit_launch_prims(const unsigned char *raw, uint32_t first, uint32_t count, const uint32_t *slot_of_index, PrimRecords recs,
+                              hipStream_t s)
 {
     if (count == 0) return hipSuccess;
-    hipLaunchKernelGGL(k_refit_prims, dim3(blocks_of(count)), dim3(256), 0, s, raw, first, count, slot_of_index, prim, primD);
+    hipLaunchKernelGGL(k_refit_prims, dim3(blocks_of(count)), dim3(256), 0, s, raw, first, count, slot_of_index, recs);
     return hipGetLastError();
 }
 
 hipError_t refit_launch_transform(unsigned char *raw, const uint32_t *start, const crt_prim_transform *ops, uint32_t n_ops, uint32_t total,
-                                  const uint32_t *slot_of_index, float4 *prim, float4 *primD, hipStream_t s)
+                                  const uint32_t *slot_of_index, PrimRecords recs, hipStream_t s)
 {
     if (total == 0) return hipSuccess;
-    hipLaunchKernelGGL(k_refit_transform, dim3(blocks_of(total)), dim3(256), 0, s, raw, start, ops, n_ops, total, slot_of_index, prim, primD);
+    hipLaunchKernelGGL(k_refit_transform, dim3(blocks_of(total)), dim3(256), 0, s, raw, start, ops, n_ops, total, slot_of_index, recs);
     return hipGetLastError();
 }
 
@@ -275,23 +272,23 @@
     return e;
 }
 
-hipError_t refit_launch_bvh2(const float4 *prim, float pad, const int *list, const std::vector<uint32_t> &off, float *nodes, hipStream_t s)
+hipError_t refit_launch_bvh2(PrimRecords recs, float pad, const int *list, const std::vector<uint32_t> &off, float *nodes, hipStream_t s)
 {
     for (size_t l = off.size() - 1; l-- > 0;) {
         const uint32_t count = off[l + 1] - off[l];
-        hipLaunchKernelGGL(k_refit_bvh2, dim3(blocks_of(count)), dim3(256), 0, s, prim, pad, list + off[l], count, nodes);
+        hipLaunchKernelGGL(k_refit_bvh2, dim3(blocks_of(count)), dim3(256), 0, s, recs, pad, list + off[l], count, nodes);
         const hipError_t e = hipGetLastError();
         if (e != hipSuccess) return e;
     }
     return hipSuccess;
 }
 
-hipError_t refit_launch_wide(const float4 *prim, float pad, const int *list, const std::vector<uint32_t> &off, const void *refs,
+hipError_t refit_launch_wide(PrimRecords recs, float pad, const int *list, const std::vector<uint32_t> &off, const void *refs,
                              bool quantised, const uint32_t *nch, float *fb, hipStream_t s)
 {
     for (size_t l = off.size() - 1; l-- > 0;) {
         const uint32_t count = off[l + 1] - off[l];
-        hipLaunchKernelGGL(k_refit_wide, dim3(blocks_of(count)), dim3(256), 0, s, prim, pad, list + off[l], count, (const uint32_t *)refs,
+        hipLaunchKernelGGL(k_refit_wide, dim3(blocks_of(count)), dim3(256), 0, s, recs, pad, list + off[l], count, (const uint32_t *)refs,
                            quantised ? 16u : 32u, quantised ? 12u : 24u, nch, fb);
         const hipError_t e = hipGetLastError();
         if (e != hipSuccess) return e;
diff --git a/computeraytracer_amd/csrc/crt_scene.cpp b/computeraytracer_amd/csrc/crt_scene.cpp
--- a/computeraytracer_amd/csrc/crt_scene.cpp
+++ b/computeraytracer_amd/csrc/crt_scene.cpp
@@ -99,13 +99,31 @@
         (void)fail(c, CRT_OK, "crt_build_accel: the PLOC build had not finished after %u rounds (the limit); built the LBVH instead", info.rounds);
 }
 
+static uint32_t count_patches(const crt_ctx *c)
+{
+    uint32_t np = 0;
+    for (const HostPrim &p : c->prims) np += p.category == 0u ? 1u : 0u;
+    return np;
+}
+
+static hipError_t alloc_records(DevBuf<float4> &prim, DevBuf<float4> &primD, size_t n, uint32_t quads)
+{
+    hipError_t e = prim.alloc(std::max<size_t>(n, 1) * quads);
+    if (e != hipSuccess) return e;
+    if (quads == 4u) {
+        primD.release();
+        if (((uintptr_t)prim.p & 63u) != 0u) return hipErrorInvalidValue;
+        return hipSuccess;
+    }
+    return primD.alloc(std::max<size_t>(n, 1));
+}
+
 static int build_accel_on_device(crt_ctx *c, bool *done)
 {
     *done = false;
     const uint32_t n = (uint32_t)c->prims.size();
     if (n < 2 || !c->quantize || c->wf_width != 4 || c->d_raw.n < (size_t)n * 80) return CRT_OK;
-    HIPCHK(c, c->d_prim.alloc((size_t)n * 3));
-    HIPCHK(c, c->d_primD.alloc(n));
+    HIPCHK(c, alloc_records(c->d_prim, c->d_primD, n, c->sc.prim_quads));
     HIPCHK(c, c->d_slot_of_index.alloc(n));
     HIPCHK(c, c->d_nodes.alloc((size_t)(n - 1) * 4));
     HIPCHK(c, c->d_nodes4q.alloc((size_t)(n - 1) * 4));
@@ -114,14 +132,14 @@
     int builder = 1;
     if (c->want_builder == 2) {
         PlocInfo info;
-        const hipError_t e = build_ploc_device(c->d_raw.p, n, c->sc.hit_pad, c->ploc, c->d_prim.p, c->d_primD.p, c->d_slot_of_index.p,
+        const hipError_t e = build_ploc_device(c->d_raw.p, n, c->sc.hit_pad, c->ploc, prim_records(c), c->d_slot_of_index.p,
                                                (float *)c->d_nodes.p, c->d_nodes4q.p, res, info, c->stream);
         if (e != hipSuccess) return fail(c, e == hipErrorOutOfMemory ? CRT_ENOMEM : CRT_EDEVICE, "crt_build_accel: GPU PLOC build: %s", hipGetErrorString(e));
         if (info.abandoned) ploc_abandoned_note(c, info);
         else builder = 2;
     }
     if (builder == 1) {
-        const hipError_t e = build_lbvh_device(c->d_raw.p, n, c->sc.hit_pad, c->d_prim.p, c->d_primD.p, c->d_slot_of_index.p,
+        const hipError_t e = build_lbvh_device(c->d_raw.p, n, c->sc.hit_pad, prim_records(c), c->d_slot_of_index.p,
                                                (float *)c->d_nodes.p, c->d_nodes4q.p, res, c->stream);
         if (e != hipSuccess) return fail(c, e == hipErrorOutOfMemory ? CRT_ENOMEM : CRT_EDEVICE, "crt_build_accel: GPU LBVH build: %s", hipGetErrorString(e));
     }
@@ -138,8 +156,7 @@
     c->sc.nodes4q = c->d_nodes4q.p;
     c->sc.nodes8q = nullptr; c->sc.root8 = -1;
     c->sc.nprim = n;
-    c->sc.npatch = 0;
-    for (const HostPrim &hp_ : c->prims) c->sc.npatch += hp_.category == 0u ? 1u : 0u;
+    c->sc.npatch = count_patches(c);
     c->accel_mode = CRT_ACCEL_BVH2;
     *done = true;
     return CRT_OK;
@@ -227,7 +244,8 @@
         c->bvh.root = -1;
     }
 
-    std::vector<float4> hp((size_t)n * 3), hd(n);
+    const uint32_t quads = c->sc.prim_quads;
+    std::vector<float4> hp((size_t)n * quads), hd(quads == 4u ? 0 : n);
     std::vector<uint32_t> slot_of(n);
     for (uint32_t slot = 0; slot < n; slot++) {
         const HostPrim &p = c->prims[order[slot]];
@@ -246,15 +264,15 @@
             float r = p.d2.x;
             B = float4{r, r * r, 0.0f, bits_f(p.index)};
         }
-        hp[3 * (size_t)slot + 0] = A; hp[3 * (size_t)slot + 1] = B; hp[3 * (size_t)slot + 2] = C;
-        hd[slot] = D;
-    }
-    HIPCHK(c, c->d_prim.alloc(std::max<size_t>(hp.size(), 3)));
-    HIPCHK(c, c->d_primD.alloc(std::max<size_t>(hd.size(), 1)));
+        float4 *rec = &hp[(size_t)quads * slot];
+        rec[0] = A; rec[1] = B; rec[2] = C;
+        if (quads == 4u) rec[3] = D; else hd[slot] = D;
+    }
+    HIPCHK(c, alloc_records(c->d_prim, c->d_primD, n, quads));
     HIPCHK(c, c->d_slot_of_index.alloc(std::max<size_t>(n, 1)));
     if (n) {
         HIPCHK(c, hipMemcpy(c->d_prim.p, hp.data(), hp.size() * sizeof(float4), hipMemcpyHostToDevice));
-        HIPCHK(c, hipMemcpy(c->d_primD.p, hd.data(), hd.size() * sizeof(float4), hipMemcpyHostToDevice));
+        if (!hd.empty()) HIPCHK(c, hipMemcpy(c->d_primD.p, hd.data(), hd.size() * sizeof(float4), hipMemcpyHostToDevice));
         HIPCHK(c, hipMemcpy(c->d_slot_of_index.p, slot_of.data(), n * sizeof(uint32_t), hipMemcpyHostToDevice));
     }
     size_t nn = c->bvh.nodes.size() / 4;
@@ -296,8 +314,7 @@
     c->sc.nodes = c->d_nodes.p;
     c->sc.root = c->bvh.root;
     c->sc.nprim = n;
-    c->sc.npatch = 0;
-    for (const HostPrim &hp_ : c->prims) c->sc.npatch += hp_.category == 0u ? 1u : 0u;
+    c->sc.npatch = count_patches(c);
     c->accel_mode = mode;
     return CRT_OK;
 }
@@ -308,6 +325,11 @@
 {
     const uint32_t need = wf_stack_need(c), lds = wf_stack_lds(c);
     return std::max(kWfOverflowLevels, need > lds ? need - lds : 0u);
+}
+
+void choose_prim_layout(crt_ctx *c)
+{
+    c->sc.prim_quads = prim_record_quads_for(c->prim_record, (uint32_t)c->prims.size(), count_patches(c));
 }
 
 int build_tree(crt_ctx *c, int mode)
@@ -432,10 +454,10 @@
         }
         c->rf_ready = true;
     }
-    HIPCHK(c, refit_launch_bvh2(c->d_prim.p, pad, c->rf_lv2.p, c->rf_off2, (float *)c->d_nodes.p, c->stream));
+    HIPCHK(c, refit_launch_bvh2(prim_records(c), pad, c->rf_lv2.p, c->rf_off2, (float *)c->d_nodes.p, c->stream));
     if (wide) {
         float *fb = wide_float ? (float *)c->d_nodes4.p : c->rf_fb.p;
-        HIPCHK(c, refit_launch_wide(c->d_prim.p, pad, c->rf_lv4.p, c->rf_off4, refs4, quant, c->rf_nch4.p, fb, c->stream));
+        HIPCHK(c, refit_launch_wide(prim_records(c), pad, c->rf_lv4.p, c->rf_off4, refs4, quant, c->rf_nch4.p, fb, c->stream));
         if (quant) {
             float root[kNode4Floats];
             uint32_t k = 0;
@@ -551,7 +573,7 @@
     if (count) {
         HIPCHK(c, hipMemcpyAsync(c->d_raw.p + (size_t)first * 80, records, (size_t)count * 80, hipMemcpyHostToDevice, c->stream));
         if (c->accel_mode >= 0 && !c->accel_topo)
-            HIPCHK(c, refit_launch_prims(c->d_raw.p, first, count, c->d_slot_of_index.p, c->d_prim.p, c->d_primD.p, c->stream));
+            HIPCHK(c, refit_launch_prims(c->d_raw.p, first, count, c->d_slot_of_index.p, prim_records(c), c->stream));
     }
     return prims_edit_end(c);
 }
@@ -596,7 +618,7 @@
         HIPCHK(c, hipMemcpyAsync(c->xf_tab.p, tab.data(), tab.size() * 4, hipMemcpyHostToDevice, c->stream));
         const bool built = c->accel_mode >= 0 && !c->accel_topo;
         HIPCHK(c, refit_launch_transform(c->d_raw.p, c->xf_tab.p, (const crt_prim_transform *)(c->xf_tab.p + head), (uint32_t)live.size(), total,
-                                         c->d_slot_of_index.p, built ? c->d_prim.p : nullptr, built ? c->d_primD.p : nullptr, c->stream));
+                                         c->d_slot_of_index.p, built ? prim_records(c) : PrimRecords{nullptr, nullptr, c->sc.prim_quads}, c->stream));
         c->prims_moved = true;
     }
     return prims_edit_end(c);
@@ -638,8 +660,7 @@
     if (new_snap) HIPCHK(c, e.snap.alloc(new_snap));
     if (e.lights_replaced) HIPCHK(c, e.d_lights.alloc(e.lights.size() * 3));
     if (records_change && c->accel_mode == CRT_ACCEL_NONE) {
-        HIPCHK(c, e.prim.alloc(std::max<size_t>(n_new * 3, 3)));
-        HIPCHK(c, e.primD.alloc(std::max<size_t>(n_new, 1)));
+        HIPCHK(c, alloc_records(e.prim, e.primD, n_new, c->sc.prim_quads));
         HIPCHK(c, e.slot.alloc(std::max<size_t>(n_new, 1)));
     }
     HIPCHK(c, e.scan.alloc(1));
@@ -671,12 +692,11 @@
             e.iota.resize(n);
             for (uint32_t i = 0; i < n; i++) e.iota[i] = i;
             HIPCHK(c, hipMemcpyAsync(e.slot.p, e.iota.data(), (size_t)n * 4, hipMemcpyHostToDevice, c->stream));
-            HIPCHK(c, refit_launch_prims(c->d_raw.p, 0, n, e.slot.p, e.prim.p, e.primD.p, c->stream));
+            HIPCHK(c, refit_launch_prims(c->d_raw.p, 0, n, e.slot.p, PrimRecords{e.prim.p, e.primD.p, S.prim_quads}, c->stream));
             c->d_prim = std::move(e.prim); c->d_primD = std::move(e.primD); c->d_slot_of_index = std::move(e.slot);
             S.prim = c->d_prim.p; S.primD = c->d_primD.p; S.slot_of_index = c->d_slot_of_index.p;
             S.nprim = n;
-            S.npatch = 0;
-            for (const HostPrim &p : c->prims) S.npatch += p.category == 0u ? 1u : 0u;
+            S.npatch = count_patches(c);
         }
         if (c->accel_mode == CRT_ACCEL_BVH2) c->accel_topo = true;
     }
diff --git a/computeraytracer_amd/csrc/crt_shade.h b/computeraytracer_amd/csrc/crt_shade.h
--- a/computeraytracer_amd/csrc/crt_shade.h
+++ b/computeraytracer_amd/csrc/crt_shade.h
@@ -1,6 +1,7 @@
 #pragma once
 #include "crt_device.h"
 #include "crt_math.h"
+#include "crt_prim.h"
 #include "../../include/crt.h"
 
 namespace crt {
@@ -163,11 +164,11 @@
 __device__ __forceinline__ bool hit_test(const DevScene &S, uint32_t slot, f3 o, f3 d, uint32_t exclude,
                                          float t_min, float &t_max, uint32_t &b_index, uint32_t &b_slot)
 {
-    const float4 A = S.prim[3 * slot + 0];
-    const float4 B = S.prim[3 * slot + 1];
-    const float4 C = S.prim[3 * slot + 2];
+    const float4 A = prim_part(S, slot, 0);
+    const float4 B = prim_part(S, slot, 1);
+    const float4 C = prim_part(S, slot, 2);
     float4 D = float4{0.0f, 0.0f, 0.0f, 0.0f};
-    if (exclude != f_bits(B.w) && (f_bits(A.w) & 3u) == 0u) D = S.primD[slot];
+    if (exclude != f_bits(B.w) && (f_bits(A.w) & 3u) == 0u) D = prim_partD(S, slot);
     return hit_test_rec<LITERAL>(A, B, C, D, S.hit_pad, slot, o, d, exclude, t_min, t_max, b_index, b_slot);
 }
 
@@ -190,11 +191,11 @@
 __device__ __forceinline__ void hit_attributes(const DevScene &S, uint32_t slot, f3 o, f3 d, float t,
                                                f3 &pos, f3 &nrm, uint32_t &meta)
 {
-    const float4 A = S.prim[3 * slot + 0];
+    const float4 A = prim_part(S, slot, 0);
     const uint32_t cat = f_bits(A.w) & 3u;
     float4 B = float4{0.0f, 0.0f, 0.0f, 0.0f}, C = B, D = B;
-    if (cat == 0u) D = S.primD[slot];
-    else if (cat == 2u) { B = S.prim[3 * slot + 1]; C = S.prim[3 * slot + 2]; }
+    if (cat == 0u) D = prim_partD(S, slot);
+    else if (cat == 2u) { B = prim_part(S, slot, 1); C = prim_part(S, slot, 2); }
     hit_attributes_rec(A, B, C, D, o, d, t, pos, nrm, meta);
 }
 
diff --git a/computeraytracer_amd/csrc/crt_wavefront.hip b/computeraytracer_amd/csrc/crt_wavefront.hip
--- a/computeraytracer_amd/csrc/crt_wavefront.hip
+++ b/computeraytracer_amd/csrc/crt_wavefront.hip
@@ -25,9 +25,6 @@
 #endif
 #ifndef CRT_WF_SPEC
 #define CRT_WF_SPEC 1
-#endif
-#ifndef CRT_WF_PATCH_RECOMPUTE
-#define CRT_WF_PATCH_RECOMPUTE 20
 #endif
 #ifndef CRT_WF_SHADE_BLOCK
 #define CRT_WF_SHADE_BLOCK 64
@@ -73,12 +70,12 @@
     return (uint32_t)__popcll(mask & ((1ull << lane) - 1ull));
 }
 
-__device__ __noinline__ float2 resolve_nonfinite(const float4 *prim, const float4 *primD, const uint32_t *slot_of_index,
+__device__ __noinline__ float2 resolve_nonfinite(const float4 *prim, const float4 *primD, uint32_t prim_quads, const uint32_t *slot_of_index,
                                                  uint32_t nprim, float hit_pad, float ox, float oy, float oz, float dx,
                                                  float dy, float dz, uint32_t exclude)
 {
     DevScene S{};
-    S.prim = prim; S.primD = primD; S.slot_of_index = slot_of_index; S.nprim = nprim; S.hit_pad = hit_pad;
+    S.prim = prim; S.primD = primD; S.prim_quads = prim_quads; S.slot_of_index = slot_of_index; S.nprim = nprim; S.hit_pad = hit_pad;
     float tm = CRT_INFINITY;
     uint32_t bi = kNoHit, bs = kNoHit;
     const f3 o = f3{ox, oy, oz}, d = f3{dx, dy, dz};
@@ -144,8 +141,8 @@
         const uint32_t include = f_bits(r.L1.w);
         if (include < S.nprim) {
             r.slot = ((cptr1)S.slot_of_index)[include];
-            const cptr4 pg = (cptr4)S.prim + 3 * (size_t)r.slot;
-            r.A = ld(pg); r.B = ld(pg + 1); r.C = ld(pg + 2); r.D = ld((cptr4)S.primD + r.slot);
+            r.A = ld((cptr4)&prim_part(S, r.slot, 0)); r.B = ld((cptr4)&prim_part(S, r.slot, 1)); r.C = ld((cptr4)&prim_part(S, r.slot, 2));
+            r.D = ld((cptr4)&prim_partD(S, r.slot));
             r.pdf_area = r.L2.w;
         }
     } else {
@@ -153,8 +150,8 @@
         const uint32_t include = f_bits(r.L1.w);
         if (include < S.nprim) {
             r.slot = S.slot_of_index[include];
-            r.A = S.prim[3 * (size_t)r.slot + 0]; r.B = S.prim[3 * (size_t)r.slot + 1]; r.C = S.prim[3 * (size_t)r.slot + 2];
-            r.D = S.primD[r.slot];
+            r.A = prim_part(S, r.slot, 0); r.B = prim_part(S, r.slot, 1); r.C = prim_part(S, r.slot, 2);
+            r.D = prim_partD(S, r.slot);
             uint32_t l2 = (f_bits(r.A.w) >> 4) & 0x3FFFu;
             if (l2 >= S.nlight) l2 = S.nlight - 1u;
             r.pdf_area = S.lights[3 * l2 + 2].w;
@@ -277,7 +274,7 @@
     const uint32_t h_slot = f_bits(h.y);
     const bool has_hit = alive && !nan_ray && !(R.flags & kWfDying) && h_slot != kNoHit;
     float4 hA = float4{0, 0, 0, 0}, hB = hA, hC = hA, hD = hA;
-    if (has_hit) { hA = S.prim[3 * (size_t)h_slot + 0]; hB = S.prim[3 * (size_t)h_slot + 1]; hC = S.prim[3 * (size_t)h_slot + 2]; if (S.npatch) hD = S.primD[h_slot]; }
+    if (has_hit) { hA = prim_part(S, h_slot, 0); hB = prim_part(S, h_slot, 1); hC = prim_part(S, h_slot, 2); if (S.npatch) hD = prim_partD(S, h_slot); }
     CRT_PROBE(tp, 2)
 
     if (alive) {
@@ -459,7 +456,7 @@
         if (so.alive) {
             stnt(&P.ray_o[slot], float4{R.ray_o.x, R.ray_o.y, R.ray_o.z, bits_f(R.exclude)});
             if (so.emit_ext && (!finite3(R.ray_o) || !finite3(R.ray_d))) {
-                P.hit[slot] = resolve_nonfinite(S.prim, S.primD, S.slot_of_index, S.nprim, S.hit_pad, R.ray_o.x, R.ray_o.y, R.ray_o.z,
+                P.hit[slot] = resolve_nonfinite(S.prim, S.primD, S.prim_quads, S.slot_of_index, S.nprim, S.hit_pad, R.ray_o.x, R.ray_o.y, R.ray_o.z,
                                                 R.ray_d.x, R.ray_d.y, R.ray_d.z, R.exclude);
                 if (COUNT) cn.prims += S.nprim;
                 resolved = 1u;
@@ -1143,7 +1140,7 @@
                     const uint32_t first = enc >> 3, cnt = (enc & 7u) + 1u;
                     for (uint32_t i = 0; i < cnt; i++) {
                         const uint32_t ps = first + i;
-                        const float4 A = prim[3 * (size_t)ps + 0], B = prim[3 * (size_t)ps + 1], C = prim[3 * (size_t)ps + 2];
+                        const float4 A = prim_part(S, ps, 0), B = prim_part(S, ps, 1), C = prim_part(S, ps, 2);
                         if ((f_bits(A.w) & 3u) == 2u) tri_test(A, B, C, ps, o, d, excl, t_min, hit_pad, t_max, b_index, b_slot);
                         else hit_test<false>(S, ps, o, d, excl, t_min, t_max, b_index, b_slot);
                     }
@@ -1411,7 +1408,7 @@
     int *__restrict__ ovf = P.stack_overflow + ((size_t)blockIdx.x * 64 + lane_id());
     const size_t ovl = P.overflow_lanes;
     const uint32_t nprim = P.sc.nprim;
-    const bool fetchD = ((unsigned long long)P.sc.npatch << CRT_WF_PATCH_RECOMPUTE) > (unsigned long long)nprim;
+    const bool fetchD = P.sc.prim_quads == 4u;
     DevScene S = P.sc;
     S.prim = prim; S.primD = primD;
 
@@ -1595,7 +1592,7 @@
                 const int owner = (int)tk.y;
                 const uint32_t ps = tk.x;
                 float4 A = float4{0, 0, 0, 0}, B = A, C = A, D = A;
-                if (lane < T) { A = prim[3 * (size_t)ps + 0]; B = prim[3 * (size_t)ps + 1]; C = prim[3 * (size_t)ps + 2]; if (fetchD) D = primD[ps]; }
+                if (lane < T) { A = prim_part(S, ps, 0); B = prim_part(S, ps, 1); C = prim_part(S, ps, 2); if (fetchD) D = prim_partD(S, ps); }
                 bool from_pend = false;
                 if (incl) {
                     from_pend = pend != 0;
diff --git a/computeraytracer_amd/renderer.py b/computeraytracer_amd/renderer.py
--- a/computeraytracer_amd/renderer.py
+++ b/computeraytracer_amd/renderer.py
@@ -569,9 +569,12 @@
     def accel_stats(self) -> dict:
         out = np.zeros(8, np.uint64)
         self._chk(self._lib.crt_accel_stats(self._h, out.ctypes.data))
+        quads = C.c_uint32()
+        self._chk(self._lib.crt_prim_record_quads(self._h, C.byref(quads)))
         return dict(nodes=int(out[0]), leaves=int(out[1]), max_depth=int(out[2]), bytes=int(out[3]),
                     bytes_per_box=int(out[4]), width=int(out[5]), wide_nodes=int(out[6]),
-                    builder=("sah-host", "lbvh-gpu", "ploc-gpu")[int(out[7])])
+                    builder=("sah-host", "lbvh-gpu", "ploc-gpu")[int(out[7])],
+                    prim_quads=int(quads.value))
 
     def debug_intersect(self, origins, directions, exclude=None) -> np.ndarray:
         o = np.asarray(origins, np.float32).reshape(-1, 3)
diff --git a/include/crt.h b/include/crt.h
--- a/include/crt.h
+++ b/include/crt.h
@@ -223,6 +223,8 @@
 
 int crt_accel_stats(crt_ctx *ctx, uint64_t out[8]);
 
+int crt_prim_record_quads(crt_ctx *ctx, uint32_t *quads);
+
 int crt_debug_intersect(crt_ctx *ctx, const float *rays, size_t n, float *out);
 int crt_debug_trace_rays(crt_ctx *ctx, const float *rays, size_t n, uint32_t *out, uint64_t report[8]);
 int crt_debug_walk_rays(crt_ctx *ctx, int walk, const float *rays, size_t n, uint32_t *out, uint64_t report[8]);
```

Result: no change. 8208 Mrays/s, median of 6 (+0.7%).
